# wang-xinyu/tensorrtx

Measured on AMD Instinct MI355X. Metric: images/sec @ batch=32 640x640 fp16 (yolov8n conv backbone + YoloLayer decode + NMS), higher is better.
Workload: dtype f16

## Files before the change

### include/trtx_hip.h

```cpp
#ifndef TRTX_HIP_H_
#define TRTX_HIP_H_

#include <stddef.h>
#include <stdint.h>

#ifdef __cplusplus
extern "C" {
#endif

#ifndef TRTX_NO_HIP_TYPES
struct ihipStream_t;
typedef struct ihipStream_t* trtx_stream_t;
#endif

#define TRTX_ABI_VERSION 1
#define TRTX_OK 0
#define TRTX_ERR_INVALID 1
#define TRTX_ERR_HIP 2
#define TRTX_ERR_WORKSPACE 3
#define TRTX_ERR_UNSUPPORTED 4
#define TRTX_ERR_NO_DEVICE 5
#define TRTX_ERR_IO 6
#define TRTX_ERR_STATE 7

// ... 19 lines not shown
                                   float* output, void* workspace, size_t workspace_bytes, trtx_stream_t stream);
int32_t trtx_yolo_task_head_decode_nhwc(const void* const* heads, const int* ld, const void* const* branches, const int* branch_ld,
                                        int n_levels, int batch, int classes, int net_h, int net_w, const int* strides,
                                        const float* dfl_weights, int max_out, int is_seg, int is_pose, int is_obb, int n_kpt,
                                        float kpt_conf, float* output, void* workspace, size_t workspace_bytes, trtx_stream_t stream);
int32_t trtx_yolo_task_head_decode_nhwc_f32(const void* const* heads, const int* ld, const void* const* branches, const int* branch_ld,
                                            int n_levels, int batch, int classes, int net_h, int net_w, const int* strides,
                                            const float* dfl_weights, int max_out, int is_seg, int is_pose, int is_obb, int n_kpt,
                                            float kpt_conf, float* output, void* workspace, size_t workspace_bytes, trtx_stream_t stream);

size_t trtx_yolo_nms_workspace(int batch);
int32_t trtx_yolo_nms(const float* decode_out, int batch, int max_out, float conf_thresh, float nms_thresh,
                      int32_t* keep_idx, int32_t* keep_cnt, float* keep_det, void* workspace, size_t workspace_bytes,
                      trtx_stream_t stream);


size_t trtx_yolov5_decode_workspace(int batch, const int* grid_w, const int* grid_h, int n_levels);
int32_t trtx_yolov5_decode(const float* const* inputs, int n_levels, int batch, int classes, int net_h, int net_w,
                           const int* grid_w, const int* grid_h, const float* anchors, int max_out, int is_segmentation,
                           float* output, void* workspace, size_t workspace_bytes, trtx_stream_t stream);
size_t trtx_yolov5_head_decode_workspace(int batch, const int* grid_w, const int* grid_h, int n_levels);
int32_t trtx_yolov5_head_decode_nhwc(const void* const* heads, const int* ld, int n_levels, int batch, int classes, int net_h, int net_w,
                                     const int* grid_w, const int* grid_h, const float* anchors, int max_out, float* output,
                                     void* workspace, size_t workspace_bytes, trtx_stream_t stream);
int32_t trtx_yolov5_head_decode_nhwc_f32(const void* const* heads, const int* ld, int n_levels, int batch, int classes, int net_h, int net_w,
                                         const int* grid_w, const int* grid_h, const float* anchors, int max_out, float* output,
                                         void* workspace, size_t workspace_bytes, trtx_stream_t stream);
size_t trtx_yolov7_decode_workspace(int batch, const int* grid_w, const int* grid_h, int n_levels);
int32_t trtx_yolov7_decode(const float* const* inputs, int n_levels, int batch, int classes, int net_h, int net_w,
                           const int* grid_w, const int* grid_h, const float* anchors, int max_out, float* output, void* workspace,
                           size_t workspace_bytes, trtx_stream_t stream);
size_t trtx_yolov7_head_decode_workspace(int batch, const int* grid_w, const int* grid_h, int n_levels);
int32_t trtx_yolov7_head_decode_nhwc(const void* const* heads, const int* ld, int n_levels, int batch, int classes, int net_h, int net_w,
                                     const int* grid_w, const int* grid_h, const float* anchors, int max_out, float* output,
                                     void* workspace, size_t workspace_bytes, trtx_stream_t stream);
int32_t trtx_yolov7_head_decode_nhwc_f32(const void* const* heads, const int* ld, int n_levels, int batch, int classes, int net_h, int net_w,
                                         const int* grid_w, const int* grid_h, const float* anchors, int max_out, float* output,
                                         void* workspace, size_t workspace_bytes, trtx_stream_t stream);
size_t trtx_darknet_decode_workspace(int batch, const int* grid_w, const int* grid_h, int n_levels);
int32_t trtx_darknet_decode(const float* const* inputs, int n_levels, int batch, int classes, int net_h, int net_w,
                            const int* grid_w, const int* grid_h, const float* anchors, int max_out, float* output, void* workspace,
                            size_t workspace_bytes, trtx_stream_t stream);
size_t trtx_darknet_head_decode_workspace(int batch, const int* grid_w, const int* grid_h, int n_levels);
int32_t trtx_darknet_head_decode_nhwc(const void* const* heads, const int* ld, int n_levels, int batch, int classes, int net_h, int net_w,
                                      const int* grid_w, const int* grid_h, const float* anchors, int max_out, float* output,
                                      void* workspace, size_t workspace_bytes, trtx_stream_t stream);
int32_t trtx_darknet_head_decode_nhwc_f32(const void* const* heads, const int* ld, int n_levels, int batch, int classes, int net_h, int net_w,
                                          const int* grid_w, const int* grid_h, const float* anchors, int max_out, float* output,
                                          void* workspace, size_t workspace_bytes, trtx_stream_t stream);
size_t trtx_yolov9_decode_workspace(int batch, int net_h, int net_w);
int32_t trtx_yolov9_decode(const float* const* inputs, int batch, int classes, int net_h, int net_w, int max_out, int is_segmentation,
                           float* output, void* workspace, size_t workspace_bytes, trtx_stream_t stream);
size_t trtx_yolov9_head_decode_workspace(int batch, int net_h, int net_w);
int32_t trtx_yolov9_head_decode_nhwc(const void* const* box, const int* box_ld, const void* const* cls, const int* cls_ld, int batch, int classes,
                                     int net_h, int net_w, const float* dfl_weights, int max_out, float* output, void* workspace,
                                     size_t workspace_bytes, trtx_stream_t stream);
int32_t trtx_yolov9_head_decode_nhwc_f32(const void* const* box, const int* box_ld, const void* const* cls, const int* cls_ld, int batch, int classes,
                                         int net_h, int net_w, const float* dfl_weights, int max_out, float* output, void* workspace,
                                         size_t workspace_bytes, trtx_stream_t stream);
int32_t trtx_yolo_nms_obb(const float* decode_out, int batch, int max_out, float conf_thresh, float nms_thresh, int32_t* keep_idx,
                          int32_t* keep_cnt, float* keep_det, void* workspace, size_t workspace_bytes, trtx_stream_t stream);
int32_t trtx_yolo_postprocess_gpu_obb(const float* decode_out, int batch, int max_out, float conf_thresh, float nms_thresh, float* out,
                                      trtx_stream_t stream);
int32_t trtx_yolov5_nms(const float* decode_out, int batch, int max_out, float conf_thresh, float nms_thresh, int32_t* keep_idx,
                        int32_t* keep_cnt, float* keep_det, void* workspace, size_t workspace_bytes, trtx_stream_t stream);
int32_t trtx_yolov9_nms(const float* decode_out, int batch, int max_out, float conf_thresh, float nms_thresh, int32_t* keep_idx,
                        int32_t* keep_cnt, float* keep_det, void* workspace, size_t workspace_bytes, trtx_stream_t stream);
int32_t trtx_yolov7_nms(const float* decode_out, int batch, int max_out, float conf_thresh, float nms_thresh, int32_t* keep_idx,
                        int32_t* keep_cnt, float* keep_det, void* workspace, size_t workspace_bytes, trtx_stream_t stream);
int32_t trtx_darknet_nms(const float* decode_out, int batch, int max_out, float conf_thresh, float nms_thresh, int32_t* keep_idx,
                         int32_t* keep_cnt, float* keep_det, void* workspace, size_t workspace_bytes, trtx_stream_t stream);
int32_t trtx_seg_masks(const float* decode_out, int det_floats, int box_format, const int32_t* keep_idx, const int32_t* keep_cnt, int batch,
                       int max_out, int max_keep, const float* proto, int mask_h, int mask_w, int net_h, int net_w, float* masks,
                       trtx_stream_t stream);

void trtx_letterbox_matrix(int src_w, int src_h, int dst_w, int dst_h, float* d2s_out );
int32_t trtx_letterbox_batch(const void* const* src, const int* src_w, const int* src_h, int batch, float* dst, int dst_w, int dst_h,
                             trtx_stream_t stream);
int32_t trtx_preprocess_init(int max_image_size, int ring_depth);
void trtx_preprocess_destroy(void);
int32_t trtx_batch_preprocess(const void* const* src_host, const int* src_w, const int* src_h, int batch, float* dst, int dst_w, int dst_h,
                              trtx_stream_t stream);

int32_t trtx_yolo_postprocess_gpu(const float* decode_out, int batch, int max_out, float conf_thresh, float nms_thresh,
                                  float* out, trtx_stream_t stream);

int32_t trtx_mish(const float* in, float* out, size_t n, trtx_stream_t stream);

size_t trtx_retina_decode_output_floats(int net_h, int net_w);
size_t trtx_retina_decode_workspace(int batch, int net_h, int net_w);
int32_t trtx_retina_decode(const float* const* inputs, int batch, int net_h, int net_w, float* output, void* workspace,
                           size_t workspace_bytes, trtx_stream_t stream);
size_t trtx_retina_nms_workspace(int batch, int net_h, int net_w);
int32_t trtx_retina_nms(const float* decode_out, int batch, int net_h, int net_w, double conf_thresh, float nms_thresh,
                        int max_keep, int32_t* keep_idx, int32_t* keep_cnt, float* keep_det, void* workspace,
                        size_t workspace_bytes, trtx_stream_t stream);

size_t trtx_rpn_decode_workspace(int batch, int num_anchors, int height, int width);
int32_t trtx_rpn_decode(int batch, const float* scores, const float* deltas, int height, int width, int image_height,
                        int image_width, float stride, const float* anchors_host, int num_anchors, int top_n,
                        float* out_scores, float* out_boxes, void* workspace, size_t workspace_bytes,
                        trtx_stream_t stream);
size_t trtx_sorted_nms_workspace(int batch, int n);
int32_t trtx_rpn_nms(int batch, const float* scores, const float* boxes, int pre_nms_topk, int post_nms_topk,
                     float nms_thresh, float* out_boxes, void* workspace, size_t workspace_bytes,
                     trtx_stream_t stream);
int32_t trtx_roi_align(int batch, const float* boxes, const float* features, int pooler_resolution, float spatial_scale,
                       int sampling_ratio, int num_proposals, int channels, int feature_h, int feature_w, float* out,
                       trtx_stream_t stream);
int32_t trtx_roi_align_nhwc_f16(int batch, const float* boxes, const void* features, int ld_in, int pooler_resolution,
                                float spatial_scale, int sampling_ratio, int num_proposals, int channels, int feature_h,
                                int feature_w, void* out, int ld_out, trtx_stream_t stream);
int32_t trtx_roi_align_nhwc_f16_strided(int batch, const float* boxes, const void* features, int ld_in, int pooler_resolution,
                                        float spatial_scale, int sampling_ratio, int num_proposals, int channels, int feature_h,
                                        int feature_w, void* out, int ld_out, int bin_step, trtx_stream_t stream);
size_t trtx_predictor_decode_workspace(int batch, int num_boxes, int num_classes);
int32_t trtx_predictor_decode(int batch, const float* scores, const float* deltas, const float* proposals, int num_boxes,
                              int num_classes, int image_height, int image_width, const float* bbox_reg_weights_host,
                              float* out_scores, float* out_boxes, float* out_classes, void* workspace,
                              size_t workspace_bytes, trtx_stream_t stream);
int32_t trtx_batched_nms(int nms_method, int batch, const float* scores, const float* boxes, const float* classes,
                         int count, int detections_per_im, float nms_thresh, float* out_scores, float* out_boxes,
                         float* out_classes, void* workspace, size_t workspace_bytes, trtx_stream_t stream);

int32_t trtx_mask_rcnn_inference(int batch, const float* labels, const float* masks, int detections_per_im, int output_size,
                                 int num_classes, float* out_masks, trtx_stream_t stream);

#define TRTX_ACT_NONE 0
#define TRTX_ACT_RELU 1
#define TRTX_ACT_SIGMOID 2
#define TRTX_ACT_SILU 3
#define TRTX_ACT_LEAKY 4
#define TRTX_ACT_TANH 5
int32_t trtx_conv_packed_dims(int cout, int cin_pad, int kh, int kw, int32_t* cout_pad, int32_t* kpad, int32_t* bn);
int32_t trtx_conv_pack_weights_f16(const float* w_kcrs, int cout, int cin, int kh, int kw, int cin_pad,
                                   const float* ch_scale, uint16_t* packed);
int32_t trtx_op_conv2d_nhwc_f16(const void* in, int N, int H, int W, int Cin, int ld_in, const void* wpacked,
                                const float* bias, void* out, int Cout, int ld_out, int kh, int kw, int sh, int sw,
                                int ph, int pw, int act1, const void* residual, int ld_res, int act2,
                                trtx_stream_t stream);
int32_t trtx_op_conv2d_tactics(int N, int H, int W, int Cin, int ld_in, int Cout, int ld_out, int kh, int kw, int sh, int sw, int ph, int pw,
                               int has_residual, int ld_res, int32_t* out6, int32_t max_out);
int32_t trtx_op_conv_force_tactic(const int32_t* tactic6);
int32_t trtx_op_conv_stem_nchw_f16(const float* in, int N, int C, int H, int W, const float* w_taps_cout, const float* bias, void* out, int Cout,
                                   int ld_out, int k, int stride, int pad, int act, trtx_stream_t stream);
int32_t trtx_op_conv_stem_pair_f16(const float* in, int N, int C, int H, int W, const float* stem_w_taps_cout, const float* stem_bias, int stem_act,
                                   const void* conv_wpacked, const float* conv_bias, int conv_act, void* out, int ld_out, trtx_stream_t stream);
int32_t trtx_op_conv_bneck_pair_f16(const void* in, int N, int H, int W, int ld_in, int in_coff, const void* w1_packed, const float* bias1, int act1,
                                    const void* w2_packed, const float* bias2, int act2, int shortcut, int act_after, void* out, int ld_out,
                                    trtx_stream_t stream);
int32_t trtx_op_conv_bneck_pair_or_two_f16(const void* in, int N, int H, int W, int ld_in, int in_coff, const void* w1_packed, const float* bias1, int act1,
                                           const void* w2_packed, const float* bias2, int act2, int shortcut, int act_after, void* mid, void* out,
                                           int ld_out, trtx_stream_t stream);
int32_t trtx_reorg_fold_weights(const float* w_kcrs, int cout, int cin, int kh, int kw, float* folded);
int32_t trtx_conv_packed_dims_f32(int cout, int cin_pad, int kh, int kw, int32_t* cout_pad, int32_t* kpad, int32_t* cink);
int32_t trtx_conv_pack_weights_f32(const float* w_kcrs, int cout, int cin, int kh, int kw, int cin_pad, const float* ch_scale, float* packed);
int32_t trtx_op_conv2d_nhwc_f32(const void* in, int N, int H, int W, int Cin, int ld_in, const void* wpacked, const float* bias, void* out, int Cout,
                                int ld_out, int kh, int kw, int sh, int sw, int ph, int pw, int act1, const void* residual, int ld_res, int act2,
                                const int32_t* tile4, trtx_stream_t stream);
int32_t trtx_op_conv2d_tactics_f32(int N, int H, int W, int Cin, int ld_in, int Cout, int ld_out, int kh, int kw, int sh, int sw, int ph, int pw,
                                   int has_residual, int ld_res, int32_t* out4, int32_t max_out);
int32_t trtx_conv_pack_weights_i8(const float* w_kcrs, int cout, int cin, int kh, int kw, const float* ch_scale, int8_t* packed, float* wscale_out,
                                  int32_t* cout_pad_out, int32_t* kpad_out);
int32_t trtx_op_conv2d_nhwc_i8(const void* in, int N, int H, int W, int Cin, int ld_in, const void* wpacked, const float* cscale, const float* bias, void* out,
                               int out_is_i8, float out_inv_scale, int Cout, int ld_out, int kh, int kw, int sh, int sw, int ph, int pw, int act1,
                               const void* residual, int res_is_i8, float res_scale, int ld_res, int act2, trtx_stream_t stream);
int32_t trtx_conv_pack_weights_grouped_f16(const float* w_kcrs, int cout, int cin_g, int kh, int kw, const float* ch_scale, uint16_t* packed,
                                           int32_t* kpad_out);
int32_t trtx_op_conv2d_grouped_nhwc_f16(const void* in, int N, int H, int W, int Cin, int ld_in, const void* wpacked, const float* bias, void* out,
                                        int Cout, int ld_out, int groups, int k, int pad, int act1, const void* residual, int ld_res, int act2,
                                        trtx_stream_t stream);
int32_t trtx_op_conv2d_dw_nhwc(const void* in, int dtype, int N, int H, int W, int C, int ld_in, const float* w_taps_c, const float* bias, void* out, int ld_out,
                               const void* residual, int ld_res, int k, int stride, int pad, int dilation, int act1, float alpha1, int act2, float alpha2,
                               trtx_stream_t stream);
int32_t trtx_op_psa_attention_f16(const void* qkv, int ld_qkv, void* out, int ld_out, void* vimg, int ld_v, int B, int heads, int N, int kd, int hd, float scale,
                                  trtx_stream_t stream);
int32_t trtx_op_area_attention_f16(const void* qkv, int ld_qkv, void* out, int ld_out, void* vimg, int ld_v, int B, int heads, int N, int area, int kd, int hd,
                                   float scale, trtx_stream_t stream);
int32_t trtx_op_area_attention_split_f16(const void* q, int ld_q, const void* k, int ld_k, const void* v, int ld_v, void* out, int ld_out, int B, int heads,
                                         int N, int area, int kd, int hd, float scale, trtx_stream_t stream);
size_t trtx_op_hgconv_workspace_bytes(int B, int N, int D, int E);
int32_t trtx_op_hgconv_geometry(int32_t* tiles, int max_tiles, int32_t* n_tiles);
int32_t trtx_op_hgconv_f16(const void* x, int ld_x, void* out, int ld_out, int B, int N, int D, int E, float logit_scale, const float* w_ctx, const float* b_ctx,
                           const float* proto, const float* w_pre, const float* b_pre, const float* w_edge, const float* b_edge, const float* w_node,
                           const float* b_node, void* workspace, size_t workspace_bytes, trtx_stream_t stream);
int32_t trtx_op_poison_lds(void* device_word, trtx_stream_t stream);
int32_t trtx_op_nchw_f32_to_nhwc_f16(const float* in, void* out, int N, int C, int H, int W, int Cpad, int ld_out,
                                     trtx_stream_t stream);
int32_t trtx_op_nhwc_f16_to_nchw_f32(const void* in, float* out, int N, int C, int H, int W, int ld_in,
                                     trtx_stream_t stream);

typedef struct trtx_builder trtx_builder;
typedef struct trtx_network trtx_network;
typedef struct trtx_hostmem trtx_hostmem;
typedef struct trtx_engine trtx_engine;
typedef struct trtx_context trtx_context;
typedef struct trtx_plugin trtx_plugin;

#define TRTX_MAX_DIMS 8
typedef struct trtx_dims {
    int32_t nb;
    int64_t d[TRTX_MAX_DIMS];
} trtx_dims;

#define TRTX_DTYPE_FLOAT 0
#define TRTX_DTYPE_HALF 1
#define TRTX_DTYPE_INT8 2
#define TRTX_DTYPE_INT32 3
#define TRTX_ACTIVATION_RELU 0
#define TRTX_ACTIVATION_SIGMOID 1
#define TRTX_ACTIVATION_TANH 2
#define TRTX_ACTIVATION_LEAKY_RELU 3
#define TRTX_POOLING_MAX 0
#define TRTX_POOLING_AVERAGE 1
#define TRTX_ELEMENTWISE_SUM 0
#define TRTX_ELEMENTWISE_PROD 1
#define TRTX_ELEMENTWISE_MAX 2
#define TRTX_ELEMENTWISE_MIN 3
#define TRTX_ELEMENTWISE_SUB 4
#define TRTX_ELEMENTWISE_DIV 5
#define TRTX_ELEMENTWISE_POW 6
#define TRTX_SCALE_UNIFORM 0
#define TRTX_SCALE_CHANNEL 1
#define TRTX_SCALE_ELEMENTWISE 2
#define TRTX_REDUCE_SUM 0
#define TRTX_REDUCE_PROD 1
#define TRTX_REDUCE_MAX 2
#define TRTX_REDUCE_MIN 3
#define TRTX_REDUCE_AVG 4
#define TRTX_MATMUL_NONE 0
#define TRTX_MATMUL_TRANSPOSE 1
#define TRTX_MATMUL_VECTOR 2
#define TRTX_UNARY_EXP 0
#define TRTX_UNARY_LAST 23
#define TRTX_RESIZE_NEAREST 0
#define TRTX_RESIZE_LINEAR 1
#define TRTX_FLAG_FP16 0
#define TRTX_FLAG_INT8 1
#define TRTX_P_STRIDE 1
#define TRTX_P_PADDING 2
#define TRTX_P_DILATION 3
#define TRTX_P_GROUPS 4
#define TRTX_P_ALPHA 5
#define TRTX_P_BETA 6
#define TRTX_P_AXIS 7
#define TRTX_P_RESHAPE 8
#define TRTX_P_FIRST_TRANSPOSE 9
#define TRTX_P_SECOND_TRANSPOSE 10
#define TRTX_P_RESIZE_MODE 11
#define TRTX_P_RESIZE_SCALES 12
#define TRTX_P_RESIZE_OUT_DIMS 13
#define TRTX_P_AVG_EXCLUSIVE 14
#define TRTX_P_KERNEL 15
#define TRTX_P_NB_OUT 16

typedef struct trtx_plugin_vtbl {
    void* self;
    int32_t (*get_nb_outputs)(void* self);
    int32_t (*get_output_dims)(void* self, int32_t index, const trtx_dims* inputs, int32_t nb_inputs, trtx_dims* out);
    int32_t (*configure)(void* self, const trtx_dims* in, int32_t nb_in, const trtx_dims* out, int32_t nb_out,
                         int32_t max_batch);
    int32_t (*initialize)(void* self);
    void (*terminate)(void* self);
    size_t (*workspace_size)(void* self, int32_t max_batch);
    int32_t (*enqueue)(void* self, int32_t batch, const void* const* inputs, void* const* outputs, void* workspace,
                       trtx_stream_t stream);
    size_t (*serialization_size)(void* self);
    void (*serialize)(void* self, void* buffer);
    const char* (*plugin_type)(void* self);
    const char* (*plugin_version)(void* self);
    int32_t (*clone)(void* self, struct trtx_plugin_vtbl* out);
    void (*destroy)(void* self);
} trtx_plugin_vtbl;

typedef struct trtx_plugin_field {
    const char* name;
    const void* data;
    int32_t type;
    int32_t length;
} trtx_plugin_field;

typedef struct trtx_creator_vtbl {
    void* self;
    const char* (*plugin_name)(void* self);
    const char* (*plugin_version)(void* self);
    int32_t (*create)(void* self, const char* name, const trtx_plugin_field* fields, int32_t nb_fields,
                      trtx_plugin_vtbl* out);
    int32_t (*deserialize)(void* self, const char* name, const void* data, size_t length, trtx_plugin_vtbl* out);
} trtx_creator_vtbl;

int32_t trtx_registry_register(const trtx_creator_vtbl* creator);
int32_t trtx_registry_get(const char* name, const char* version, trtx_creator_vtbl* out);

typedef struct trtx_wts trtx_wts;
int32_t trtx_wts_load(const char* path, trtx_wts** out);
int32_t trtx_wts_count(const trtx_wts* w);
int32_t trtx_wts_entry(const trtx_wts* w, int32_t i, const char** name, const float** values, int64_t* count);
int32_t trtx_wts_find(const trtx_wts* w, const char* name, const float** values, int64_t* count);
void trtx_wts_free(trtx_wts* w);

int32_t trtx_builder_create(trtx_builder** out);
void trtx_builder_destroy(trtx_builder* b);
int32_t trtx_builder_set_max_batch(trtx_builder* b, int32_t n);
int32_t trtx_builder_set_flag(trtx_builder* b, int32_t flag, int32_t on);
int32_t trtx_builder_set_workspace(trtx_builder* b, size_t bytes);
typedef struct trtx_calibrator_vtbl {
// ... 88 lines not shown
```

### tensorrtx_amd/capi.py

```python
import ctypes
import os

_HERE = os.path.dirname(os.path.abspath(__file__))
_LIB = None


class TrtxError(RuntimeError):
    def __init__(self, status, what):
        self.status = status
        msg = lib().trtx_status_string(status).decode() if _LIB is not None else "?"
        super().__init__(f"{what}: status {status} ({msg})")


def lib_path() -> str:
    return os.environ.get("TRTX_HIP_LIB") or os.path.join(_HERE, "lib", "libtrtx_hip.so")


def hip_runtimes_mapped():
    seen = []
    with open("/proc/self/maps") as f:
        for line in f:
            path = line.rsplit(" ", 1)[-1].strip()
            if "libamdhip64" in os.path.basename(path) and path not in seen:
                seen.append(path)
# ... 331 lines not shown
    return out


def yolov9_head_decode_nhwc(box, cls, classes, net_h, net_w, dfl_w, max_out=1000, out=None, batch=None, box_ld=None, cls_ld=None, ws=None):
    import torch
    L = lib()
    assert len(box) == 3 and len(cls) == 3
    B = box[0].shape[0] if batch is None else batch
    dev = box[0].device
    bp = (ctypes.c_void_p * 3)(*[x.data_ptr() for x in box])
    cp = (ctypes.c_void_p * 3)(*[x.data_ptr() for x in cls])
    bl = (ctypes.c_int * 3)(*(box_ld if box_ld is not None else [x.shape[-1] for x in box]))
    cl = (ctypes.c_int * 3)(*(cls_ld if cls_ld is not None else [x.shape[-1] for x in cls]))
    L.trtx_yolov9_head_decode_workspace.restype = ctypes.c_size_t
    if ws is None:
        ws = torch.empty(max(L.trtx_yolov9_head_decode_workspace(B, net_h, net_w), 256), dtype=torch.uint8, device=dev)
    if out is None:
        out = torch.zeros((B, 1 + max_out * DET5_FLOATS), dtype=torch.float32, device=dev)
    fn = L.trtx_yolov9_head_decode_nhwc_f32 if box[0].dtype == torch.float32 else L.trtx_yolov9_head_decode_nhwc
    check(fn(bp, bl, cp, cl, B, classes, net_h, net_w, _p(dfl_w), max_out, _p(out), _p(ws), ctypes.c_size_t(ws.numel()), _stream()),
          "trtx_yolov9_head_decode_nhwc")
    return out


def yolov9_nms(decode_out, max_out=1000, conf_thresh=0.5, nms_thresh=0.45, out=None, ws=None):
    L = lib()
    B = decode_out.shape[0]
    keep_idx, keep_cnt, keep_det, ws = _nms_buffers(B, max_out, 6, decode_out.device, out, ws)
    check(L.trtx_yolov9_nms(_p(decode_out), B, max_out, ctypes.c_float(conf_thresh), ctypes.c_float(nms_thresh), _p(keep_idx), _p(keep_cnt),
                            _p(keep_det), _p(ws), ctypes.c_size_t(ws.numel()), _stream()), "trtx_yolov9_nms")
    return keep_idx, keep_cnt, keep_det


def seg_masks(decode_out, keep_idx, keep_cnt, proto, net_h, net_w, max_keep, box_format=0, out=None):
    import torch
    B, max_out = keep_idx.shape
    assert decode_out.shape[0] == B and (decode_out.shape[1] - 1) % max_out == 0
    det_floats = (decode_out.shape[1] - 1) // max_out
    assert proto.dim() == 4 and proto.shape[0] == B and proto.shape[1] == 32
    mask_h, mask_w = int(proto.shape[2]), int(proto.shape[3])
    for t, dt in ((decode_out, torch.float32), (keep_idx, torch.int32), (keep_cnt, torch.int32), (proto, torch.float32)):
        assert t.is_cuda and t.dtype == dt and t.is_contiguous()
    if out is None:
        out = torch.zeros((B, max(max_keep, 0), mask_h, mask_w), dtype=torch.float32, device=proto.device)
    assert out.is_cuda and out.dtype == torch.float32 and out.is_contiguous() and out.numel() >= B * max(max_keep, 0) * mask_h * mask_w
    check(lib().trtx_seg_masks(_p(decode_out), det_floats, box_format, _p(keep_idx), _p(keep_cnt), B, max_out, max_keep, _p(proto), mask_h,
                               mask_w, net_h, net_w, _p(out), _stream()), "trtx_seg_masks")
    return out


def yolo_postprocess_gpu(decode_out, max_out=1000, conf_thresh=0.5, nms_thresh=0.45, out=None, ws=None):
    import torch
    B = decode_out.shape[0]
    if out is None:
        out = torch.empty((B, 1 + max_out * 7), dtype=torch.float32, device=decode_out.device)
    check(lib().trtx_yolo_postprocess_gpu(_p(decode_out), B, max_out, ctypes.c_float(conf_thresh), ctypes.c_float(nms_thresh),
                                          _p(out), _stream()), "trtx_yolo_postprocess_gpu")
    return out


ACT = {"none": 0, "relu": 1, "sigmoid": 2, "silu": 3, "leaky": 4, "tanh": 5, "mish": 6}


def _hw(v):
    if isinstance(v, (tuple, list)):
        h, w = v
        return int(h), int(w)
    return int(v), int(v)


def pack_conv_weights_f16(w_kcrs, cin_pad=None, ch_scale=None):
    import numpy as np
    L = lib()
    w = np.ascontiguousarray(w_kcrs, dtype=np.float32)
    cout, cin, kh, kw = w.shape
    cin_pad = cin_pad or (cin + 7) // 8 * 8
    cp, kp, bn = ctypes.c_int32(), ctypes.c_int32(), ctypes.c_int32()
    check(L.trtx_conv_packed_dims(cout, cin_pad, kh, kw, ctypes.byref(cp), ctypes.byref(kp), ctypes.byref(bn)),
          "trtx_conv_packed_dims")
    packed = np.zeros((cp.value, kp.value), dtype=np.uint16)
    sc = None
    if ch_scale is not None:
        sc = np.ascontiguousarray(ch_scale, dtype=np.float32)
    check(L.trtx_conv_pack_weights_f16(w.ctypes.data_as(ctypes.c_void_p), cout, cin, kh, kw, cin_pad,
                                       sc.ctypes.data_as(ctypes.c_void_p) if sc is not None else None,
                                       packed.ctypes.data_as(ctypes.c_void_p)), "trtx_conv_pack_weights_f16")
    return packed, cp.value, kp.value, bn.value


def conv2d_nhwc_f16(x, wpacked, bias, cout, kh, kw, stride, pad, act1="none", residual=None, act2="none",
                    out=None, out_ld=None):
    import torch
    L = lib()
    N, H, W, Cin = x.shape
    (sh, sw), (ph, pw) = _hw(stride), _hw(pad)
    Ho = (H + 2 * ph - kh) // sh + 1
    Wo = (W + 2 * pw - kw) // sw + 1
    if out is None:
        out = torch.empty((N, Ho, Wo, cout), dtype=torch.float16, device=x.device)
    ld_out = out_ld or out.shape[-1]
    check(L.trtx_op_conv2d_nhwc_f16(_p(x), N, H, W, Cin, x.stride(2), _p(wpacked), _p(bias), _p(out), cout, ld_out,
                                    kh, kw, sh, sw, ph, pw, ACT[act1], _p(residual),
                                    residual.stride(2) if residual is not None else 0, ACT[act2], _stream()),
          "trtx_op_conv2d_nhwc_f16")
    return out


def stem_weights(w_kcrs):
    import numpy as np
    w = np.ascontiguousarray(w_kcrs, dtype=np.float32)
    return np.ascontiguousarray(w.reshape(w.shape[0], -1).T)


def conv_stem_nchw_f16(x, w_taps_cout, bias, k, stride, pad, act="none", out=None, out_ld=None):
    import torch
    N, C, H, W = x.shape
    cout = w_taps_cout.shape[1]
    Ho, Wo = (H + 2 * pad - k) // stride + 1, (W + 2 * pad - k) // stride + 1
    if out is None:
        out = torch.empty((N, Ho, Wo, cout), dtype=torch.float16, device=x.device)
    check(lib().trtx_op_conv_stem_nchw_f16(_p(x), N, C, H, W, _p(w_taps_cout), _p(bias), _p(out), cout, out_ld or out.shape[-1], k, stride, pad,
                                           ACT[act], _stream()), "trtx_op_conv_stem_nchw_f16")
    return out


def conv_stem_pair_f16(x, stem_w_taps_cout, stem_bias, conv_wpacked, conv_bias, stem_act="silu", conv_act="silu", out=None, out_ld=None):
    import torch
    N, C, H, W = x.shape
    Hi, Wi = (H - 1) // 2 + 1, (W - 1) // 2 + 1
    Ho, Wo = (Hi - 1) // 2 + 1, (Wi - 1) // 2 + 1
    if out is None:
        out = torch.empty((N, Ho, Wo, 32), dtype=torch.float16, device=x.device)
    check(lib().trtx_op_conv_stem_pair_f16(_p(x), N, C, H, W, _p(stem_w_taps_cout), _p(stem_bias), ACT[stem_act], _p(conv_wpacked), _p(conv_bias),
                                           ACT[conv_act], _p(out), out_ld or out.shape[-1], _stream()), "trtx_op_conv_stem_pair_f16")
    return out


def conv_bneck_pair_f16(x, w1_packed, bias1, w2_packed, bias2, act1="silu", act2="silu", shortcut=True, act_after="none", out=None, out_ld=None, in_coff=None,
                        mid=None):
    import torch
    N, H, W, C = x.shape
    assert x.dtype == torch.float16 and x.stride(3) == 1 and (C == 16 if in_coff is None else in_coff + 16 <= C)
    if out is None:
        out = torch.empty((N, H, W, 16), dtype=torch.float16, device=x.device)
    head = (_p(x), N, H, W, x.stride(2), in_coff or 0, _p(w1_packed), _p(bias1), ACT[act1], _p(w2_packed), _p(bias2), ACT[act2], 1 if shortcut else 0, ACT[act_after])
    if mid is None:
        check(lib().trtx_op_conv_bneck_pair_f16(*head, _p(out), out_ld or out.shape[-1], _stream()), "trtx_op_conv_bneck_pair_f16")
    else:
        assert mid.dtype == torch.float16 and mid.is_contiguous() and tuple(mid.shape) == (N, H, W, 16)
        check(lib().trtx_op_conv_bneck_pair_or_two_f16(*head, _p(mid), _p(out), out_ld or out.shape[-1], _stream()), "trtx_op_conv_bneck_pair_or_two_f16")
    return out


def pack_conv_weights_grouped_f16(w_kcrs, ch_scale=None):
    import numpy as np
    L = lib()
    w = np.ascontiguousarray(w_kcrs, dtype=np.float32)
    cout, cin_g, kh, kw = w.shape
    kp = ctypes.c_int32()
    check(L.trtx_conv_pack_weights_grouped_f16(w.ctypes.data_as(ctypes.c_void_p), cout, cin_g, kh, kw, None, None, ctypes.byref(kp)),
          "trtx_conv_pack_weights_grouped_f16 (dims)")
    packed = np.zeros((cout, kp.value), dtype=np.uint16)
    sc = None if ch_scale is None else np.ascontiguousarray(ch_scale, dtype=np.float32)
    check(L.trtx_conv_pack_weights_grouped_f16(w.ctypes.data_as(ctypes.c_void_p), cout, cin_g, kh, kw,
                                               sc.ctypes.data_as(ctypes.c_void_p) if sc is not None else None,
                                               packed.ctypes.data_as(ctypes.c_void_p), ctypes.byref(kp)), "trtx_conv_pack_weights_grouped_f16")
    return packed


def conv2d_grouped_nhwc_f16(x, wpacked, bias, cout, groups, k, pad, act1="none", residual=None, act2="none", out=None, out_ld=None):
    import torch
    N, H, W, Cin = x.shape
    if out is None:
        out = torch.empty((N, H + 2 * pad - k + 1, W + 2 * pad - k + 1, cout), dtype=torch.float16, device=x.device)
    check(lib().trtx_op_conv2d_grouped_nhwc_f16(_p(x), N, H, W, Cin, x.stride(2), _p(wpacked), _p(bias), _p(out), cout, out_ld or out.shape[-1], groups, k,
                                                pad, ACT[act1], _p(residual), residual.stride(2) if residual is not None else 0, ACT[act2], _stream()),
          "trtx_op_conv2d_grouped_nhwc_f16")
    return out


def conv2d_dw_nhwc(x, w, bias, k, stride, act1="none", residual=None, act2="none", out=None, out_ld=None, alpha1=0.1, alpha2=0.1, pad=None, dilation=1):
    import numpy as np
    import torch
    N, H, W, C = x.shape
    assert x.dtype in (torch.float16, torch.float32) and (residual is None or residual.dtype == x.dtype)
    pad = k // 2 if pad is None else pad
    Ho, Wo = (H + 2 * pad - dilation * (k - 1) - 1) // stride + 1, (W + 2 * pad - dilation * (k - 1) - 1) // stride + 1
    taps = np.ascontiguousarray(np.asarray(w, dtype=np.float32).reshape(C, k * k).T)
    wg = torch.from_numpy(taps).to(x.device)
    if out is None:
        out = torch.empty((N, Ho, Wo, C), dtype=x.dtype, device=x.device)
    assert out.dtype == x.dtype
    check(lib().trtx_op_conv2d_dw_nhwc(_p(x), 1 if x.dtype == torch.float16 else 0, N, H, W, C, x.stride(2), _p(wg), _p(bias), _p(out),
                                       out_ld or out.shape[-1], _p(residual), residual.stride(2) if residual is not None else 0, k, stride, pad, dilation,
                                       ACT[act1], ctypes.c_float(alpha1), ACT[act2], ctypes.c_float(alpha2), _stream()), "trtx_op_conv2d_dw_nhwc")
    return out


def _attention(fn, what, qkv, heads, scale, out, vimg, out_ld, v_ld, qkv_ld, kd, hd, extra):
    import torch
    B, N, _ = qkv.shape
    for t in (qkv, out, vimg):
        assert t.is_cuda and t.dtype == torch.float16
    check(fn(_p(qkv), qkv_ld or qkv.stride(1), _p(out), out_ld or out.stride(1), _p(vimg), v_ld or vimg.stride(1), B, heads, N, *extra, kd, hd,
             ctypes.c_float(scale), _stream()), what)
    return out, vimg


def psa_attention(qkv, heads, scale, out=None, vimg=None, out_ld=None, v_ld=None, qkv_ld=None, kd=32, hd=64):
    import torch
    B, N, _ = qkv.shape
    out = torch.empty((B, N, heads * hd), dtype=torch.float16, device=qkv.device) if out is None else out
    vimg = torch.empty((B, N, heads * hd), dtype=torch.float16, device=qkv.device) if vimg is None else vimg
    return _attention(lib().trtx_op_psa_attention_f16, "trtx_op_psa_attention_f16", qkv, heads, scale, out, vimg, out_ld, v_ld, qkv_ld, kd, hd, ())


def area_attention(qkv, heads, area, scale, out=None, vimg=None, out_ld=None, v_ld=None, qkv_ld=None, kd=32, hd=32):
    import torch
    B, N, _ = qkv.shape
    out = torch.empty((B, N, heads * hd), dtype=torch.float16, device=qkv.device) if out is None else out
    vimg = torch.empty((B, N, heads * hd), dtype=torch.float16, device=qkv.device) if vimg is None else vimg
    return _attention(lib().trtx_op_area_attention_f16, "trtx_op_area_attention_f16", qkv, heads, scale, out, vimg, out_ld, v_ld, qkv_ld, kd, hd, (area,))


def area_attention_split(q, k, v, heads, area, scale, out=None, q_ld=None, k_ld=None, v_ld=None, out_ld=None, kd=32, hd=32):
    import torch
    B, N, _ = q.shape
    out = torch.empty((B, N, heads * hd), dtype=torch.float16, device=q.device) if out is None else out
    for t in (q, k, v, out):
        assert t.is_cuda and t.dtype == torch.float16
    check(lib().trtx_op_area_attention_split_f16(_p(q), q_ld or q.stride(1), _p(k), k_ld or k.stride(1), _p(v), v_ld or v.stride(1), _p(out),
                                                 out_ld or out.stride(1), B, heads, N, area, kd, hd, ctypes.c_float(scale), _stream()),
          "trtx_op_area_attention_split_f16")
    return out


HGCONV_WEIGHTS = ("w_ctx", "b_ctx", "proto", "w_pre", "b_pre", "w_edge", "b_edge", "w_node", "b_node")


def hgconv_workspace_bytes(B, N, D, E):
    L = lib()
    L.trtx_op_hgconv_workspace_bytes.restype = ctypes.c_size_t
    return int(L.trtx_op_hgconv_workspace_bytes(int(B), int(N), int(D), int(E)))


def hgconv_geometry():
    arr, n = (ctypes.c_int32 * 8)(), ctypes.c_int32()
    check(lib().trtx_op_hgconv_geometry(arr, 8, ctypes.byref(n)), "trtx_op_hgconv_geometry")
    return [int(arr[i]) for i in range(min(n.value, 8))]


def hgconv(x, E, logit_scale, weights, out=None, x_ld=None, out_ld=None, D=None, workspace=None):
    import torch
    L = lib()
    B, N, Dx = x.shape
    D = Dx if D is None else D
    assert x.is_cuda and x.dtype == torch.float16
    out = torch.empty((B, N, D), dtype=torch.float16, device=x.device) if out is None else out
    assert out.is_cuda and out.dtype == torch.float16
    ws = workspace if workspace is not None else torch.empty(max(hgconv_workspace_bytes(B, N, D, E), 256), dtype=torch.uint8, device=x.device)
    ws_arr = [weights[k].contiguous() for k in HGCONV_WEIGHTS]
    for w in ws_arr:
        assert w.is_cuda and w.dtype == torch.float32
    L.trtx_op_hgconv_f16.argtypes = ([ctypes.c_void_p, ctypes.c_int, ctypes.c_void_p, ctypes.c_int] + [ctypes.c_int] * 4 + [ctypes.c_float] +
                                     [ctypes.c_void_p] * 9 + [ctypes.c_void_p, ctypes.c_size_t, ctypes.c_void_p])
    check(L.trtx_op_hgconv_f16(_p(x), x_ld or x.stride(1), _p(out), out_ld or out.stride(1), B, N, D, E, float(logit_scale), *[_p(w) for w in ws_arr],
                               _p(ws), ws.numel(), _stream()), "trtx_op_hgconv_f16")
    return out


def pack_conv_weights_f32(w_kcrs, cin_pad=None, ch_scale=None):
    import numpy as np
    L = lib()
    w = np.ascontiguousarray(w_kcrs, dtype=np.float32)
    cout, cin, kh, kw = w.shape
    cin_pad = cin_pad or (cin + 3) // 4 * 4
    cp, kp, ck = ctypes.c_int32(), ctypes.c_int32(), ctypes.c_int32()
    check(L.trtx_conv_packed_dims_f32(cout, cin_pad, kh, kw, ctypes.byref(cp), ctypes.byref(kp), ctypes.byref(ck)), "trtx_conv_packed_dims_f32")
    packed = np.zeros((cp.value, kp.value), dtype=np.float32)
    sc = np.ascontiguousarray(ch_scale, dtype=np.float32) if ch_scale is not None else None
    check(L.trtx_conv_pack_weights_f32(w.ctypes.data_as(ctypes.c_void_p), cout, cin, kh, kw, cin_pad,
                                       sc.ctypes.data_as(ctypes.c_void_p) if sc is not None else None,
                                       packed.ctypes.data_as(ctypes.c_void_p)), "trtx_conv_pack_weights_f32")
    return packed, cp.value, kp.value, ck.value


def conv2d_nhwc_f32(x, wpacked, bias, cout, kh, kw, stride, pad, act1="none", residual=None, act2="none", out=None, out_ld=None, tile=None):
    import torch
    L = lib()
    N, H, W, Cin = x.shape
    if bias is not None and bias.numel() < (cout + 15) // 16 * 16:
        raise ValueError(f"bias holds {bias.numel()} floats, the fp32 tile reads cout_pad = {(cout + 15) // 16 * 16}")
    (sh, sw), (ph, pw) = _hw(stride), _hw(pad)
    Ho = (H + 2 * ph - kh) // sh + 1
    Wo = (W + 2 * pw - kw) // sw + 1
    if out is None:
        out = torch.empty((N, Ho, Wo, cout), dtype=torch.float32, device=x.device)
    ld_out = out_ld or out.shape[-1]
    t2 = (ctypes.c_int32 * 4)(*tile) if tile is not None else None
    check(L.trtx_op_conv2d_nhwc_f32(_p(x), N, H, W, Cin, x.stride(2), _p(wpacked), _p(bias), _p(out), cout, ld_out, kh, kw, sh, sw, ph, pw,
                                    ACT[act1], _p(residual), residual.stride(2) if residual is not None else 0, ACT[act2], t2, _stream()),
          "trtx_op_conv2d_nhwc_f32")
    return out


def conv2d_tactics_f32(N, H, W, Cin, Cout, k, stride, pad, residual=False, ld_in=None, ld_out=None, ld_res=None, max_out=32):
# ... 62 lines not shown
```

### tensorrtx_amd/csrc/kernels/conv_igemm.hip

```cpp
#include "../options.h"
#include "igemm_tile.h"
#include "patch_tile.h"

namespace trtx {
namespace {


struct ConvPatchGroupArgs {
    int n;
    int slot_start[kMaxConvGroup + 1];
    int chunk[kMaxConvGroup], tiles[kMaxConvGroup], tiles_n[kMaxConvGroup], tiles_x[kMaxConvGroup], tiles_y[kMaxConvGroup];
    unsigned in_bytes[kMaxConvGroup], w_bytes[kMaxConvGroup];
    ConvArgs p[kMaxConvGroup];
};
template <int NFRAG, int KC, int MI>
__global__ __launch_bounds__(256) void conv_patch_group_f16_kernel(const ConvPatchGroupArgs g) {
    __shared__ __attribute__((aligned(16))) char smem[patch_lds_bytes<NFRAG, KC, MI>()];
    const int xcd = blockIdx.x & 7, slot = blockIdx.x >> 3;
    int pid = 0;
#pragma unroll
    for (int k = 1; k < kMaxConvGroup; ++k) pid += (k < g.n && slot >= g.slot_start[k]) ? 1 : 0;
    pid = __builtin_amdgcn_readfirstlane(pid);
    const int local = xcd * g.chunk[pid] + (slot - g.slot_start[pid]);
    if (local >= g.tiles[pid]) return;
// ... 457 lines not shown
    const bool ws_ok = fp16 && !pinned && conv_ws_supported(a);
    if (ws_ok) push(a.bn, a.bk, 128, WSK_OFF, WS_ON);
    else push(a.bn, a.bk, 128, (wsk_default(a) && !work_efficient_only && !pinned) ? WSK_ON : WSK_OFF, WS_OFF);
    if (fp16 && options().gemm256 && conv_gemm256_worthwhile(a)) push(256, 64, 256, WSK_OFF, WS_OFF);
    const int bks[2] = {a.bk, (fp16 && a.CinK % 64 == 0 && a.CinK != 16 && a.Kpad % 64 == 0) ? (a.bk == 32 ? 64 : 32) : a.bk};
    static const int bns[5] = {128, 80, 64, 32, 16};
    for (int bi = 0; bi < 5; ++bi) {
        const int bn = bns[bi];
        if (a.Cout_pad % bn) continue;
        if (bn == 16 && a.Cout_pad > 32 && bn != a.bn) continue;
        if (work_efficient_only && bn != a.bn && bn != 64) continue;
        for (int ki = 0; ki < 2; ++ki) {
            ConvArgs t = a;
            t.bn = bn;
            t.bk = bks[ki];
            if (ki == 1 && bks[1] == bks[0]) continue;
            push(bn, t.bk, 128, WSK_OFF, WS_OFF);
            if (bm64_possible(t) && !work_efficient_only) push(bn, t.bk, 64, WSK_OFF, WS_OFF);
            if (bm256_possible(t) && (long)((a.M + 255) / 256) * (a.Cout_pad / bn) >= 512) push(bn, t.bk, 256, WSK_OFF, WS_OFF);
            if (wsk_possible(t) && !work_efficient_only && !pinned) push(bn, t.bk, 128, WSK_ON, WS_OFF);
            if (fp16 && options().patch && patch_possible(t)) push(bn, t.bk, 128, WSK_OFF, WS_PATCH);
            if (fp16 && (options().res & 1) && conv_res_possible(t)) push(bn, t.bk, 128, WSK_OFF, WS_RES3);
            if (fp16 && (options().res & 2) && !work_efficient_only && conv_res1_possible(t)) push(bn, t.bk, 128, WSK_OFF, WS_RES1);
        }
    }
    return n;
}

void conv_apply_tactic(ConvArgs* a, const ConvTactic& t) {
    a->bn = t.bn;
    a->bk = t.bk;
    a->bm = t.bm;
    a->t_wsk = t.wsk;
    a->t_ws = t.ws;
}

int32_t conv_igemm_f16(const ConvArgs& a0, hipStream_t s) {
    if (!conv_igemm_supported(a0) || (a0.in_i8 && !a0.cscale)) return TRTX_ERR_UNSUPPORTED;
    const bool fp16 = !a0.in_i8 && !a0.out_i8 && !a0.res_i8;
    if (a0.bn == 256) return conv_gemm256_f16(a0, s);
    if (fp16 && a0.t_ws == WS_RES3 && conv_res_possible(a0)) return conv_res_f16(&a0, 1, s);
    if (fp16 && a0.t_ws == WS_RES1 && conv_res1_possible(a0)) return conv_res1_f16(a0, s);
    if (fp16 && a0.t_ws != WS_OFF && a0.t_ws != WS_PATCH && a0.t_ws != WS_RES3 && a0.t_ws != WS_RES1 && conv_ws_supported(a0)) return conv_ws_f16(a0, s);
    const size_t img_in = (size_t)a0.H * a0.W * a0.ld_in * 2;
    const int per = (int)std::max<size_t>(1, (size_t)2000000000 / img_in);
    const unsigned w_bytes = (unsigned)((size_t)a0.Cout_pad * a0.Kpad * 2);
    for (int n0 = 0; n0 < a0.N; n0 += per) {
        ConvArgs a = a0;
        a.N = std::min(per, a0.N - n0);
        a.M = a.N * a.Ho * a.Wo;
        a.in = static_cast<const char*>(a0.in) + (size_t)n0 * img_in;
        a.out = static_cast<char*>(a0.out) + (size_t)n0 * a.Ho * a.Wo * a.ld_out * (a0.out_i8 ? 1 : 2);
        if (a0.residual) a.residual = static_cast<const char*>(a0.residual) + (size_t)n0 * a.Ho * a.Wo * a.ld_res * (a0.res_i8 ? 1 : 2);
        if (a0.up_C) a.up_in = static_cast<const char*>(a0.up_in) + (size_t)n0 * a.up_H * a.up_W * a.up_ld * 2;
        const unsigned in_bytes = (unsigned)((((size_t)a.N * a.H * a.W - 1) * a.ld_in + a.Cin) * 2);
        const bool wsk = a.t_wsk == WSK_OFF ? false : (a.t_wsk == WSK_ON ? wsk_possible(a) : wsk_default(a));
        const bool bm64 = a.bm == 64, bm256 = a.bm == 256;
        int32_t st = TRTX_OK;
        if (a.in_i8) {
            st = launch_bn<32, 1, true>(a, in_bytes, w_bytes, s);
        } else if (a.t_ws == WS_PATCH && patch_possible(a)) {
            st = launch_patch(a, in_bytes, w_bytes, s);
        } else if (wsk) {
            if (a.bn == 64) launch_wsk<4>(a, in_bytes, w_bytes, s);
            else launch_wsk<5>(a, in_bytes, w_bytes, s);
        } else if (a.bk == 64) {
            st = bm64 ? launch_bn<64, 1, false, 1>(a, in_bytes, w_bytes, s)
                      : (bm256 ? launch_bn<64, 1, false, 4>(a, in_bytes, w_bytes, s) : launch_bn<64, 1>(a, in_bytes, w_bytes, s));
        } else if (a.CinK == 16) {
            st = launch_bn<32, 2>(a, in_bytes, w_bytes, s);
        } else {
            st = bm64 ? launch_bn<32, 1, false, 1>(a, in_bytes, w_bytes, s)
                      : (bm256 ? launch_bn<32, 1, false, 4>(a, in_bytes, w_bytes, s) : launch_bn<32, 1>(a, in_bytes, w_bytes, s));
        }
        if (st != TRTX_OK) return st;
    }
    return check_launch("conv_igemm_f16");
}

namespace {
bool group_member_ok(const ConvArgs& a) {
    return conv_igemm_supported(a) && (a.in_i8 || (!a.out_i8 && !a.res_i8)) && !a.up_C && !a.scalar_out && a.CinK != 16 && a.bk == 32 && (a.bn == 64 || a.bn == 80) &&
           (a.bm == 0 || a.bm == 128) && a.t_wsk != WSK_ON && a.t_ws != WS_PATCH && (double)a.N * a.H * a.W * a.ld_in * 2.0 < 2.0e9;
}
template <int NFRAG, bool RS, bool ONE, bool I8 = false>
void launch_group(const ConvGroupArgs& g, hipStream_t s) {
    TRTX_LAUNCH((conv_igemm_group_f16_kernel<NFRAG, 32, RS, ONE, I8>), dim3(g.slot_start[g.n] * 8), dim3(256), 0, s, g);
}
}

bool conv_igemm_group_supported(const ConvArgs* a, int n) {
    if (n < 2 || n > kMaxConvGroup) return false;
    for (int k = 0; k < n; ++k) {
        if (!group_member_ok(a[k])) return false;
        if (a[k].t_ws != WS_OFF && conv_ws_supported(a[k])) return false;
        if (a[k].bn != a[0].bn || a[k].in_i8 != a[0].in_i8 || (a[k].t_rs != 0) != (a[0].t_rs != 0) || plain_gemm(a[k]) != plain_gemm(a[0])) return false;
    }
    return true;
}

int32_t conv_igemm_group_f16(const ConvArgs* a, int n, hipStream_t s) {
    if (!conv_igemm_group_supported(a, n)) return TRTX_ERR_UNSUPPORTED;
    if ((options().res & 4) && conv_res_group_possible(a, n)) return conv_res_f16(a, n, s);
    if (options().patch && patch_group_possible(a, n)) {
        const int32_t st = launch_patch_group(a, n, s);
        return st != TRTX_OK ? st : check_launch("conv_patch_group_f16");
    }
    ConvGroupArgs g{};
    g.n = n;
    int order[kMaxConvGroup];
    for (int k = 0; k < n; ++k) order[k] = k;
    std::sort(order, order + n, [&](int x, int y) {
        if (a[x].Kpad != a[y].Kpad) return a[x].Kpad > a[y].Kpad;
        const long mx = (long)a[x].N * a[x].Ho * a[x].Wo, my = (long)a[y].N * a[y].Ho * a[y].Wo;
        return mx != my ? mx > my : x < y;
    });
    int slots = 0;
    for (int k = 0; k < n; ++k) {
        const ConvArgs& ak = a[order[k]];
        g.p[k] = ak;
        g.p[k].M = ak.N * ak.Ho * ak.Wo;
        g.tiles_n[k] = ak.Cout_pad / ak.bn;
        g.tiles[k] = ((g.p[k].M + 127) / 128) * g.tiles_n[k];
        g.chunk[k] = (g.tiles[k] + 7) / 8;
        g.slot_start[k] = slots;
        slots += g.chunk[k];
        g.in_bytes[k] = (unsigned)((((size_t)ak.N * ak.H * ak.W - 1) * ak.ld_in + ak.Cin) * 2);
        g.w_bytes[k] = (unsigned)((size_t)ak.Cout_pad * ak.Kpad * 2);
    }
    for (int k = n; k <= kMaxConvGroup; ++k) g.slot_start[k] = slots;
    const bool rs = a[0].t_rs != 0;
    const bool one = plain_gemm(a[0]);
    const int nf = a[0].bn / 16;
    if (a[0].in_i8) {
        for (int k = 0; k < n; ++k)
            if (!a[k].cscale) return TRTX_ERR_UNSUPPORTED;
        if (nf == 4) {
            if (one) rs ? launch_group<4, true, true, true>(g, s) : launch_group<4, false, true, true>(g, s);
            else rs ? launch_group<4, true, false, true>(g, s) : launch_group<4, false, false, true>(g, s);
        } else {
            if (one) rs ? launch_group<5, true, true, true>(g, s) : launch_group<5, false, true, true>(g, s);
            else rs ? launch_group<5, true, false, true>(g, s) : launch_group<5, false, false, true>(g, s);
        }
    } else if (nf == 4) {
        if (one) rs ? launch_group<4, true, true>(g, s) : launch_group<4, false, true>(g, s);
        else rs ? launch_group<4, true, false>(g, s) : launch_group<4, false, false>(g, s);
    } else {
        if (one) rs ? launch_group<5, true, true>(g, s) : launch_group<5, false, true>(g, s);
        else rs ? launch_group<5, true, false>(g, s) : launch_group<5, false, false>(g, s);
    }
    return check_launch("conv_igemm_group_f16");
}

}
```

### tensorrtx_amd/csrc/kernels/igemm_tile.h

```cpp
#pragma once
#include <hip/hip_fp16.h>
#include <hip/hip_runtime.h>
#include <stdint.h>
#include <stdlib.h>
#include <string.h>

#include <algorithm>
#include <type_traits>

#include "../common.h"
#include "act.h"
#include "kernels.h"
#include "launch.h"
#include "patch_index.h"

#ifndef TRTX_STAMP
#define TRTX_STAMP(i, kt)
#endif
#ifndef TRTX_MARK
#define TRTX_MARK(i)
#endif

namespace trtx {
namespace {
// ... 135 lines not shown
                      (p.act2 == ACT_NONE || p.act2 == ACT_RELU);
#ifndef TRTX_NO_FAST_EPILOGUE
    if (fast) {
        if (res) conv_epilogue_fast<NFRAG, MI, I8, true, PS, !BIAS_FIXED>(p, acc, acci, mine, bias_lds, lane, n0, rbase, bf0, bf1, second, pixel_of);
        else conv_epilogue_fast<NFRAG, MI, I8, false, PS, !BIAS_FIXED>(p, acc, acci, mine, bias_lds, lane, n0, rbase, bf0, bf1, second, pixel_of);
        return;
    }
#endif
#pragma nounroll
    for (int i = 0; i < MI; ++i) {
#pragma unroll
        for (int ii = 0; ii < MI; ++ii) {
            if (ii != i) continue;
#pragma unroll
            for (int j = 0; j < NFRAG; ++j) {
                floatx4 v = acc[ii][j];
                if constexpr (I8) {
                    const float4 cs = *reinterpret_cast<const float4*>(p.cscale + n0 + j * 16 + ch_in);
                    v = floatx4{(float)acci[ii][j][0] * cs.x, (float)acci[ii][j][1] * cs.y, (float)acci[ii][j][2] * cs.z, (float)acci[ii][j][3] * cs.w};
                }
                *reinterpret_cast<floatx4*>(mine + px_in * PS + (j * 16 + ch_in) * 4) = v;
            }
        }
#pragma nounroll
        for (int q = lane; q < ITEMS; q += 64) {
            const int row = q / CPR, cc = q % CPR;
            const int m = pixel_of(rbase + i * 16 + row);
            const int co = n0 + cc * 8;
            if (m < 0 || co >= p.Cout) continue;
            const floatx4 lo = *reinterpret_cast<const floatx4*>(mine + row * PS + cc * 32);
            const floatx4 hi = *reinterpret_cast<const floatx4*>(mine + row * PS + cc * 32 + 16);
            float x[8] = {lo[0], lo[1], lo[2], lo[3], hi[0], hi[1], hi[2], hi[3]};
            if (p.bias) {
                float4 b0 = bf0, b1 = bf1;
                if constexpr (!BIAS_FIXED) {
                    b0 = *reinterpret_cast<const float4*>(bias_lds + cc * 32);
                    b1 = *reinterpret_cast<const float4*>(bias_lds + cc * 32 + 16);
                }
                x[0] += b0.x; x[1] += b0.y; x[2] += b0.z; x[3] += b0.w;
                x[4] += b1.x; x[5] += b1.y; x[6] += b1.z; x[7] += b1.w;
            }
            half8 v;
            if (p.act1 == ACT_SILU) {
#pragma unroll
                for (int e = 0; e < 8; ++e) v[e] = round_to_half(x[e] * __builtin_amdgcn_rcpf(1.0f + __expf(-x[e])));
            } else if (p.act1 == ACT_RELU) {
#pragma unroll
                for (int e = 0; e < 8; ++e) v[e] = round_to_half(x[e] > 0.f ? x[e] : 0.f);
            } else if (p.act1 == ACT_NONE) {
#pragma unroll
                for (int e = 0; e < 8; ++e) v[e] = round_to_half(x[e]);
            } else {
#pragma nounroll
                for (int e = 0; e < 8; ++e) v[e] = round_to_half(act_fast_rare(x[e], p.act1, p.alpha1));
            }
            const bool vec = !p.scalar_out;
            if (second) {
                half8 rv = half8{0, 0, 0, 0, 0, 0, 0, 0};
                if (res) {
                    if (p.res_i8) {
                        const long long rq = *reinterpret_cast<const long long*>(static_cast<const int8_t*>(p.residual) + (size_t)m * p.ld_res + co);
#pragma unroll
                        for (int e = 0; e < 8; ++e) rv[e] = round_to_half((float)(int8_t)(rq >> (8 * e)) * p.res_scale);
                    } else if (vec) {
                        rv = *reinterpret_cast<const half8*>(res + (size_t)m * p.ld_res + co);
                    } else {
#pragma nounroll
                        for (int e = 0; e < 8; ++e)
                            if (co + e < p.Cout) rv[e] = res[(size_t)m * p.ld_res + co + e];
                    }
                }
                if (p.act2 == ACT_NONE) {
#pragma unroll
                    for (int e = 0; e < 8; ++e) v[e] = round_to_half((float)v[e] + (float)rv[e]);
                } else if (p.act2 == ACT_RELU) {
#pragma unroll
                    for (int e = 0; e < 8; ++e) {
                        const float t = (float)v[e] + (float)rv[e];
                        v[e] = round_to_half(t > 0.f ? t : 0.f);
                    }
                } else {
#pragma nounroll
                    for (int e = 0; e < 8; ++e) v[e] = round_to_half(act_fast((float)v[e] + (float)rv[e], p.act2, p.alpha2));
                }
            }
            if (p.out_i8) {
                unsigned long long qv = 0;
#pragma unroll
                for (int e = 0; e < 8; ++e) {
                    float t = rintf((float)v[e] * p.out_inv_scale);
                    t = t > 127.f ? 127.f : (t < -127.f ? -127.f : t);
                    qv |= (unsigned long long)(unsigned char)(int8_t)(int)t << (8 * e);
                }
                *reinterpret_cast<unsigned long long*>(static_cast<int8_t*>(p.out) + (size_t)m * p.ld_out + co) = qv;
            } else if (vec) {
                *reinterpret_cast<half8*>(out + (size_t)m * p.ld_out + co) = v;
            } else {
#pragma nounroll
                for (int e = 0; e < 8; ++e)
                    if (co + e < p.Cout) out[(size_t)m * p.ld_out + co + e] = v[e];
            }
        }
    }
}

template <int NFRAG, int MI, typename PixelOf>
__device__ __forceinline__ void conv_epilogue_f32(const ConvArgs& p, floatx4 (&acc)[MI][NFRAG], int lane, int n0, PixelOf&& pixel_of, int rbase) {
    float* __restrict__ out = static_cast<float*>(p.out);
    const float* __restrict__ res = static_cast<const float*>(p.residual);
    const int px_in = lane & 15;
    const int ch_in = (lane >> 4) * 4;
    const bool vec = !p.scalar_out;
#pragma nounroll
    for (int i = 0; i < MI; ++i) {
        floatx4 v[NFRAG];
#pragma unroll
        for (int ii = 0; ii < MI; ++ii) {
            if (ii != i) continue;
#pragma unroll
            for (int j = 0; j < NFRAG; ++j) v[j] = acc[ii][j];
        }
        const int m = pixel_of(rbase + i * 16 + px_in);
#pragma unroll
        for (int j = 0; j < NFRAG; ++j) {
            const int co = n0 + j * 16 + ch_in;
            if (m < 0 || co >= p.Cout) continue;
            floatx4 x = v[j];
#pragma unroll
            for (int e = 0; e < 4; ++e) x[e] = act_f32(x[e], p.act1, p.alpha1);
            if (res) {
                floatx4 r = floatx4{0.f, 0.f, 0.f, 0.f};
                if (vec) {
                    r = *reinterpret_cast<const floatx4*>(res + (size_t)m * p.ld_res + co);
                } else {
#pragma unroll
                    for (int e = 0; e < 4; ++e)
                        if (co + e < p.Cout) r[e] = res[(size_t)m * p.ld_res + co + e];
                }
                x += r;
            }
#pragma unroll
            for (int e = 0; e < 4; ++e) x[e] = act_f32(x[e], p.act2, p.alpha2);
            if (vec) {
                *reinterpret_cast<floatx4*>(out + (size_t)m * p.ld_out + co) = x;
            } else {
#pragma unroll
                for (int e = 0; e < 4; ++e)
                    if (co + e < p.Cout) out[(size_t)m * p.ld_out + co + e] = x[e];
            }
        }
    }
}

template <int NFRAG, int BKT, int MI, bool RS>
constexpr int igemm_lds_bytes() {
    constexpr int BN = 16 * NFRAG, BM = kWaves * 16 * MI, ROW_B = BKT * 2, CH = BKT / 8, RPI = 64 / CH;
    constexpr int B_PASSES = (BN + kWaves * RPI - 1) / (kWaves * RPI), B_ROWS = B_PASSES * kWaves * RPI;
    constexpr int STAGE_BYTES = BM * ROW_B + B_ROWS * ROW_B;
    constexpr int NST = RS ? 2 : (BKT == 64 ? 2 : 3);
    constexpr int EPI_BYTES = kWaves * 16 * (16 * NFRAG * 4 + 16);
    return NST * STAGE_BYTES > EPI_BYTES ? NST * STAGE_BYTES : EPI_BYTES;
}

template <int NFRAG, int BKT, int TPS, bool I8 = false, int MI = 2, bool RS = false, bool UP = false, bool ONE = false, bool F32 = false, bool ROLES = false>
__device__ __forceinline__ void conv_igemm_tile(const ConvArgs& p, unsigned in_bytes, unsigned w_bytes, const int m0, const int n0, char* __restrict__ smem) {
    TRTX_MARK(0);
    constexpr int BN = 16 * NFRAG;
    constexpr int BM = kWaves * 16 * MI;
    constexpr int WR = 16 * MI;
    constexpr int ROW_B = BKT * 2;
    constexpr int CH = BKT / 8;
    constexpr int RPI = 64 / CH;
    constexpr int A_LOADS = BM / (kWaves * RPI);
    constexpr int B_PASSES = (BN + kWaves * RPI - 1) / (kWaves * RPI);
    constexpr int B_ROWS = B_PASSES * kWaves * RPI;
    constexpr int A_BYTES = BM * ROW_B;
    constexpr int STAGE_BYTES = A_BYTES + B_ROWS * ROW_B;
    constexpr int LOADS_PER_TILE = A_LOADS + B_PASSES;
    constexpr int KSUB = BKT / 32;
    constexpr int NST = RS ? 2 : (BKT == 64 ? 2 : 3);
    constexpr int EPI_BYTES = kWaves * 16 * (16 * NFRAG * 4 + 16);
    constexpr int LDS_BYTES = NST * STAGE_BYTES > EPI_BYTES ? NST * STAGE_BYTES : EPI_BYTES;
    static_assert(LDS_BYTES == igemm_lds_bytes<NFRAG, BKT, MI, RS>(), "the entry points allocate what the tile function uses");

    const int tid = threadIdx.x;
    const int lane = tid & 63;
    const int wave_all = __builtin_amdgcn_readfirstlane(tid >> 6);
    const bool fetcher = ROLES && wave_all >= kWaves;
    const int wave = ROLES ? (wave_all & (kWaves - 1)) : wave_all;
    static_assert(!ROLES || !RS, "roles: LDS-DMA operands, 4 + 4 waves");

    const __amdgpu_buffer_rsrc_t rs_in = __builtin_amdgcn_make_buffer_rsrc(const_cast<void*>(p.in), 0, in_bytes, 0x00020000);
    const __amdgpu_buffer_rsrc_t rs_w = __builtin_amdgcn_make_buffer_rsrc(const_cast<void*>(p.wgt), 0, w_bytes, 0x00020000);
    const unsigned up_bytes = UP ? (unsigned)((((size_t)p.N * p.up_H * p.up_W - 1) * p.up_ld + p.up_C) * 2) : 0u;
    const __amdgpu_buffer_rsrc_t rs_up = UP ? __builtin_amdgcn_make_buffer_rsrc(const_cast<void*>(p.up_in), 0, up_bytes, 0x00020000) : rs_in;

    const int lrow = lane / CH;
    const int lswz = BKT == 32 ? swz<32>(lrow) : ((lrow >> 1) | ((wave & 1) << 2));
    const int lchunk = (lane % CH) ^ lswz;
    const int tsel = TPS == 2 ? (lchunk >> 1) : 0;
    const int cchunk = TPS == 2 ? (lchunk & 1) : lchunk;
    const int HoWo = p.Ho * p.Wo;
    const float inv_howo = __builtin_amdgcn_rcpf((float)HoWo), inv_wo = __builtin_amdgcn_rcpf((float)p.Wo);
    unsigned a_base[A_LOADS];
    unsigned a_rows[A_LOADS];
    unsigned a_cols[A_LOADS];
    unsigned a_up[UP ? A_LOADS : 1];
#pragma unroll
    for (int i = 0; i < A_LOADS; ++i) {
        const int m = m0 + (kWaves * i + wave) * RPI + lrow;
        const bool ok = m < p.M;
        const int mm = ok ? m : 0;
        int n = (int)((float)mm * inv_howo);
        int rem = mm - n * HoWo;
        if (rem < 0) { --n; rem += HoWo; }
        if (rem >= HoWo) { ++n; rem -= HoWo; }
        int ho = (int)((float)rem * inv_wo);
        int wo = rem - ho * p.Wo;
        if (wo < 0) { --ho; wo += p.Wo; }
        if (wo >= p.Wo) { ++ho; wo -= p.Wo; }
        const int hi0 = ho * p.stride_h - p.pad_h;
        const int wi0 = wo * p.stride_w - p.pad_w;
        a_base[i] = (unsigned)(((n * p.H + hi0) * p.W + wi0) * p.ld_in + cchunk * 8) * 2u;
        if constexpr (UP) a_up[i] = (unsigned)(((n * p.up_H + (ho >> 1)) * p.up_W + (wo >> 1)) * p.up_ld + cchunk * 8) * 2u;
        if constexpr (ONE) a_base[i] = ok ? a_base[i] : kOOB;
        a_rows[i] = ok ? tap_range_mask(hi0, p.kh, p.H) : 0u;
        a_cols[i] = tap_range_mask(wi0, p.kw, p.W);
    }
    const int cmax = p.Cin - cchunk * 8;
    unsigned b_off[B_PASSES];
#pragma unroll
    for (int j = 0; j < B_PASSES; ++j) {
        const int row = (kWaves * j + wave) * RPI + lrow;
        b_off[j] = row < BN ? (unsigned)(((n0 + row) * p.Kpad + lchunk * 8) * 2) : kOOB;
    }
    constexpr bool B_PARTIAL = !RS && (BN % (kWaves * RPI) != 0);
    const bool b_last_live = !B_PARTIAL || (kWaves * (B_PASSES - 1) + wave) * RPI < BN;

    const int nk = p.Kpad / BKT;
    int s_kt = 0, s_uc = 0;
    unsigned a_taps[A_LOADS];
    unsigned t_add = 0, t_tap = 0;
    const int spt = p.CinK / BKT;
    const float inv_spt = __builtin_amdgcn_rcpf((float)spt), inv_kw = __builtin_amdgcn_rcpf((float)p.kw);
    auto build_window = [&](int base) {
        const int e = base + lane;
        const int tap = (int)(((float)e + 0.5f) * inv_spt);
        const int ucs = (e - tap * spt) * BKT;
        const int r = (int)(((float)tap + 0.5f) * inv_kw);
        const int q = tap - r * p.kw;
        t_add = (unsigned)((r * p.dil_h * p.W + q * p.dil_w) * p.ld_in + ucs) * 2u;
        t_tap = (unsigned)(tap < 31 ? tap : 31) | ((unsigned)ucs << 8);
    };
    if (TPS == 1) {
        build_window(0);
        unsigned rep = 0;
        for (int r = 0; r < p.kh; ++r) rep |= 1u << (r * p.kw);
#pragma unroll
        for (int i = 0; i < A_LOADS; ++i) {
            const unsigned rows = a_rows[i];
            const int lo = rows ? __builtin_ctz(rows) : 0, hi = rows ? 32 - __builtin_clz(rows) : 0;
            const unsigned range = hi > lo ? ((hi * p.kw >= 32 ? ~0u : ((1u << (hi * p.kw)) - 1u)) & ~((1u << (lo * p.kw)) - 1u)) : 0u;
            a_taps[i] = (a_cols[i] * rep) & range;
        }
    }
    const bool full_c = p.Cin == p.CinK;
    int s_r[TPS], s_q[TPS];
    unsigned s_toff[TPS];
    auto tap_next = [&](int& r, int& q) {
        ++q;
        const int wq = q == p.kw;
        q = wq ? 0 : q;
        r += wq;
    };
    s_r[0] = 0;
    s_q[0] = 0;
    if constexpr (TPS == 2) {
        s_r[1] = 0;
        s_q[1] = 0;
        tap_next(s_r[1], s_q[1]);
    }
#pragma unroll
    for (int t = 0; t < TPS; ++t) s_toff[t] = (unsigned)((s_r[t] * p.dil_h * p.W + s_q[t] * p.dil_w) * p.ld_in) * 2u;

    intx4 ra[RS ? A_LOADS : 1], rb[RS ? B_PASSES : 1];
    auto issue_tile = [&](int stage) {
        char* sbase = smem + stage * STAGE_BYTES;
        const bool live = s_kt < nk;
        if constexpr (ONE) {
            const unsigned koff = (unsigned)s_kt * (unsigned)(BKT * 2);
#pragma unroll
            for (int i = 0; i < A_LOADS; ++i) {
                const unsigned voff = a_base[i] + koff;
                if constexpr (RS) ra[i] = __builtin_amdgcn_raw_buffer_load_b128(rs_in, voff, 0, 0);
                else __builtin_amdgcn_raw_ptr_buffer_load_lds(rs_in, (lds_ptr_t)(sbase + (kWaves * i + wave) * RPI * ROW_B), 16, voff, 0, 0, 0);
            }
        } else if (TPS == 1) {
            const unsigned add = (unsigned)__builtin_amdgcn_readlane((int)t_add, s_kt & 63);
            const unsigned tw = (unsigned)__builtin_amdgcn_readlane((int)t_tap, s_kt & 63);
            const int tap = (int)(tw & 255u), uc = (int)(tw >> 8);
            const bool chunk_ok = full_c || uc < cmax;
            const bool from_up = UP && uc < p.up_C;
            const __amdgpu_buffer_rsrc_t rs_a = from_up ? rs_up : rs_in;
#pragma unroll
            for (int i = 0; i < A_LOADS; ++i) {
                const bool ok = ((a_taps[i] >> tap) & 1u) && chunk_ok && live;
                unsigned voff = ok ? a_base[i] + add : kOOB;
                if constexpr (UP) voff = from_up ? (ok ? a_up[i] + (unsigned)uc * 2u : kOOB) : voff;
                if constexpr (RS) ra[i] = __builtin_amdgcn_raw_buffer_load_b128(rs_a, voff, 0, 0);
                else __builtin_amdgcn_raw_ptr_buffer_load_lds(rs_a, (lds_ptr_t)(sbase + (kWaves * i + wave) * RPI * ROW_B), 16, voff, 0, 0, 0);
            }
        } else {
            const int r = tsel ? s_r[TPS - 1] : s_r[0];
            const int q = tsel ? s_q[TPS - 1] : s_q[0];
            const unsigned add = (tsel ? s_toff[TPS - 1] : s_toff[0]) + (unsigned)s_uc * 2u;
#pragma unroll
            for (int i = 0; i < A_LOADS; ++i) {
                const bool ok = ((a_rows[i] >> r) & (a_cols[i] >> q) & 1u) && s_uc < cmax && live;
                const unsigned voff = ok ? a_base[i] + add : kOOB;
                if constexpr (RS) ra[i] = __builtin_amdgcn_raw_buffer_load_b128(rs_in, voff, 0, 0);
                else __builtin_amdgcn_raw_ptr_buffer_load_lds(rs_in, (lds_ptr_t)(sbase + (kWaves * i + wave) * RPI * ROW_B), 16, voff, 0, 0, 0);
            }
        }
#pragma unroll
        for (int j = 0; j < B_PASSES; ++j) {
            if (B_PARTIAL && j == B_PASSES - 1 && !b_last_live) continue;
            const unsigned voff = ONE ? b_off[j] : (s_kt < nk ? b_off[j] : kOOB);
            if constexpr (RS) rb[j] = __builtin_amdgcn_raw_buffer_load_b128(rs_w, voff, 0, 0);
            else __builtin_amdgcn_raw_ptr_buffer_load_lds(rs_w, (lds_ptr_t)(sbase + A_BYTES + (kWaves * j + wave) * RPI * ROW_B), 16, voff, 0, 0, 0);
            b_off[j] += BKT * 2;
        }
        ++s_kt;
        if (TPS == 2) {
#pragma unroll
            for (int t = 0; t < TPS; ++t) {
                tap_next(s_r[t], s_q[t]);
                tap_next(s_r[t], s_q[t]);
                s_toff[t] = (unsigned)((s_r[t] * p.dil_h * p.W + s_q[t] * p.dil_w) * p.ld_in) * 2u;
            }
        } else if (!ONE && (s_kt & 63) == 0) {
            build_window(s_kt);
        }
    };

    auto commit = [&](int stage) {
        char* sbase = smem + stage * STAGE_BYTES + lane * 16;
#pragma unroll
        for (int i = 0; i < A_LOADS; ++i) *reinterpret_cast<intx4*>(sbase + (kWaves * i + wave) * RPI * ROW_B) = ra[i];
#pragma unroll
        for (int j = 0; j < B_PASSES; ++j) *reinterpret_cast<intx4*>(sbase + A_BYTES + (kWaves * j + wave) * RPI * ROW_B) = rb[j];
    };

    floatx4 acc[MI][NFRAG];
    intx4 acci[MI][NFRAG];
    floatx4 part[F32 ? MI : 1][F32 ? NFRAG : 1];
#pragma unroll
    for (int i = 0; i < MI; ++i)
#pragma unroll
        for (int j = 0; j < NFRAG; ++j) {
            acc[i][j] = floatx4{0.f, 0.f, 0.f, 0.f};
            acci[i][j] = intx4{0, 0, 0, 0};
            if constexpr (F32) part[i][j] = floatx4{0.f, 0.f, 0.f, 0.f};
        }
    if constexpr (F32) {
        if (p.bias) {
#pragma unroll
            for (int j = 0; j < NFRAG; ++j) {
                const floatx4 b4 = *reinterpret_cast<const floatx4*>(p.bias + n0 + j * 16 + (lane >> 4) * 4);
#pragma unroll
                for (int i = 0; i < MI; ++i) acc[i][j] = b4;
            }
        }
    }

    const int frow = lane & 15;
    const int fswz = swz<BKT>(frow);
    int f_off[KSUB];
#pragma unroll
    for (int h = 0; h < KSUB; ++h) f_off[h] = frow * ROW_B + ((((lane >> 4) + 4 * h) ^ fswz) * 16);
    const int a_frag = wave * WR * ROW_B;
    const int b_frag = A_BYTES;

    auto compute = [&](int stage) {
        const char* sb = smem + stage * STAGE_BYTES;
        if constexpr (F32) {
            static_assert(!F32 || !I8, "fp32 operands");
            __builtin_amdgcn_s_setprio(1);
#pragma unroll
            for (int h = 0; h < KSUB; ++h) {
                floatx4 af[MI], bf[NFRAG];
#pragma unroll
                for (int i = 0; i < MI; ++i) af[i] = *reinterpret_cast<const floatx4*>(sb + a_frag + i * 16 * ROW_B + f_off[h]);
#pragma unroll
                for (int j = 0; j < NFRAG; ++j) bf[j] = *reinterpret_cast<const floatx4*>(sb + b_frag + j * 16 * ROW_B + f_off[h]);
#pragma unroll
                for (int j = 0; j < NFRAG; ++j)
#pragma unroll
                    for (int i = 0; i < MI; ++i) {
                        acc[i][j] += part[i][j];
                        part[i][j] = __builtin_amdgcn_mfma_f32_16x16x4f32(bf[j][0], af[i][0], floatx4{0.f, 0.f, 0.f, 0.f}, 0, 0, 0);
                    }
#pragma unroll
                for (int s4 = 1; s4 < 4; ++s4)
#pragma unroll
                    for (int j = 0; j < NFRAG; ++j)
#pragma unroll
                        for (int i = 0; i < MI; ++i) part[i][j] = __builtin_amdgcn_mfma_f32_16x16x4f32(bf[j][s4], af[i][s4], part[i][j], 0, 0, 0);
            }
            __builtin_amdgcn_s_setprio(0);
            return;
        }
#pragma unroll
        for (int h = 0; h < KSUB; ++h) {
            if constexpr (I8) {
                intx4 af[MI];
#pragma unroll
                for (int i = 0; i < MI; ++i) af[i] = *reinterpret_cast<const intx4*>(sb + a_frag + i * 16 * ROW_B + f_off[h]);
#pragma unroll
                for (int j = 0; j < NFRAG; ++j) {
                    const intx4 bf = *reinterpret_cast<const intx4*>(sb + b_frag + j * 16 * ROW_B + f_off[h]);
#pragma unroll
                    for (int i = 0; i < MI; ++i) acci[i][j] = __builtin_amdgcn_mfma_i32_16x16x64_i8(bf, af[i], acci[i][j], 0, 0, 0);
                }
            } else {
                half8 af[MI];
#pragma unroll
                for (int i = 0; i < MI; ++i) af[i] = *reinterpret_cast<const half8*>(sb + a_frag + i * 16 * ROW_B + f_off[h]);
#pragma unroll
                for (int j = 0; j < NFRAG; ++j) {
                    const half8 bf = *reinterpret_cast<const half8*>(sb + b_frag + j * 16 * ROW_B + f_off[h]);
#pragma unroll
                    for (int i = 0; i < MI; ++i) acc[i][j] = __builtin_amdgcn_mfma_f32_16x16x32_f16(bf, af[i], acc[i][j], 0, 0, 0);
                }
            }
        }
    };

#define TRTX_KSTEP(S)                                                         \
    {                                                                         \
        TRTX_STAMP(0, kt);                                                    \
        if (B_PARTIAL && !b_last_live) asm volatile("s_waitcnt vmcnt(%0) lgkmcnt(0)" ::"n"((LOADS_PER_TILE - 1) * (NST - 2)) : "memory"); \
        else asm volatile("s_waitcnt vmcnt(%0) lgkmcnt(0)" ::"n"(LOADS_PER_TILE * (NST - 2)) : "memory"); \
        TRTX_STAMP(1, kt);                                                    \
        __builtin_amdgcn_s_barrier();                                         \
        TRTX_STAMP(2, kt);                                                    \
        issue_tile(((S) + NST - 1) % NST);                                    \
        TRTX_STAMP(3, kt);                                                    \
        compute(S);                                                           \
        TRTX_STAMP(4, kt);                                                    \
    }

    if constexpr (ROLES) {
        if (fetcher) {
#pragma unroll
            for (int st = 0; st < NST - 1; ++st) issue_tile(st);
            for (int kt = 0;;) {
                bool done = false;
#pragma unroll
                for (int st = 0; st < NST; ++st) {
                    if (done) continue;
                    if (B_PARTIAL && !b_last_live) asm volatile("s_waitcnt vmcnt(%0)" ::"n"((LOADS_PER_TILE - 1) * (NST - 2)) : "memory");
                    else asm volatile("s_waitcnt vmcnt(%0)" ::"n"(LOADS_PER_TILE * (NST - 2)) : "memory");
                    __builtin_amdgcn_s_barrier();
                    issue_tile((st + NST - 1) % NST);
                    if (++kt == nk) done = true;
                }
                if (done) break;
            }
            asm volatile("s_waitcnt vmcnt(0)" ::: "memory");
            if constexpr (!F32) __builtin_amdgcn_s_barrier();
            return;
        }
        for (int kt = 0;;) {
            bool done = false;
#pragma unroll
            for (int st = 0; st < NST; ++st) {
                if (done) continue;
                asm volatile("s_waitcnt lgkmcnt(0)" ::: "memory");
                __builtin_amdgcn_s_barrier();
                compute(st);
                if (++kt == nk) done = true;
            }
            if (done) break;
        }
        if constexpr (!F32) __builtin_amdgcn_s_barrier();
    } else if constexpr (RS) {
        issue_tile(0);
        commit(0);
        issue_tile(0);
        for (int kt = 0;;) {
            asm volatile("s_waitcnt lgkmcnt(0)" ::: "memory");
            __builtin_amdgcn_s_barrier();
            compute(kt & 1);
            commit((kt + 1) & 1);
            issue_tile(0);
            if (++kt == nk) break;
        }
    } else {
#pragma unroll
    for (int st = 0; st < NST - 1; ++st) {
        issue_tile(st);
        if (st == 0) TRTX_MARK(1);
    }
    for (int kt = 0;;) {
        bool done = false;
#pragma unroll
        for (int st = 0; st < NST; ++st) {
            if (done) continue;
            TRTX_KSTEP(st);
            if (++kt == nk) done = true;
        }
        if (done) break;
    }
    }
#undef TRTX_KSTEP
    asm volatile("s_waitcnt vmcnt(0)" ::: "memory");
    TRTX_MARK(2);

    if constexpr (F32) {
#pragma unroll
        for (int i = 0; i < MI; ++i)
#pragma unroll
            for (int j = 0; j < NFRAG; ++j) acc[i][j] += part[i][j];
        conv_epilogue_f32<NFRAG, MI>(p, acc, lane, n0, [&](int t) {
            const int m = m0 + t;
            return m < p.M ? m : -1;
        }, wave * WR);
    } else {
    conv_epilogue<NFRAG, MI, I8, LDS_BYTES>(p, acc, acci, smem, wave, lane, n0, [&](int t) {
        const int m = m0 + t;
        return m < p.M ? m : -1;
    }, wave * WR);
    }
    TRTX_MARK(3);
}

template <int NFRAG, int BKT, int TPS, bool I8 = false, int MI = 2, bool RS = false, bool UP = false, bool ONE = false, bool F32 = false, bool ROLES = false>
__global__ __launch_bounds__(kWaves * 64 * (ROLES ? 2 : 1)) void conv_igemm_f16_kernel(const ConvArgs p, unsigned in_bytes, unsigned w_bytes, int tiles_n,
                                                             int total_tiles, int xcd_chunk) {
    __shared__ __attribute__((aligned(16))) char smem[igemm_lds_bytes<NFRAG, BKT, MI, RS>()];
    int tile = blockIdx.x;
    if (xcd_chunk) {
        tile = (tile & 7) * xcd_chunk + (tile >> 3);
        if (tile >= total_tiles) return;
    }
    const int m0 = (tile / tiles_n) * (kWaves * 16 * MI);
    const int n0 = (tile % tiles_n) * (16 * NFRAG);
    conv_igemm_tile<NFRAG, BKT, TPS, I8, MI, RS, UP, ONE, F32, ROLES>(p, in_bytes, w_bytes, m0, n0, smem);
}

struct ConvGroupArgs {
    int n;
    int slot_start[kMaxConvGroup + 1];
    int chunk[kMaxConvGroup];
    int tiles[kMaxConvGroup];
    int tiles_n[kMaxConvGroup];
    unsigned in_bytes[kMaxConvGroup], w_bytes[kMaxConvGroup];
    ConvArgs p[kMaxConvGroup];
};
template <int NFRAG, int BKT, bool RS, bool ONE, bool I8 = false>
__global__ __launch_bounds__(256) void conv_igemm_group_f16_kernel(const ConvGroupArgs g) {
    __shared__ __attribute__((aligned(16))) char smem[igemm_lds_bytes<NFRAG, BKT, 2, RS>()];
    const int xcd = blockIdx.x & 7, slot = blockIdx.x >> 3;
    int pid = 0;
#pragma unroll
    for (int k = 1; k < kMaxConvGroup; ++k) pid += (k < g.n && slot >= g.slot_start[k]) ? 1 : 0;
    pid = __builtin_amdgcn_readfirstlane(pid);
    const int local = xcd * g.chunk[pid] + (slot - g.slot_start[pid]);
    if (local >= g.tiles[pid]) return;
    const int tn = g.tiles_n[pid];
    const int m0 = (local / tn) * 128;
    const int n0 = (local % tn) * (16 * NFRAG);
    conv_igemm_tile<NFRAG, BKT, 1, I8, 2, RS, false, ONE>(g.p[pid], g.in_bytes[pid], g.w_bytes[pid], m0, n0, smem);
}

}
}
```

### tensorrtx_amd/csrc/kernels/kernels.h

```cpp
#pragma once
#include <hip/hip_runtime.h>
#include <stddef.h>
#include <stdint.h>

namespace trtx {

enum Act : int { ACT_NONE = 0, ACT_RELU = 1, ACT_SIGMOID = 2, ACT_SILU = 3, ACT_LEAKY = 4, ACT_TANH = 5,
                 ACT_MISH = 6 ,
                 ACT_GELU_TANH = 7 ,
                 ACT_EXP = 8  };
enum DType : int { DT_F32 = 0, DT_F16 = 1, DT_I8 = 2 };
inline size_t dtype_size(int dt) { return dt == DT_F16 ? 2 : (dt == DT_I8 ? 1 : 4); }
enum EwOp : int { EW_SUM = 0, EW_PROD = 1, EW_MAX = 2, EW_MIN = 3, EW_SUB = 4, EW_DIV = 5, EW_POW = 6 };
enum PoolOp : int { POOL_MAX = 0, POOL_AVG = 1 };

enum Ws : int {
    WS_AUTO = 0,
    WS_OFF = 1,
    WS_ON = 2,
    WS_PATCH = 3,
    WS_F32_REGS = 5,
    WS_F32_ROLES = 6,
    WS_RES3 = 7,
    WS_RES1 = 8,
};
enum Wsk : int {
    WSK_RULE = 0,
    WSK_OFF = 1,
    WSK_ON = 2,
};

struct ConvArgs {
    const void* in;
    const void* wgt;
    const float* bias;
    void* out;
    const void* residual;
    int N, H, W, Cin, ld_in;
    int Ho, Wo, Cout, Cout_pad, ld_out, ld_res;
    int kh, kw, stride_h, stride_w, pad_h, pad_w, dil_h, dil_w, groups;
    int K, Kpad, M;
    int act1, act2;
    float alpha1, alpha2;
    int bn;
    int scalar_out;
    int CinK;
    int bk;
    int in_i8, out_i8, res_i8;
    const float* cscale;
    float out_inv_scale, res_scale;
    int bm;
    int t_wsk;
    int t_ws;
    int t_rs;
    const void* up_in;
    int up_C, up_ld, up_H, up_W;
    int f32;
    int k_pinned;
};

struct ConvTactic {
    int bn, bk, bm;
    int wsk, ws;
};

struct LaunchProbe {
    hipEvent_t start = nullptr, stop = nullptr;
    int launches = 0;
};
void conv_set_launch_probe(LaunchProbe* p);
LaunchProbe* conv_launch_probe();

int conv_igemm_pick_bn(int cout);
int conv_igemm_pick_bk(int cin, int taps);
int conv_igemm_pick_cink(int cin, int bk);
bool conv_igemm_supported(const ConvArgs& a);
void conv_pack_weights_i8(const float* w_kcrs, int cout, int cin, int kh, int kw, int cink, const float* ch_scale, int cout_pad, int kpad,
                          int8_t* packed, float* wscale_out);
int32_t conv_igemm_f16(const ConvArgs& a, hipStream_t s);
int conv_tactics(const ConvArgs& a, ConvTactic* out, int max_out, bool work_efficient_only = false);
void conv_apply_tactic(ConvArgs* a, const ConvTactic& t);
constexpr int kMaxConvGroup = 4;
bool conv_igemm_group_supported(const ConvArgs* a, int n);
int32_t conv_igemm_group_f16(const ConvArgs* a, int n, hipStream_t s);
bool conv_gemm256_possible(const ConvArgs& a);
bool conv_gemm256_worthwhile(const ConvArgs& a);
int32_t conv_gemm256_f16(const ConvArgs& a, hipStream_t s);
int conv_igemm_f32_pick_cink(int cin);
bool conv_igemm_f32_supported(const ConvArgs& a);
int32_t conv_igemm_f32(const ConvArgs& a, hipStream_t s);
int conv_tactics_f32(const ConvArgs& a, ConvTactic* out, int max_out);
void conv_pack_weights_igemm_f32(const float* w_kcrs, int cout, int cin, int kh, int kw, int cink, int kpad, int cout_pad, const float* ch_scale, float* packed);
bool conv_res_possible(const ConvArgs& a);
bool conv_res_group_possible(const ConvArgs* a, int n);
int32_t conv_res_f16(const ConvArgs* a, int n, hipStream_t s);
bool conv_res1_possible(const ConvArgs& a);
int32_t conv_res1_f16(const ConvArgs& a, hipStream_t s);
bool conv_ws_supported(const ConvArgs& a);
int32_t conv_ws_f16(const ConvArgs& a, hipStream_t s);
int32_t poison_lds(unsigned* device_word, hipStream_t s);
bool conv_stem_supported(const ConvArgs& a);
int32_t conv_stem_nchw_f32(const ConvArgs& a, hipStream_t s);
bool conv_stem_f32_supported(const ConvArgs& a);
int32_t conv_stem_nchw_f32_out_f32(const ConvArgs& a, hipStream_t s);
constexpr int kStemMaxFrames = 64;
struct StemFrame {
    const void* src;
    int w, h;
    float d2s[6];
};
int32_t conv_stem_frames_f32(const ConvArgs& a, const StemFrame* frames, hipStream_t s);
bool conv_stem_pair_possible(const ConvArgs& stem, const ConvArgs& conv);
int32_t conv_stem_pair_f16(const ConvArgs& stem, const ConvArgs& conv, hipStream_t s);
bool conv_bneck_pair_possible(const ConvArgs& first, const ConvArgs& second);
int32_t conv_bneck_pair_f16(const ConvArgs& first, const ConvArgs& second, hipStream_t s);
int32_t conv_bneck_pair_or_two_f16(const ConvArgs& first, const ConvArgs& second, hipStream_t s);
int32_t conv_direct(const ConvArgs& a, int dtype, hipStream_t s);
bool conv_dw_supported(const ConvArgs& a);
bool psa_attention_supported(int kd, int hd);
int32_t psa_attention_f16(const void* qkv, int ld_qkv, void* out, int ld_out, void* vimg, int ld_v, int B, int heads, int N, int kd, int hd,
                          float scale, hipStream_t s);
bool area_attention_supported(int kd, int hd);
int32_t area_attention_f16(const void* qkv, int ld_qkv, void* out, int ld_out, void* vimg, int ld_v, int B, int heads, int N, int area, int kd,
                           int hd, float scale, hipStream_t s);
bool area_attention_split_supported(int kd, int hd);
int32_t area_attention_split_f16(const void* q, int ld_q, const void* k, int ld_k, const void* v, int ld_v, void* out, int ld_out, int B, int heads, int N,
                                 int area, int kd, int hd, float scale, hipStream_t s);
int32_t conv_dw(const ConvArgs& a, int dtype, hipStream_t s);
struct HgconvWeights {
    const float* w_ctx;
    const float* b_ctx;
    const float* proto;
    const float* w_pre;
    const float* b_pre;
    const float* w_edge;
    const float* b_edge;
    const float* w_node;
    const float* b_node;
};
bool hgconv_supported(int D, int E);
size_t hgconv_workspace_bytes(int B, int N, int D, int E);
int hgconv_geometry(int32_t* tiles, int max_tiles);
int32_t hgconv_f16(const void* x, int ld_x, void* out, int ld_out, int B, int N, int D, int E, float logit_scale, const HgconvWeights& w, void* workspace,
                   size_t workspace_bytes, hipStream_t s);
bool conv_grouped_supported(const ConvArgs& a);
int conv_grouped_kpad(const ConvArgs& a);
int32_t conv_grouped(const ConvArgs& a, hipStream_t s);
int32_t deconv_direct(const ConvArgs& a, int dtype, hipStream_t s);

int32_t nchw_f32_to_nhwc(const float* in, void* out, int dtype, int N, int C, int H, int W, int Cpad, int ld_out,
                         hipStream_t s);
int32_t nhwc_to_nchw_f32(const void* in, int dtype, float* out, int N, int C, int H, int W, int ld_in, hipStream_t s);

int32_t nhwc_maxpool_chain3_f16(const void* in, void* o1, void* o2, void* o3, int N, int H, int W, int C, int ld_in, int ld1,
                                int ld2, int ld3, int k, hipStream_t s, int f32 = 0);
int32_t nhwc_depth_to_space_f16(const void* in, void* out, int N, int H, int W, int C, int bh, int bw, int ld_in, int ld_out,
                                hipStream_t s);
int32_t nhwc_pool(const void* in, void* out, int dtype, int op, int N, int H, int W, int C, int ld_in, int Ho, int Wo,
                  int ld_out, int kh, int kw, int sh, int sw, int ph, int pw, int avg_exclusive, hipStream_t s);
int32_t nhwc_resize_nearest(const void* in, void* out, int dtype, int N, int H, int W, int C, int ld_in, int Ho,
                            int Wo, int ld_out, hipStream_t s);
int32_t nhwc_zero_pad(const void* in, void* out, int dtype, int N, int H, int W, int C, int ld_in, int Ho, int Wo, int ld_out, int top,
                      int left, hipStream_t s);
int32_t nhwc_elementwise(const void* a, const void* b, void* out, int dtype, int op, long pixels, int C, int ld_a,
                         int ld_b, int ld_out, hipStream_t s);
int32_t nhwc_activation(const void* in, void* out, int dtype, int act, float alpha, long pixels, int C, int ld_in,
                        int ld_out, hipStream_t s);
int32_t nhwc_gated_add(const void* a, const void* b, const float* gate, void* out, int dtype, long pixels, int C, int ld_a, int ld_b, int ld_out,
                       hipStream_t s);
int32_t nhwc_scale(const void* in, void* out, int dtype, const float* scale, const float* shift, long pixels, int C,
                   int ld_in, int ld_out, hipStream_t s);
int32_t nhwc_copy(const void* in, void* out, int dtype, long pixels, int C, int ld_in, int ld_out, hipStream_t s);
int32_t nhwc_reduce_hw_avg(const void* in, void* out, int dtype, int N, int HW, int C, int ld_in, int ld_out,
                           hipStream_t s);

int32_t nhwc_absmax_f16(const void* x, long pixels, int C, int ld, unsigned* out_float_bits, hipStream_t s);
int32_t nhwc_hist_f16(const void* x, long pixels, int C, int ld, float range, unsigned long long* hist8192, hipStream_t s);
int32_t nhwc_resize_nearest_i8(const void* in, void* out, int N, int H, int W, int C, int ld_in, int Ho, int Wo, int ld_out, float ratio,
                               hipStream_t s);

struct StridedView {
    int rank;
    long shape[6];
    long stride_in[6];
    long stride_in2[6];
};
int32_t lin_gather(const float* in, float* out, const StridedView& v, hipStream_t s);
int32_t lin_scatter(const float* in, float* out, const StridedView& v, hipStream_t s);
int32_t lin_elementwise(const float* a, const float* b, float* out, int op, const StridedView& v, hipStream_t s);
int32_t lin_activation(const float* in, float* out, int act, float alpha, long n, hipStream_t s);
int32_t lin_softmax(const float* in, float* out, long outer, long axis, long inner, hipStream_t s);
int32_t lin_matmul(const float* A, const float* B, float* C, int batch, int M, int N, int K, int ta, int tb,
                   long bsA, long bsB, hipStream_t s, int binner = 1, long bsA2 = 0, long bsB2 = 0);
int32_t lin_reduce(const float* in, float* out, int op , long outer, long axis, long inner,
                   hipStream_t s);
int32_t lin_scale(const float* in, float* out, const float* scale, const float* shift, const float* power, int mode,
                  long outer, long C, long inner, hipStream_t s);

}
```

### tensorrtx_amd/csrc/ops_capi.cpp

```cpp
#include <hip/hip_runtime.h>
#include <stdlib.h>
#include <string.h>

#include <vector>

#include "common.h"
#include "options.h"
#include "kernels/kernels.h"
#include "runtime/pack.h"

using namespace trtx;

extern "C" const char* trtx_status_string(int32_t s) {
    switch (s) {
        case TRTX_OK: return "ok";
        case TRTX_ERR_INVALID: return "invalid argument";
        case TRTX_ERR_HIP: return "HIP error";
        case TRTX_ERR_WORKSPACE: return "workspace too small";
        case TRTX_ERR_UNSUPPORTED: return "unsupported configuration";
        case TRTX_ERR_NO_DEVICE: return "no HIP device";
        case TRTX_ERR_IO: return "I/O or parse error";
        case TRTX_ERR_STATE: return "invalid call order";
        default: return "unknown status";
    }
// ... 15 lines not shown
extern "C" int32_t trtx_conv_packed_dims(int cout, int cin_pad, int kh, int kw, int32_t* cout_pad, int32_t* kpad,
                                         int32_t* bn) {
    if (cout < 1 || cin_pad < 1 || kh < 1 || kw < 1) return TRTX_ERR_INVALID;
    const int b = conv_igemm_pick_bn(cout);
    if (bn) *bn = b;
    if (cout_pad) *cout_pad = (cout + b - 1) / b * b;
    if (kpad) {
        const int bk = conv_igemm_pick_bk(cin_pad, kh * kw);
        *kpad = (kh * kw * conv_igemm_pick_cink(cin_pad, bk) + bk - 1) / bk * bk;
    }
    return TRTX_OK;
}

extern "C" int32_t trtx_conv_pack_weights_f16(const float* w_kcrs, int cout, int cin, int kh, int kw, int cin_pad,
                                              const float* ch_scale, uint16_t* packed) {
    if (!w_kcrs || !packed || cin_pad < cin) return TRTX_ERR_INVALID;
    const int bk = conv_igemm_pick_bk(cin_pad, kh * kw);
    pack_conv_weights_f16(w_kcrs, cout, cin, kh, kw, conv_igemm_pick_cink(cin_pad, bk), bk, ch_scale, packed);
    return TRTX_OK;
}

static ConvArgs op_conv_args(int N, int H, int W, int Cin, int ld_in, int Cout, int ld_out, int kh, int kw, int sh, int sw, int ph, int pw,
                             int act1, int has_res, int ld_res, int act2) {
    ConvArgs a{};
    a.N = N; a.H = H; a.W = W; a.Cin = Cin; a.ld_in = ld_in;
    a.Ho = (H + 2 * ph - kh) / sh + 1;
    a.Wo = (W + 2 * pw - kw) / sw + 1;
    a.Cout = Cout;
    a.bn = conv_igemm_pick_bn(Cout);
    a.Cout_pad = (Cout + a.bn - 1) / a.bn * a.bn;
    a.ld_out = ld_out; a.ld_res = ld_res;
    a.kh = kh; a.kw = kw; a.stride_h = sh; a.stride_w = sw; a.pad_h = ph; a.pad_w = pw; a.dil_h = 1; a.dil_w = 1;
    a.groups = 1;
    a.bk = conv_igemm_pick_bk(Cin, kh * kw);
    a.CinK = conv_igemm_pick_cink(Cin, a.bk);
    a.K = kh * kw * a.CinK;
    a.Kpad = (a.K + a.bk - 1) / a.bk * a.bk;
    a.M = N * a.Ho * a.Wo;
    a.act1 = act1; a.act2 = act2; a.alpha1 = 0.1f; a.alpha2 = 0.1f;
    a.scalar_out = (Cout % 8 || ld_out % 8 || (has_res && ld_res % 8)) ? 1 : 0;
    return a;
}

static bool g_force_tactic = false;
static ConvTactic g_forced{};

extern "C" int32_t trtx_op_conv_force_tactic(const int32_t* t) {
    if (t && t[5] != 0) return TRTX_ERR_UNSUPPORTED;
    g_force_tactic = t != nullptr;
    if (t) g_forced = ConvTactic{t[0], t[1], t[2], t[3], t[4]};
    return TRTX_OK;
}

extern "C" int32_t trtx_op_conv2d_tactics(int N, int H, int W, int Cin, int ld_in, int Cout, int ld_out, int kh, int kw, int sh, int sw, int ph,
                                          int pw, int has_residual, int ld_res, int32_t* out6, int32_t max_out) {
    if (!out6 || max_out < 1 || N < 1 || kh < 1 || kw < 1 || sh < 1 || sw < 1) return 0;
    ConvArgs a = op_conv_args(N, H, W, Cin, ld_in, Cout, ld_out, kh, kw, sh, sw, ph, pw, 0, has_residual, ld_res, 0);
    a.residual = has_residual ? reinterpret_cast<const void*>(1) : nullptr;
    std::vector<ConvTactic> t(max_out);
    const int n = conv_tactics(a, t.data(), max_out);
    for (int i = 0; i < n; ++i) {
        out6[6 * i + 0] = t[i].bn; out6[6 * i + 1] = t[i].bk; out6[6 * i + 2] = t[i].bm; out6[6 * i + 3] = t[i].wsk; out6[6 * i + 4] = t[i].ws;
        out6[6 * i + 5] = 0;
    }
    return n;
}

extern "C" int32_t trtx_op_conv2d_nhwc_f16(const void* in, int N, int H, int W, int Cin, int ld_in, const void* wpacked,
                                           const float* bias, void* out, int Cout, int ld_out, int kh, int kw, int sh,
                                           int sw, int ph, int pw, int act1, const void* residual, int ld_res,
                                           int act2, trtx_stream_t stream) {
    ConvArgs a = op_conv_args(N, H, W, Cin, ld_in, Cout, ld_out, kh, kw, sh, sw, ph, pw, act1, residual != nullptr, ld_res, act2);
    a.in = in;
    a.wgt = wpacked;
    a.bias = bias;
    a.out = out;
    a.residual = residual;
    if (reinterpret_cast<uintptr_t>(out) & 15) a.scalar_out = 1;
    if (g_force_tactic) conv_apply_tactic(&a, g_forced);
    const int reps = options().op_reps;
    int32_t st = TRTX_OK;
    for (int r = 0; r < reps && st == TRTX_OK; ++r) st = conv_igemm_f16(a, stream);
    return st;
}

static ConvArgs op_stem_args(const float* in, int N, int C, int H, int W, const float* w_taps_cout, const float* bias, int Cout, int k, int stride, int pad, int act) {
    ConvArgs a{};
    a.in = in; a.wgt = w_taps_cout; a.bias = bias;
    a.N = N; a.H = H; a.W = W; a.Cin = C; a.ld_in = C;
    a.Ho = (H + 2 * pad - k) / stride + 1;
    a.Wo = (W + 2 * pad - k) / stride + 1;
    a.Cout = Cout; a.Cout_pad = Cout;
    a.kh = k; a.kw = k; a.stride_h = stride; a.stride_w = stride; a.pad_h = pad; a.pad_w = pad; a.dil_h = 1; a.dil_w = 1;
    a.groups = 1;
    a.K = k * k * C; a.Kpad = a.K;
    a.M = N * a.Ho * a.Wo;
    a.act1 = act; a.alpha1 = 0.1f; a.alpha2 = 0.1f;
    return a;
}

extern "C" int32_t trtx_op_conv_stem_nchw_f16(const float* in, int N, int C, int H, int W, const float* w_taps_cout, const float* bias, void* out, int Cout,
                                              int ld_out, int k, int stride, int pad, int act, trtx_stream_t stream) {
    if (!in || !w_taps_cout || !out || N < 1 || C < 1 || H < 1 || W < 1 || k < 1 || stride < 1 || pad < 0 || H + 2 * pad < k || W + 2 * pad < k) return TRTX_ERR_INVALID;
    ConvArgs a = op_stem_args(in, N, C, H, W, w_taps_cout, bias, Cout, k, stride, pad, act);
    a.out = out;
    a.ld_out = ld_out;
    return conv_stem_nchw_f32(a, static_cast<hipStream_t>(stream));
}

extern "C" int32_t trtx_op_conv_stem_pair_f16(const float* in, int N, int C, int H, int W, const float* stem_w_taps_cout, const float* stem_bias, int stem_act,
                                              const void* conv_wpacked, const float* conv_bias, int conv_act, void* out, int ld_out, trtx_stream_t stream) {
    if (!in || !stem_w_taps_cout || !conv_wpacked || !out || N < 1 || C < 1 || H < 1 || W < 1) return TRTX_ERR_INVALID;
    const ConvArgs s = op_stem_args(in, N, C, H, W, stem_w_taps_cout, stem_bias, 16, 3, 2, 1, stem_act);
    ConvArgs c = op_conv_args(N, s.Ho, s.Wo, 16, 16, 32, ld_out, 3, 3, 2, 2, 1, 1, conv_act, 0, 0, 0);
    c.wgt = conv_wpacked;
    c.bias = conv_bias;
    c.out = out;
    return conv_stem_pair_f16(s, c, static_cast<hipStream_t>(stream));
}

static int32_t op_bneck_pair(const void* in, int N, int H, int W, int ld_in, int in_coff, const void* w1_packed, const float* bias1, int act1, const void* w2_packed,
                             const float* bias2, int act2, int shortcut, int act_after, void* mid, void* out, int ld_out, bool or_two, trtx_stream_t stream) {
    if (!in || !w1_packed || !w2_packed || !out || N < 1 || H < 1 || W < 1 || ld_in < 16 || ld_in % 8 || in_coff < 0 || in_coff % 8 || in_coff + 16 > ld_in ||
        ld_out < 16 || ld_out % 8 || (or_two && !mid))
        return TRTX_ERR_INVALID;
    ConvArgs a = op_conv_args(N, H, W, 16, ld_in, 16, 16, 3, 3, 1, 1, 1, 1, act1, 0, 0, 0);
    ConvArgs b = op_conv_args(N, H, W, 16, 16, 16, ld_out, 3, 3, 1, 1, 1, 1, act2, shortcut ? 1 : 0, shortcut ? ld_in : 0, act_after);
    a.in = static_cast<const uint16_t*>(in) + in_coff;
    a.wgt = w1_packed;
    a.bias = bias1;
    a.out = mid;
    b.in = mid;
    b.wgt = w2_packed;
    b.bias = bias2;
    b.out = out;
    b.residual = shortcut ? a.in : nullptr;
    if (or_two) return conv_bneck_pair_or_two_f16(a, b, static_cast<hipStream_t>(stream));
    if (!conv_bneck_pair_possible(a, b)) return TRTX_ERR_INVALID;
    return conv_bneck_pair_f16(a, b, static_cast<hipStream_t>(stream));
}

extern "C" int32_t trtx_op_conv_bneck_pair_f16(const void* in, int N, int H, int W, int ld_in, int in_coff, const void* w1_packed, const float* bias1, int act1,
                                               const void* w2_packed, const float* bias2, int act2, int shortcut, int act_after, void* out, int ld_out,
                                               trtx_stream_t stream) {
    return op_bneck_pair(in, N, H, W, ld_in, in_coff, w1_packed, bias1, act1, w2_packed, bias2, act2, shortcut, act_after, nullptr, out, ld_out, false, stream);
}

extern "C" int32_t trtx_op_conv_bneck_pair_or_two_f16(const void* in, int N, int H, int W, int ld_in, int in_coff, const void* w1_packed, const float* bias1, int act1,
                                                      const void* w2_packed, const float* bias2, int act2, int shortcut, int act_after, void* mid, void* out,
                                                      int ld_out, trtx_stream_t stream) {
    return op_bneck_pair(in, N, H, W, ld_in, in_coff, w1_packed, bias1, act1, w2_packed, bias2, act2, shortcut, act_after, mid, out, ld_out, true, stream);
}

extern "C" int32_t trtx_conv_pack_weights_grouped_f16(const float* w_kcrs, int cout, int cin_g, int kh, int kw, const float* ch_scale, uint16_t* packed,
                                                      int32_t* kpad_out) {
    if (!w_kcrs || cout < 1 || cin_g < 1 || kh < 1 || kw < 1) return TRTX_ERR_INVALID;
    const int kpad = (kh * kw * cin_g + 31) / 32 * 32;
    if (kpad_out) *kpad_out = kpad;
    if (packed) pack_conv_weights_grouped_f16(w_kcrs, cout, cin_g, kh, kw, kpad, ch_scale, packed);
    return TRTX_OK;
}

extern "C" int32_t trtx_op_conv2d_grouped_nhwc_f16(const void* in, int N, int H, int W, int Cin, int ld_in, const void* wpacked, const float* bias, void* out,
                                                   int Cout, int ld_out, int groups, int k, int pad, int act1, const void* residual, int ld_res, int act2,
                                                   trtx_stream_t stream) {
    if (N < 1 || H < 1 || W < 1 || Cin < 1 || Cout < 1 || groups < 1 || k < 1 || pad < 0 || H + 2 * pad < k || W + 2 * pad < k) return TRTX_ERR_INVALID;
    ConvArgs a{};
    a.in = in; a.wgt = wpacked; a.bias = bias; a.out = out; a.residual = residual;
    a.N = N; a.H = H; a.W = W; a.Cin = Cin; a.ld_in = ld_in;
    a.Ho = H + 2 * pad - k + 1;
    a.Wo = W + 2 * pad - k + 1;
    a.Cout = Cout; a.Cout_pad = Cout; a.ld_out = ld_out; a.ld_res = ld_res;
    a.kh = k; a.kw = k; a.stride_h = 1; a.stride_w = 1; a.pad_h = pad; a.pad_w = pad; a.dil_h = 1; a.dil_w = 1;
    a.groups = groups;
    a.K = k * k * (Cin / groups);
    a.Kpad = conv_grouped_kpad(a);
    a.M = N * a.Ho * a.Wo;
    a.act1 = act1; a.act2 = act2; a.alpha1 = 0.1f; a.alpha2 = 0.1f;
    const int reps = options().op_reps;
    int32_t st = TRTX_OK;
    for (int r = 0; r < reps && st == TRTX_OK; ++r) st = conv_grouped(a, static_cast<hipStream_t>(stream));
    return st;
}

extern "C" int32_t trtx_op_conv2d_dw_nhwc(const void* in, int dtype, int N, int H, int W, int C, int ld_in, const float* w_taps_c, const float* bias, void* out,
                                          int ld_out, const void* residual, int ld_res, int k, int stride, int pad, int dilation, int act1, float alpha1,
                                          int act2, float alpha2, trtx_stream_t stream) {
    if (!in || !w_taps_c || !out || N < 1 || H < 1 || W < 1 || C < 1 || k < 1 || stride < 1 || pad < 0 || dilation < 1) return TRTX_ERR_INVALID;
    if (dtype != DT_F16 && dtype != DT_F32) return TRTX_ERR_UNSUPPORTED;
    if (H + 2 * pad < dilation * (k - 1) + 1 || W + 2 * pad < dilation * (k - 1) + 1) return TRTX_ERR_INVALID;
    ConvArgs a{};
    a.in = in; a.wgt = w_taps_c; a.bias = bias; a.out = out; a.residual = residual;
    a.N = N; a.H = H; a.W = W; a.Cin = C; a.ld_in = ld_in;
    a.Ho = (H + 2 * pad - dilation * (k - 1) - 1) / stride + 1;
    a.Wo = (W + 2 * pad - dilation * (k - 1) - 1) / stride + 1;
    a.Cout = C; a.Cout_pad = C; a.ld_out = ld_out; a.ld_res = ld_res;
    a.kh = k; a.kw = k; a.stride_h = stride; a.stride_w = stride; a.pad_h = pad; a.pad_w = pad; a.dil_h = dilation; a.dil_w = dilation;
    a.groups = C;
    a.K = k * k;
    a.Kpad = a.K;
    a.M = N * a.Ho * a.Wo;
    a.act1 = act1; a.act2 = act2; a.alpha1 = alpha1; a.alpha2 = alpha2;
    a.f32 = dtype == DT_F32;
    return conv_dw(a, dtype, static_cast<hipStream_t>(stream));
}

extern "C" int32_t trtx_op_psa_attention_f16(const void* qkv, int ld_qkv, void* out, int ld_out, void* vimg, int ld_v, int B, int heads, int N, int kd, int hd,
                                             float scale, trtx_stream_t stream) {
    if (!qkv || !out || !vimg) return TRTX_ERR_INVALID;
    return psa_attention_f16(qkv, ld_qkv, out, ld_out, vimg, ld_v, B, heads, N, kd, hd, scale, static_cast<hipStream_t>(stream));
}

extern "C" int32_t trtx_op_area_attention_f16(const void* qkv, int ld_qkv, void* out, int ld_out, void* vimg, int ld_v, int B, int heads, int N, int area,
                                              int kd, int hd, float scale, trtx_stream_t stream) {
    if (!qkv || !out || !vimg) return TRTX_ERR_INVALID;
    return area_attention_f16(qkv, ld_qkv, out, ld_out, vimg, ld_v, B, heads, N, area, kd, hd, scale, static_cast<hipStream_t>(stream));
}

extern "C" int32_t trtx_op_area_attention_split_f16(const void* q, int ld_q, const void* k, int ld_k, const void* v, int ld_v, void* out, int ld_out, int B,
                                                    int heads, int N, int area, int kd, int hd, float scale, trtx_stream_t stream) {
    if (!q || !k || !v || !out) return TRTX_ERR_INVALID;
    return area_attention_split_f16(q, ld_q, k, ld_k, v, ld_v, out, ld_out, B, heads, N, area, kd, hd, scale, static_cast<hipStream_t>(stream));
}

extern "C" size_t trtx_op_hgconv_workspace_bytes(int B, int N, int D, int E) { return hgconv_workspace_bytes(B, N, D, E); }

extern "C" int32_t trtx_op_hgconv_geometry(int32_t* tiles, int max_tiles, int32_t* n_tiles) {
    if (!tiles || !n_tiles || max_tiles < 1) return TRTX_ERR_INVALID;
    *n_tiles = hgconv_geometry(tiles, max_tiles);
    return TRTX_OK;
}

extern "C" int32_t trtx_op_hgconv_f16(const void* x, int ld_x, void* out, int ld_out, int B, int N, int D, int E, float logit_scale, const float* w_ctx,
                                      const float* b_ctx, const float* proto, const float* w_pre, const float* b_pre, const float* w_edge, const float* b_edge,
                                      const float* w_node, const float* b_node, void* workspace, size_t workspace_bytes, trtx_stream_t stream) {
    if (!x || !out || !w_ctx || !b_ctx || !proto || !w_pre || !b_pre || !w_edge || !b_edge || !w_node || !b_node || !workspace) return TRTX_ERR_INVALID;
    const HgconvWeights w{w_ctx, b_ctx, proto, w_pre, b_pre, w_edge, b_edge, w_node, b_node};
    return hgconv_f16(x, ld_x, out, ld_out, B, N, D, E, logit_scale, w, workspace, workspace_bytes, static_cast<hipStream_t>(stream));
}

static ConvArgs op_conv_args_f32(int N, int H, int W, int Cin, int ld_in, int Cout, int ld_out, int kh, int kw, int sh, int sw, int ph, int pw,
                                 int act1, int has_res, int ld_res, int act2) {
    ConvArgs a{};
    a.f32 = 1;
    a.N = N; a.H = H; a.W = W; a.Cin = Cin; a.ld_in = ld_in;
    a.Ho = (H + 2 * ph - kh) / sh + 1;
    a.Wo = (W + 2 * pw - kw) / sw + 1;
    a.Cout = Cout;
    a.Cout_pad = (Cout + 15) / 16 * 16;
    a.ld_out = ld_out; a.ld_res = ld_res;
    a.kh = kh; a.kw = kw; a.stride_h = sh; a.stride_w = sw; a.pad_h = ph; a.pad_w = pw; a.dil_h = 1; a.dil_w = 1;
    a.groups = 1;
    a.bk = 16;
    a.CinK = conv_igemm_f32_pick_cink(Cin);
    a.K = kh * kw * a.CinK;
    a.Kpad = (a.K + 15) / 16 * 16;
    a.M = N * a.Ho * a.Wo;
    a.act1 = act1; a.act2 = act2; a.alpha1 = 0.1f; a.alpha2 = 0.1f;
    a.scalar_out = (Cout % 4 || ld_out % 4 || (has_res && ld_res % 4)) ? 1 : 0;
    return a;
}

extern "C" int32_t trtx_conv_packed_dims_f32(int cout, int cin_pad, int kh, int kw, int32_t* cout_pad, int32_t* kpad, int32_t* cink) {
    if (cout < 1 || cin_pad < 1 || kh < 1 || kw < 1) return TRTX_ERR_INVALID;
    const int ck = conv_igemm_f32_pick_cink(cin_pad);
    if (cout_pad) *cout_pad = (cout + 15) / 16 * 16;
    if (kpad) *kpad = (kh * kw * ck + 15) / 16 * 16;
    if (cink) *cink = ck;
    return TRTX_OK;
}

extern "C" int32_t trtx_conv_pack_weights_f32(const float* w_kcrs, int cout, int cin, int kh, int kw, int cin_pad, const float* ch_scale, float* packed) {
    if (!w_kcrs || !packed || cin_pad < cin) return TRTX_ERR_INVALID;
    const int ck = conv_igemm_f32_pick_cink(cin_pad);
    conv_pack_weights_igemm_f32(w_kcrs, cout, cin, kh, kw, ck, (kh * kw * ck + 15) / 16 * 16, (cout + 15) / 16 * 16, ch_scale, packed);
    return TRTX_OK;
}

extern "C" int32_t trtx_op_conv2d_tactics_f32(int N, int H, int W, int Cin, int ld_in, int Cout, int ld_out, int kh, int kw, int sh, int sw, int ph,
                                              int pw, int has_residual, int ld_res, int32_t* out2, int32_t max_out) {
    if (!out2 || max_out < 1 || N < 1 || kh < 1 || kw < 1 || sh < 1 || sw < 1) return 0;
    ConvArgs a = op_conv_args_f32(N, H, W, Cin, ld_in, Cout, ld_out, kh, kw, sh, sw, ph, pw, 0, has_residual, ld_res, 0);
    a.residual = has_residual ? reinterpret_cast<const void*>(1) : nullptr;
    std::vector<ConvTactic> t(max_out);
    const int n = conv_tactics_f32(a, t.data(), max_out);
    for (int i = 0; i < n; ++i) {
        out2[4 * i + 0] = t[i].bn;
        out2[4 * i + 1] = t[i].bm;
        out2[4 * i + 2] = t[i].ws;
        out2[4 * i + 3] = t[i].bk;
    }
    return n;
}

extern "C" int32_t trtx_op_conv2d_nhwc_f32(const void* in, int N, int H, int W, int Cin, int ld_in, const void* wpacked, const float* bias, void* out,
                                           int Cout, int ld_out, int kh, int kw, int sh, int sw, int ph, int pw, int act1, const void* residual,
                                           int ld_res, int act2, const int32_t* tile2, trtx_stream_t stream) {
    ConvArgs a = op_conv_args_f32(N, H, W, Cin, ld_in, Cout, ld_out, kh, kw, sh, sw, ph, pw, act1, residual != nullptr, ld_res, act2);
    a.in = in;
    a.wgt = wpacked;
    a.bias = bias;
    a.out = out;
    a.residual = residual;
    if ((reinterpret_cast<uintptr_t>(out) & 15) || (residual && (reinterpret_cast<uintptr_t>(residual) & 15))) a.scalar_out = 1;
    if (tile2) {
        a.bn = tile2[0];
// ... 72 lines not shown
```

### tensorrtx_amd/csrc/options.cpp

```cpp
#include "options.h"

#include <stdlib.h>

namespace trtx {
namespace {
const char* env(const char* name) { return getenv(name); }
int env_int(const char* name, int unset) {
    const char* v = env(name);
    return (v && *v) ? atoi(v) : unset;
}
bool env_is(const char* name, int value) {
    const char* v = env(name);
    return v && *v && atoi(v) == value;
}
bool env_set(const char* name) { return env(name) != nullptr; }
}

Options read_options() {
    Options o;
    o.tune = env_int("TRTX_TUNE", -1);
    o.tune_verbose = env_set("TRTX_TUNE_VERBOSE");
    o.tune_margin = env_int("TRTX_TUNE_MARGIN", -1);
    if (const char* v = env("TRTX_TACTIC_CACHE")) o.tactic_cache = v;
    o.graph = env_is("TRTX_GRAPH", 1);
    if (const char* v = env("TRTX_CALIB_REPORT")) o.calib_report = v;
    if (const char* v = env("TRTX_INT8_CLIP_LIMIT"); v && *v) o.int8_clip_limit = atof(v);
    o.lanes = env_int("TRTX_LANES", 0);
    o.group_convs = !env_is("TRTX_GROUP_CONVS", 0);
    o.fold_upsample = !env_is("TRTX_FOLD_UPSAMPLE", 0);
    o.stem_pair = !env_is("TRTX_STEM_PAIR", 0);
    o.bneck_pair = !env_is("TRTX_BNECK_PAIR", 0);
    o.ws = !env_set("TRTX_CONV_NOWS");
    o.wsk = !env_set("TRTX_CONV_NOWSK");
    o.gemm256 = !env_is("TRTX_GEMM256", 0);
    o.patch = !env_is("TRTX_CONV_PATCH", 0);
    o.res = env_int("TRTX_CONV_RES", 7);
    o.roles = !env_is("TRTX_CONV_ROLES", 0);
    o.f32_mfma = !env_set("TRTX_F32_DIRECT");
    o.conv_grouped = !env_is("TRTX_CONV_GROUPED", 0);
    o.area_attention = !env_is("TRTX_AREA_ATTENTION", 0);
    o.aattn_split = !env_is("TRTX_AATTN_SPLIT", 0);
    o.hgconv = !env_is("TRTX_HGCONV", 0);
    o.gated_add = !env_is("TRTX_GATED_ADD", 0);
    o.yolo5_head = !env_is("TRTX_YOLO5_HEAD", 0);
    o.yolo7_head = !env_is("TRTX_YOLO7_HEAD", 0);
    o.darknet_head = !env_is("TRTX_DARKNET_HEAD", 0);
    o.reorg_fold = !env_is("TRTX_REORG_FOLD", 0);
    o.spp_parallel_chain = !env_is("TRTX_SPP_PARALLEL_CHAIN", 0);
    o.yolo9_head = !env_is("TRTX_YOLO9_HEAD", 0);
    o.roialign_fused = !env_set("TRTX_ROIALIGN_PLUGIN");
    o.roialign_fold_stride = !env_is("TRTX_ROIALIGN_FOLD_STRIDE", 0);
    o.profile_kernel_events = !env_set("TRTX_PROFILE_NO_KERNEL_EVENTS");
    o.op_reps = env_int("TRTX_OP_REPS", 1);
    return o;
}

const Options& options() {
    static const Options o = read_options();
    return o;
}

}
```

### tensorrtx_amd/csrc/options.h

```cpp
#pragma once
#include <string>

namespace trtx {

struct Options {
    int tune = -1;
    bool tune_verbose = false;
    int tune_margin = -1;
    std::string tactic_cache;
    bool graph = false;
    std::string calib_report;
    double int8_clip_limit = 1e-4;
    int lanes = 0;
    bool group_convs = true;
    bool fold_upsample = true;
    bool stem_pair = true;
    bool bneck_pair = true;
    bool ws = true;
    bool wsk = true;
    bool gemm256 = true;
    bool patch = true;
    int res = 7;
    bool roles = true;
    bool f32_mfma = true;
    bool conv_grouped = true;
    bool area_attention = true;
    bool aattn_split = true;
    bool hgconv = true;
    bool gated_add = true;
    bool yolo9_head = true;
    bool yolo5_head = true;
    bool yolo7_head = true;
    bool darknet_head = true;
    bool reorg_fold = true;
    bool spp_parallel_chain = true;
    bool roialign_fused = true;
    bool roialign_fold_stride = true;
    bool profile_kernel_events = true;
    int op_reps = 1;
};

Options read_options();
const Options& options();

}
```

### tensorrtx_amd/csrc/runtime/engine.cpp

```cpp
#include "engine.h"

#include <stdlib.h>
#include <string.h>

#include <sstream>

#include "../common.h"
#include "../options.h"
#include "int8.h"
#include "plugin.h"

using namespace trtx;

trtx_engine::~trtx_engine() {
    int left = plugins_initialized;
    for (auto& op : plan.ops)
        if (op.kind == OP_PLUGIN && left-- > 0 && op.plugin->v.terminate) op.plugin->v.terminate(op.plugin->v.self);
    if (d_weights) (void)hipFree(d_weights);
}

trtx_context::~trtx_context() {
    for (hipStream_t st : lane_stream)
        if (st) {
            (void)hipStreamSynchronize(st);
            (void)hipStreamDestroy(st);
        }
    for (hipEvent_t ev : op_event)
        if (ev) (void)hipEventDestroy(ev);
    for (hipEvent_t ev : lane_done)
        if (ev) (void)hipEventDestroy(ev);
    if (start_event) (void)hipEventDestroy(start_event);
    for (auto& g : graphs) {
        if (g.exec) (void)hipGraphExecDestroy(g.exec);
        if (g.graph) (void)hipGraphDestroy(g.graph);
    }
    if (d_arena) (void)hipFree(d_arena);
}

namespace trtx {

namespace {

struct Resolver {
    const Plan& plan;
    char* arena;
    char* weights;
    void* const* bindings;
    char* base(const PTensor& t) const {
        const Storage& s = plan.storages[t.storage];
        switch (s.kind) {
            case ST_ARENA: return arena + s.offset;
            case ST_WEIGHTS: return weights + s.offset;
            default: return static_cast<char*>(bindings[s.binding]);
        }
    }
    void* ptr(int tid) const {
        const PTensor& t = plan.tensors[tid];
        const size_t es = dtype_size(t.dtype);
        return base(t) + (t.layout == LAY_NHWC ? (size_t)t.rcoff : (size_t)t.reoff) * es;
    }
};

StridedView batch_view(const StridedView& v, int batch, long bs_in, long bs_in2) {
    StridedView o{};
    o.rank = v.rank + 1;
    o.shape[0] = batch;
    o.stride_in[0] = bs_in;
    o.stride_in2[0] = bs_in2;
    for (int d = 0; d < v.rank; ++d) {
        o.shape[d + 1] = v.shape[d];
        o.stride_in[d + 1] = v.stride_in[d];
        o.stride_in2[d + 1] = v.stride_in2[d];
    }
    return o;
}

}

int32_t execute_plan(trtx_context* c, int batch, void* const* bindings, hipStream_t stream,
                     std::vector<OpTiming>* prof) {
    trtx_engine* e = c->engine;
    const Plan& plan = e->plan;
    if (batch < 1 || batch > plan.max_batch) {
        fprintf(stderr, "[trtx_hip] enqueue: batch %d outside [1, %d]\n", batch, plan.max_batch);
        return TRTX_ERR_INVALID;
    }
    for (size_t b = 0; b < plan.binding_tensor.size(); ++b)
        if (!bindings[b] && !(c->frames && plan.binding_is_input[b])) {
            fprintf(stderr, "[trtx_hip] enqueue: binding %zu is null\n", b);
            return TRTX_ERR_INVALID;
        }
    Resolver R{plan, static_cast<char*>(c->d_arena), static_cast<char*>(e->d_weights), bindings};
    char* W = static_cast<char*>(e->d_weights);
    std::vector<hipEvent_t> evs;
    std::vector<LaunchProbe> probes;
    const bool no_probe = !options().profile_kernel_events;
    if (prof) {
        evs.resize(plan.ops.size() + 1);
        for (auto& ev : evs) TRTX_HIP_TRY(hipEventCreate(&ev));
        probes.resize(plan.ops.size());
        if (!no_probe && !c->tuning)
            for (size_t k = 0; k < plan.ops.size(); ++k)
                if ((plan.ops[k].kind == OP_CONV && plan.ops[k].igemm) || plan.ops[k].kind == OP_CONV_GROUP)
                    if (hipEventCreate(&probes[k].start) != hipSuccess || hipEventCreate(&probes[k].stop) != hipSuccess) (void)hipGetLastError();
        TRTX_HIP_TRY(hipEventRecord(evs[0], stream));
    }
    auto free_probes = [&]() {
        conv_set_launch_probe(nullptr);
        for (auto& pr : probes) {
            if (pr.start) (void)hipEventDestroy(pr.start);
            if (pr.stop) (void)hipEventDestroy(pr.stop);
        }
        probes.clear();
    };
    hipStream_t const user_stream = stream;
    const bool lanes = !prof && !c->observer && plan.num_lanes > 1;
    std::vector<char> lane_started(plan.num_lanes, 0);
    auto bail = [&](int32_t st) {
        (void)hipGetLastError();
        if (lanes)
            for (int l = 1; l < plan.num_lanes; ++l)
                if (lane_started[l] && hipEventRecord(c->lane_done[l], c->lane_stream[l]) == hipSuccess)
                    (void)hipStreamWaitEvent(user_stream, c->lane_done[l], 0);
        for (auto& ev : evs) (void)hipEventDestroy(ev);
        evs.clear();
        free_probes();
        return st;
    };
    if (lanes && hipEventRecord(c->start_event, user_stream) != hipSuccess) return bail(TRTX_ERR_HIP);
    ConvArgs pair_stem{};
    bool pair_pending = false;
    auto defers_to_next = [&](size_t k) {
        if (c->observer || c->tuning || k + 1 >= plan.ops.size()) return false;
        const POp &o = plan.ops[k], &nx = plan.ops[k + 1];
        return nx.bneck_pair && nx.kind == OP_CONV && o.kind == OP_CONV && o.igemm && nx.lane == o.lane && nx.in[0] == o.out[0];
    };
    for (size_t k = 0; k < plan.ops.size(); ++k) {
        const POp& op = plan.ops[k];
        hipStream_t stream = user_stream;
        if (lanes) {
            if (op.lane > 0) {
                stream = c->lane_stream[op.lane];
                if (!lane_started[op.lane]) {
                    if (hipStreamWaitEvent(stream, c->start_event, 0) != hipSuccess) return bail(TRTX_ERR_HIP);
                    lane_started[op.lane] = 1;
                }
            }
            for (int d : op.wait_ops)
                if (hipStreamWaitEvent(stream, c->op_event[d], 0) != hipSuccess) return bail(TRTX_ERR_HIP);
        }
        const PTensor& t0 = plan.tensors[op.in.empty() ? op.out[0] : op.in[0]];
        const PTensor& to = plan.tensors[op.out[0]];
        auto nb = [&](const PTensor& t) { return (t.nfix ? t.nfix : batch) * t.nmul; };
        int32_t st = TRTX_OK;
        const bool skip = c->tuning && (op.kind == OP_PLUGIN || op.kind == OP_YOLO_HEAD || op.kind == OP_YOLO_TASK_HEAD || op.kind == OP_YOLO5_HEAD || op.kind == OP_YOLO9_HEAD || op.kind == OP_YOLO7_HEAD || op.kind == OP_DARKNET_HEAD || op.kind == OP_ROI_ALIGN);
        if (!skip) switch (op.kind) {
            case OP_CONV:
            case OP_DECONV: {
                ConvArgs a = op.conv;
                a.in = R.ptr(op.in[0]);
                a.out = R.ptr(op.out[0]);
                a.residual = op.in.size() > 1 ? R.ptr(op.in[1]) : nullptr;
                a.up_in = op.extra_in.empty() ? nullptr : R.ptr(op.extra_in[0]);
                a.wgt = W + op.w_off;
                a.bias = reinterpret_cast<const float*>(W + op.b_off);
                a.cscale = a.in_i8 ? reinterpret_cast<const float*>(W + op.s_off) : nullptr;
                a.N = op.stem ? (plan.explicit_batch ? (int)t0.dims.d[0] : batch) : nb(t0);
                a.M = a.N * a.Ho * a.Wo;
                if (op.stem && !c->frames && !c->observer && !c->tuning && k + 1 < plan.ops.size() && plan.ops[k + 1].stem_pair && plan.ops[k + 1].lane == op.lane) {
                    const POp& nx = plan.ops[k + 1];
                    ConvArgs b = nx.conv;
                    b.out = R.ptr(nx.out[0]);
                    b.wgt = W + nx.w_off;
                    b.bias = reinterpret_cast<const float*>(W + nx.b_off);
                    b.N = nb(to);
                    b.M = b.N * b.Ho * b.Wo;
                    if (conv_stem_pair_possible(a, b)) {
                        pair_stem = a;
                        pair_pending = true;
                        break;
                    }
                }
                if (op.stem_pair && pair_pending) {
                    pair_pending = false;
                    if (prof && probes[k].start && probes[k].stop) conv_set_launch_probe(&probes[k]);
                    st = conv_stem_pair_f16(pair_stem, a, stream);
                    conv_set_launch_probe(nullptr);
                    break;
                }
                if (defers_to_next(k)) break;
                if (op.bneck_pair && k > 0 && defers_to_next(k - 1)) {
                    const POp& fo = plan.ops[k - 1];
                    ConvArgs f = fo.conv;
                    f.in = R.ptr(fo.in[0]);
                    f.out = R.ptr(fo.out[0]);
                    f.wgt = W + fo.w_off;
                    f.bias = reinterpret_cast<const float*>(W + fo.b_off);
                    f.N = nb(plan.tensors[fo.in[0]]);
                    f.M = f.N * f.Ho * f.Wo;
                    if (prof && probes[k].start && probes[k].stop) conv_set_launch_probe(&probes[k]);
                    st = conv_bneck_pair_or_two_f16(f, a, stream);
                    conv_set_launch_probe(nullptr);
                    break;
                }
                if (op.kind == OP_DECONV)
                    st = deconv_direct(a, op.dtype, stream);
                else if (op.stem && c->frames)
                    st = a.f32 ? TRTX_ERR_UNSUPPORTED : conv_stem_frames_f32(a, c->frames, stream);
                else if (op.stem)
                    st = a.f32 ? conv_stem_nchw_f32_out_f32(a, stream) : conv_stem_nchw_f32(a, stream);
                else if (op.igemm) {
                    if (prof && probes[k].start && probes[k].stop) conv_set_launch_probe(&probes[k]);
                    st = a.f32 ? conv_igemm_f32(a, stream) : conv_igemm_f16(a, stream);
                    conv_set_launch_probe(nullptr);
                } else if (op.dw)
                    st = conv_dw(a, op.dtype, stream);
                else if (op.grouped)
                    st = conv_grouped(a, stream);
                else
                    st = conv_direct(a, op.dtype, stream);
                break;
            }
            case OP_CONV_GROUP: {
                ConvArgs ga[kMaxConvGroup];
                const int gn = (int)op.group.size();
                if (gn < 2 || gn > kMaxConvGroup) { st = TRTX_ERR_STATE; break; }
                for (int m = 0; m < gn; ++m) {
                    const POp& mo = op.group[m];
                    ConvArgs& a = ga[m];
                    a = mo.conv;
                    a.in = R.ptr(mo.in[0]);
                    a.out = R.ptr(mo.out[0]);
                    a.residual = mo.in.size() > 1 ? R.ptr(mo.in[1]) : nullptr;
                    a.up_in = nullptr;
                    a.wgt = W + mo.w_off;
                    a.bias = reinterpret_cast<const float*>(W + mo.b_off);
                    a.cscale = a.in_i8 ? reinterpret_cast<const float*>(W + mo.s_off) : nullptr;
                    a.N = nb(plan.tensors[mo.in[0]]);
                    a.M = a.N * a.Ho * a.Wo;
                }
                if (prof && probes[k].start && probes[k].stop) conv_set_launch_probe(&probes[k]);
                st = conv_igemm_group_f16(ga, gn, stream);
                conv_set_launch_probe(nullptr);
                if (st == TRTX_ERR_UNSUPPORTED) {
                    st = TRTX_OK;
                    for (int m = 0; m < gn && st == TRTX_OK; ++m) st = conv_igemm_f16(ga[m], stream);
                }
                break;
            }
            case OP_POOL:
                st = nhwc_pool(R.ptr(op.in[0]), R.ptr(op.out[0]), op.dtype, op.i[0], nb(t0), t0.H, t0.W, t0.C, t0.ld, to.H,
                               to.W, to.ld, op.i[1], op.i[2], op.i[3], op.i[4], op.i[5], op.i[6], op.i[7], stream);
                break;
            case OP_POOL_CHAIN: {
                const PTensor &y1 = plan.tensors[op.out[0]], &y2 = plan.tensors[op.out[1]], &y3 = plan.tensors[op.out[2]];
                st = nhwc_maxpool_chain3_f16(R.ptr(op.in[0]), R.ptr(op.out[0]), R.ptr(op.out[1]), R.ptr(op.out[2]), nb(t0), t0.H,
                                             t0.W, t0.C, t0.ld, y1.ld, y2.ld, y3.ld, op.i[1], stream, op.dtype == DT_F32 ? 1 : 0);
                break;
            }
            case OP_D2S:
                st = nhwc_depth_to_space_f16(R.ptr(op.in[0]), R.ptr(op.out[0]), nb(t0), t0.H, t0.W, to.C, op.i[0], op.i[1], t0.ld,
                                             to.ld, stream);
                break;
            case OP_RESIZE:
                if (t0.dtype == DT_I8) {
                    st = nhwc_resize_nearest_i8(R.ptr(op.in[0]), R.ptr(op.out[0]), nb(t0), t0.H, t0.W, t0.C, t0.ld, to.H, to.W, to.ld,
                                                t0.scale / to.scale, stream);
                    break;
                }
                st = nhwc_resize_nearest(R.ptr(op.in[0]), R.ptr(op.out[0]), op.dtype, nb(t0), t0.H, t0.W, t0.C, t0.ld, to.H,
                                         to.W, to.ld, stream);
                break;
            case OP_EW_NHWC: {
                const PTensor& t1 = plan.tensors[op.in[1]];
                st = nhwc_elementwise(R.ptr(op.in[0]), R.ptr(op.in[1]), R.ptr(op.out[0]), op.dtype, op.i[0],
                                      (long)nb(t0) * t0.H * t0.W, t0.C, t0.ld, t1.ld, to.ld, stream);
                break;
            }
            case OP_GATED_ADD: {
                const PTensor& t1 = plan.tensors[op.in[1]];
                st = nhwc_gated_add(R.ptr(op.in[0]), R.ptr(op.in[1]), reinterpret_cast<const float*>(W + op.w_off), R.ptr(op.out[0]), op.dtype,
                                    (long)nb(t0) * t0.H * t0.W, t0.C, t0.ld, t1.ld, to.ld, stream);
                break;
            }
            case OP_ACT_NHWC:
                st = nhwc_activation(R.ptr(op.in[0]), R.ptr(op.out[0]), op.dtype, op.i[0], op.f[0],
                                     (long)nb(t0) * t0.H * t0.W, t0.C, t0.ld, to.ld, stream);
                break;
            case OP_SCALE_NHWC:
                st = nhwc_scale(R.ptr(op.in[0]), R.ptr(op.out[0]), op.dtype, reinterpret_cast<const float*>(W + op.s_off),
                                reinterpret_cast<const float*>(W + op.b_off), (long)nb(t0) * t0.H * t0.W, t0.C, t0.ld,
                                to.ld, stream);
                break;
            case OP_COPY_NHWC:
                st = nhwc_copy(R.ptr(op.in[0]), R.ptr(op.out[0]), op.dtype, (long)nb(t0) * t0.H * t0.W, t0.C, t0.ld, to.ld,
                               stream);
                break;
            case OP_REDUCE_HW:
                st = nhwc_reduce_hw_avg(R.ptr(op.in[0]), R.ptr(op.out[0]), op.dtype, nb(t0), t0.H * t0.W, t0.C, t0.ld, to.ld,
                                        stream);
                break;
            case OP_TO_NHWC:
                st = nchw_f32_to_nhwc(static_cast<const float*>(R.ptr(op.in[0])), R.ptr(op.out[0]), to.dtype, nb(to), to.C,
                                      to.H, to.W, to.Calloc ? to.Calloc : to.C, to.ld, stream);
                break;
            case OP_TO_LINEAR:
                st = nhwc_to_nchw_f32(R.ptr(op.in[0]), t0.dtype, static_cast<float*>(R.ptr(op.out[0])), nb(t0), t0.C, t0.H,
                                      t0.W, t0.ld, stream);
                break;
            case OP_GATHER: {
                const float* src = static_cast<const float*>(R.ptr(op.in[0])) + op.off0;
                const StridedView v = to.batched ? batch_view(op.view, batch, t0.batched ? t0.dims.volume() : 0, 0) : op.view;
                st = lin_gather(src, static_cast<float*>(R.ptr(op.out[0])), v, stream);
                break;
            }
            case OP_SCATTER: {
                float* dst = static_cast<float*>(R.ptr(op.out[0])) + op.off0;
                StridedView v = op.view;
                if (to.batched) {
                    if (!t0.batched) {
                        for (int b = 0; b < batch && st == TRTX_OK; ++b)
                            st = lin_scatter(static_cast<const float*>(R.ptr(op.in[0])), dst + (long)b * to.dims.volume(), v,
                                             stream);
                        break;
                    }
                    v = batch_view(op.view, batch, to.dims.volume(), 0);
                }
                st = lin_scatter(static_cast<const float*>(R.ptr(op.in[0])), dst, v, stream);
                break;
            }
            case OP_EW_LIN: {
                const PTensor& t1 = plan.tensors[op.in[1]];
                const StridedView v = to.batched ? batch_view(op.view, batch, t0.batched ? t0.dims.volume() : 0,
                                                              t1.batched ? t1.dims.volume() : 0)
                                                 : op.view;
                st = lin_elementwise(static_cast<const float*>(R.ptr(op.in[0])), static_cast<const float*>(R.ptr(op.in[1])),
                                     static_cast<float*>(R.ptr(op.out[0])), op.i[0], v, stream);
                break;
            }
            case OP_ACT_LIN:
                st = lin_activation(static_cast<const float*>(R.ptr(op.in[0])), static_cast<float*>(R.ptr(op.out[0])), op.i[0],
                                    op.f[0], (long)(to.batched ? batch : 1) * to.dims.volume(), stream);
                break;
            case OP_SCALE_LIN: {
                const long bmul = to.batched ? batch : 1;
                st = lin_scale(static_cast<const float*>(R.ptr(op.in[0])), static_cast<float*>(R.ptr(op.out[0])),
                               reinterpret_cast<const float*>(W + op.s_off), reinterpret_cast<const float*>(W + op.b_off),
                               reinterpret_cast<const float*>(W + op.w_off), op.i[0], bmul * op.i[1], op.i[2], op.i[3],
                               stream);
                break;
            }
            case OP_SOFTMAX:
                st = lin_softmax(static_cast<const float*>(R.ptr(op.in[0])), static_cast<float*>(R.ptr(op.out[0])),
                                 (long)(to.batched ? batch : 1) * op.i[0], op.i[1], op.i[2], stream);
                break;
            case OP_MATMUL: {
                const PTensor& t1 = plan.tensors[op.in[1]];
                if (op.view.rank > 0) {
                    const StridedView& v = op.view;
                    const long outer = v.rank == 2 ? v.shape[0] : 1, inner = v.shape[v.rank - 1];
                    st = lin_matmul(static_cast<const float*>(R.ptr(op.in[0])), static_cast<const float*>(R.ptr(op.in[1])),
                                    static_cast<float*>(R.ptr(op.out[0])), (int)(outer * inner), op.i[0], op.i[1], op.i[2], op.i[3], op.i[4],
                                    v.rank == 2 ? v.stride_in[0] : 0, v.rank == 2 ? v.stride_in2[0] : 0, stream, (int)inner,
                                    v.stride_in[v.rank - 1], v.stride_in2[v.rank - 1]);
                    break;
                }
                st = lin_matmul(static_cast<const float*>(R.ptr(op.in[0])), static_cast<const float*>(R.ptr(op.in[1])),
                                static_cast<float*>(R.ptr(op.out[0])), to.batched ? batch : 1, op.i[0], op.i[1], op.i[2],
                                op.i[3], op.i[4], t0.batched ? t0.dims.volume() : 0, t1.batched ? t1.dims.volume() : 0,
                                stream);
                break;
            }
            case OP_REDUCE_LIN:
                st = lin_reduce(static_cast<const float*>(R.ptr(op.in[0])), static_cast<float*>(R.ptr(op.out[0])), op.i[0],
                                (long)(to.batched ? batch : 1) * op.i[1], op.i[2], op.i[3], stream);
                break;
            case OP_PLUGIN: {
                std::vector<const void*> ins;
                std::vector<void*> outs;
                for (int t : op.in) ins.push_back(R.ptr(t));
                for (int t : op.out) outs.push_back(R.ptr(t));
                void* ws = op.ws_bytes ? static_cast<char*>(c->d_arena) + op.ws_off : nullptr;
                const int pb = plan.explicit_batch && op.i[0] > 0 ? op.i[0] : batch;
                const int rc = op.plugin->v.enqueue(op.plugin->v.self, pb, ins.data(), outs.data(), ws, stream);
                if (rc != 0) {
                    fprintf(stderr, "[trtx_hip] plugin %s enqueue returned %d\n", op.name.c_str(), rc);
                    st = TRTX_ERR_HIP;
                }
                break;
            }
            case OP_YOLO_HEAD: {
                const int nl = op.i[4];
// ... 487 lines not shown
```

### tensorrtx_amd/csrc/runtime/plan.cpp

```cpp
#include "plan.h"

#include <sstream>

namespace trtx {

const char* op_kind_name(int k) {
    static const char* n[] = {"conv",     "deconv",    "pool",      "resize",     "ew_nhwc", "act_nhwc", "scale_nhwc",
                              "copy_nhwc", "reduce_hw", "to_nhwc",   "to_linear",  "gather",  "scatter",  "ew_lin",
                              "act_lin",  "scale_lin", "softmax",   "matmul",     "reduce_lin", "plugin", "copy_lin", "yolo_head",
                              "pool_chain", "depth_to_space", "roi_align", "conv_chain", "conv_group", "attention",
                              "yolo_task_head", "yolo5_head", "yolo9_head", "yolo7_head", "hgconv", "gated_add", "attention_split",
                              "darknet_head", "pad_nhwc"};
    return (k >= 0 && k <= OP_PAD_NHWC) ? n[k] : "?";
}

std::string Plan::describe_json() const {
    std::ostringstream o;
    double flops = 0, bytes = 0;
    int n_conv = 0, n_igemm = 0;
    for (const auto& op : ops) {
        flops += op.flops;
        bytes += op.bytes;
        if (op.kind == OP_CONV) {
            ++n_conv;
            n_igemm += op.igemm ? 1 : 0;
        }
        n_conv += (int)op.group.size();
        n_igemm += (int)op.group.size();
    }
    o << "{\"fp16\":" << (fp16 ? "true" : "false") << ",\"max_batch\":" << max_batch << ",\"arena_bytes\":" << arena_bytes
      << ",\"weight_bytes\":" << weight_bytes << ",\"n_lanes\":" << num_lanes << ",\"n_ops\":" << ops.size() << ",\"n_conv\":" << n_conv
      << ",\"n_igemm\":" << n_igemm << ",\"flops_per_sample\":" << flops << ",\"bytes_per_sample\":" << bytes
      << ",\"ops\":[";
    for (size_t k = 0; k < ops.size(); ++k) {
        const POp& op = ops[k];
        o << (k ? "," : "") << "{\"kind\":\"" << op_kind_name(op.kind) << "\",\"name\":\"";
        for (char c : op.name) o << ((c == '"' || c == '\\' || (unsigned char)c < 0x20) ? ' ' : c);
        o << "\",\"flops\":" << op.flops << ",\"bytes\":" << op.bytes;
        auto conv_fields = [&](const POp& op) {
            const ConvArgs& a = op.conv;
            o << ",\"igemm\":" << (op.igemm ? "true" : "false") << ",\"stem\":" << (op.stem ? "true" : "false") << (op.stem_pair ? ",\"stem_pair\":true" : "")
              << (op.bneck_pair ? ",\"bneck_pair\":true" : "") << ",\"cin\":" << (a.in_i8 ? 2 * a.Cin : a.Cin) << ",\"cout\":" << a.Cout
              << ",\"k\":[" << a.kh << "," << a.kw << "],\"stride\":[" << a.stride_h << "," << a.stride_w << "],\"hw_in\":["
              << a.H << "," << a.W << "],\"hw_out\":[" << a.Ho << "," << a.Wo << "],\"act1\":" << a.act1
              << ",\"act2\":" << a.act2 << ",\"alpha1\":" << a.alpha1 << ",\"alpha2\":" << a.alpha2 << ",\"up_c\":" << a.up_C << ",\"residual\":" << (op.in.size() > 1 ? "true" : "false")
              << ",\"bn_folded\":" << (op.scale_layer >= 0 ? "true" : "false") << ",\"ld_in\":" << a.ld_in
              << ",\"ld_out\":" << a.ld_out << ",\"i8\":[" << a.in_i8 << "," << a.out_i8 << "," << a.res_i8 << "],\"nmul\":" << (op.stem ? 1 : tensors[op.in[0]].nmul) << ",\"nfix\":"
              << (op.stem ? 0 : tensors[op.in[0]].nfix);
            if (op.dw) o << ",\"dw\":true";
            if (op.grouped) o << ",\"grouped\":true";
            if (op.cout_real) o << ",\"cout_real\":" << op.cout_real;
            if (op.reorg_cin) o << ",\"reorg_cin\":" << op.reorg_cin;
        };
        if (op.kind == OP_CONV || op.kind == OP_DECONV) conv_fields(op);
        if (op.kind == OP_ACT_NHWC || op.kind == OP_ACT_LIN) o << ",\"act\":" << op.i[0];
        if (op.kind == OP_ATTENTION) o << ",\"heads\":" << op.i[0] << ",\"n\":" << op.i[1] << ",\"kd\":" << op.i[2] << ",\"hd\":" << op.i[3];
        if (op.kind == OP_ATTENTION && op.i[4] > 0) o << ",\"area\":" << op.i[4] << ",\"kernel\":\"mfma\"";
        if (op.kind == OP_ATTENTION_SPLIT)
            o << ",\"heads\":" << op.i[0] << ",\"n\":" << op.i[1] << ",\"kd\":" << op.i[2] << ",\"hd\":" << op.i[3] << ",\"area\":" << op.i[4] << ",\"k_offset\":" << op.i[5];
        if (op.kind == OP_HGCONV)
            o << ",\"n\":" << op.i[0] << ",\"d\":" << op.i[1] << ",\"e\":" << op.i[2] << ",\"logit_scale\":" << op.f[0] << ",\"ld\":[" << tensors[op.in[0]].ld << ","
              << tensors[op.out[0]].ld << "],\"ws_bytes\":" << op.ws_bytes;
        if (op.kind == OP_YOLO_TASK_HEAD) {
            o << ",\"task\":\"" << (op.i[9] == 1 ? "seg" : (op.i[9] == 2 ? "pose" : "obb")) << "\",\"classes\":" << op.i[0] << ",\"nk\":" << op.i[10]
              << ",\"branch_ld\":[";
            for (size_t j = 0; j < op.extra_in.size(); ++j) o << (j ? "," : "") << tensors[op.extra_in[j]].ld;
            o << "]";
        }
        if (op.kind == OP_POOL || op.kind == OP_POOL_CHAIN)
            o << ",\"k\":[" << op.i[1] << "," << op.i[2] << "],\"stride\":[" << op.i[3] << "," << op.i[4] << "],\"outputs\":" << op.out.size();
        if (op.kind == OP_PAD_NHWC) o << ",\"pre\":[" << op.i[0] << "," << op.i[1] << "]";
        if (op.kind == OP_YOLO5_HEAD || op.kind == OP_YOLO7_HEAD || op.kind == OP_DARKNET_HEAD) {
            o << ",\"classes\":" << op.i[0] << ",\"levels\":" << op.i[4] << ",\"anchor_levels\":" << op.fv.size() / 6 << ",\"grids\":[";
            for (int j = 0; j < op.i[4]; ++j) o << (j ? "," : "") << "[" << op.iv[2 * j] << "," << op.iv[2 * j + 1] << "]";
            o << "],\"ld\":[";
            for (size_t j = 0; j < op.in.size(); ++j) o << (j ? "," : "") << tensors[op.in[j]].ld;
            o << "]";
        }
        if (op.kind == OP_YOLO9_HEAD) {
            o << ",\"classes\":" << op.i[0] << ",\"levels\":" << op.i[4] << ",\"grids\":[";
            for (int j = 0; j < op.i[4]; ++j) o << (j ? "," : "") << "[" << op.i[2] / (8 << j) << "," << op.i[1] / (8 << j) << "]";
            o << "],\"strides\":[";
            for (int j = 0; j < op.i[4]; ++j) o << (j ? "," : "") << (8 << j);
            o << "],\"box_ld\":[";
            for (size_t j = 0; j < op.in.size(); ++j) o << (j ? "," : "") << tensors[op.in[j]].ld;
            o << "],\"cls_ld\":[";
            for (size_t j = 0; j < op.extra_in.size(); ++j) o << (j ? "," : "") << tensors[op.extra_in[j]].ld;
            o << "]";
        }
        if (op.kind == OP_CONV_GROUP) {
            o << ",\"members\":[";
            for (size_t j = 0; j < op.group.size(); ++j) {
                const POp& m = op.group[j];
                o << (j ? "," : "") << "{\"name\":\"";
                for (char c : m.name) o << ((c == '"' || c == '\\' || (unsigned char)c < 0x20) ? ' ' : c);
                o << "\",\"flops\":" << m.flops << ",\"bytes\":" << m.bytes;
                conv_fields(m);
                o << ",\"in\":[";
                for (size_t q = 0; q < m.in.size(); ++q) o << (q ? "," : "") << m.in[q];
                o << "],\"out\":[" << m.out[0] << "]}";
            }
            o << "]";
        }
        o << ",\"lane\":" << op.lane << ",\"waits\":[";
        for (size_t j = 0; j < op.wait_ops.size(); ++j) o << (j ? "," : "") << op.wait_ops[j];
        o << "],\"in\":[";
        for (size_t j = 0; j < op.in.size(); ++j) o << (j ? "," : "") << op.in[j];
        o << "],\"out\":[";
        for (size_t j = 0; j < op.out.size(); ++j) o << (j ? "," : "") << op.out[j];
        o << "]}";
    }
    o << "],\"tensors\":[";
    for (size_t k = 0; k < tensors.size(); ++k) {
        const PTensor& t = tensors[k];
        o << (k ? "," : "") << "{\"id\":" << t.id << ",\"net\":" << t.net_tensor << ",\"layout\":\""
          << (t.layout == LAY_NHWC ? "nhwc" : "linear") << "\",\"dims\":[";
        for (int d = 0; d < t.dims.nb; ++d) o << (d ? "," : "") << t.dims.d[d];
        o << "],\"storage\":" << t.storage << ",\"coff\":" << t.rcoff << ",\"ld\":" << t.ld << ",\"dtype\":" << t.dtype << ",\"scale\":" << t.scale
          << ",\"view\":"
          << (t.parent >= 0 ? "true" : "false") << "}";
    }
    o << "],\"storages\":[";
    for (size_t k = 0; k < storages.size(); ++k) {
        const Storage& s = storages[k];
        o << (k ? "," : "") << "{\"kind\":" << s.kind << ",\"bytes\":" << s.bytes << ",\"offset\":" << s.offset
          << ",\"first\":" << s.first_use << ",\"last\":" << s.last_use << "}";
    }
    o << "]}";
    return o.str();
}

}
```

### tensorrtx_amd/csrc/runtime/plan.h

```cpp
#pragma once
#include <memory>
#include <string>
#include <vector>

#include "../kernels/kernels.h"
#include "graph.h"
#include "plugin.h"

namespace trtx {

enum Layout : int { LAY_LINEAR = 0, LAY_NHWC = 1 };
enum StorageKind : int { ST_ARENA = 0, ST_WEIGHTS = 1, ST_BINDING = 2 };

enum OpKind : int {
    OP_CONV = 0,
    OP_DECONV,
    OP_POOL,
    OP_RESIZE,
    OP_EW_NHWC,
    OP_ACT_NHWC,
    OP_SCALE_NHWC,
    OP_COPY_NHWC,
    OP_REDUCE_HW,
    OP_TO_NHWC,
    OP_TO_LINEAR,
    OP_GATHER,
    OP_SCATTER,
    OP_EW_LIN,
    OP_ACT_LIN,
    OP_SCALE_LIN,
    OP_SOFTMAX,
    OP_MATMUL,
    OP_REDUCE_LIN,
    OP_PLUGIN,
    OP_COPY_LIN,
    OP_YOLO_HEAD,
    OP_POOL_CHAIN,
    OP_D2S,
    OP_ROI_ALIGN,
    OP_RESERVED_47,
    OP_CONV_GROUP,
    OP_ATTENTION,
    OP_YOLO_TASK_HEAD,
    OP_YOLO5_HEAD,
    OP_YOLO9_HEAD,
    OP_YOLO7_HEAD,
    OP_HGCONV,
    OP_GATED_ADD,
    OP_ATTENTION_SPLIT,
    OP_DARKNET_HEAD,
    OP_PAD_NHWC,
};
const char* op_kind_name(int k);

struct PTensor {
    int id = -1;
    int net_tensor = -1;
    std::string name;
    Dims dims;
    bool batched = true;
    int layout = LAY_LINEAR;
    int dtype = DT_F32;
    int nfix = 0;
    int nmul = 1;
    int C = 0, H = 0, W = 0;
    bool pad_zeroed = false;
    int parent = -1;
    int coff = 0;
    long eoff = 0;
    int ld = 0;
    int storage = -1;
    int rcoff = 0;
    long reoff = 0;
    int Calloc = 0;
    float scale = 0.f;
    long sample_elems() const { return layout == LAY_NHWC ? (long)nmul * H * W * ld : (long)dims.volume(); }
};

struct Storage {
    int kind = ST_ARENA;
    size_t bytes = 0;
    size_t offset = 0;
    int binding = -1;
    int first_use = 1 << 30, last_use = -1;
};
inline size_t align256(size_t v) { return (v + 255) / 256 * 256; }

struct POp {
    int kind = 0;
    std::string name;
    std::vector<int> in, out;
    std::vector<int> extra_in;
    int dtype = DT_F32;
    ConvArgs conv{};
    bool igemm = false;
    bool stem = false;
    bool stem_pair = false;
    bool bneck_pair = false;
    bool from_deconv = false;
    bool dw = false;
    bool grouped = false;
    int reorg_cin = 0;
    int cout_real = 0;
    std::vector<POp> group;
    int src_layer = -1;
    int scale_layer = -1;
    size_t w_off = 0, b_off = 0, s_off = 0;
    int i[12] = {0};
    float f[4] = {0};
    std::vector<int> iv;
    std::vector<float> fv;
    StridedView view{};
    long off0 = 0;
    bool view_batched_in = false, view_batched_in2 = false, view_batched_out = true;
    std::shared_ptr<PluginHolder> plugin;
    size_t ws_off = 0, ws_bytes = 0;
    int lane = 0;
    std::vector<int> wait_ops;
    bool signal = false;
    double flops = 0;
    double bytes = 0;
};

struct Plan {
    bool explicit_batch = false;
    bool fp16 = false;
    int max_batch = 1;
    std::vector<PTensor> tensors;
    std::vector<Storage> storages;
    std::vector<POp> ops;
    std::vector<int> binding_tensor;
    std::vector<int> binding_ptensor;
    std::vector<bool> binding_is_input;
    int num_lanes = 1;
    size_t arena_bytes = 0;
    size_t weight_bytes = 0;
    std::vector<uint8_t> weight_blob;
    std::string error;

    std::string describe_json() const;
};

bool lower_network(const Network& net, Plan* plan);
struct CalibrationLowering {
    CalibrationLowering();
    ~CalibrationLowering();
    static bool active();
};
bool pack_weights(const Network& net, Plan* plan);

}
```

### tensorrtx_amd/csrc/runtime/plan_passes.cpp

```cpp
#include "plan_passes.h"

#include <algorithm>

namespace trtx {
namespace {

bool fail(std::string* err, const std::string& m) {
    *err = m;
    return false;
}

size_t tensor_bytes(const Plan& plan, const PTensor& t) {
    const size_t es = dtype_size(t.dtype);
    if (t.layout == LAY_NHWC) {
        const size_t n = (t.nfix ? (size_t)t.nfix : (size_t)plan.max_batch) * (size_t)t.nmul;
        return n * t.H * t.W * (size_t)t.Calloc * es;
    }
    return (t.batched ? (size_t)plan.max_batch : 1) * (size_t)t.dims.volume() * es;
}

bool choose_conv_kernel(const Plan& plan, const PassInputs& e, POp& op) {
    ConvArgs& a = op.conv;
    const PTensor& ti = plan.tensors[op.in[0]];
    const PTensor& to = plan.tensors[op.out[0]];
// ... 540 lines not shown
            for (int m : mem) indep = indep && !anc.has(m, j) && !anc.has(j, m);
            if (!indep) continue;
            margs.push_back(args_at_max_batch(plan.ops[j]));
            std::vector<ConvArgs> trial = margs;
            int big = 0;
            for (size_t q = 1; q < trial.size(); ++q)
                if (trial[q].M > trial[big].M) big = (int)q;
            const int rs = trial[big].t_rs;
            for (ConvArgs& ma : trial) ma.t_rs = rs;
            if (!conv_igemm_group_supported(trial.data(), (int)trial.size())) {
                margs.pop_back();
                continue;
            }
            mem.push_back(j);
        }
        if (mem.size() < 2) continue;
        const int gi = (int)groups.size();
        groups.push_back(mem);
        for (int m : mem) group_of[m] = gi;
        if (!acyclic()) {
            for (int m : mem) group_of[m] = -1;
            groups.pop_back();
        }
    }
    if (groups.empty()) return;
    if (mark_only) {
        for (const auto& mem : groups)
            for (int m : mem) {
                plan.ops[m].conv.t_wsk = WSK_OFF;
                plan.ops[m].conv.k_pinned = 1;
            }
        return;
    }
    Contracted c = contract();
    const int nn = (int)c.first_op.size();
    std::vector<int>&indeg = c.indeg, &first_op = c.first_op;
    const std::vector<std::vector<int>>& succ = c.succ;
    std::vector<char> emitted(nn, 0);
    std::vector<POp> out;
    out.reserve(nn);
    for (int step = 0; step < nn; ++step) {
        int pick = -1;
        for (int v = 0; v < nn; ++v)
            if (!emitted[v] && indeg[v] == 0) { pick = v; break; }
        if (pick < 0) return;
        emitted[pick] = 1;
        for (int w : succ[pick]) --indeg[w];
        const int k0 = first_op[pick];
        if (group_of[k0] < 0) {
            out.push_back(plan.ops[k0]);
            continue;
        }
        POp g;
        g.kind = OP_CONV_GROUP;
        g.dtype = plan.ops[k0].dtype;
        g.conv = plan.ops[k0].conv;
        int big = groups[group_of[k0]][0];
        for (int m : groups[group_of[k0]])
            if ((long)plan.ops[m].conv.Ho * plan.ops[m].conv.Wo * plan.tensors[plan.ops[m].in[0]].nmul >
                (long)plan.ops[big].conv.Ho * plan.ops[big].conv.Wo * plan.tensors[plan.ops[big].in[0]].nmul)
                big = m;
        for (int m : groups[group_of[k0]]) {
            POp mo = plan.ops[m];
            mo.conv.t_rs = plan.ops[big].conv.t_rs;
            mo.conv.t_wsk = WSK_OFF;
            mo.conv.k_pinned = 1;
            g.group.push_back(mo);
            g.name += (g.name.empty() ? "" : " + ") + mo.name;
            for (int t : mo.in)
                if (std::find(g.in.begin(), g.in.end(), t) == g.in.end()) g.in.push_back(t);
            g.out.push_back(mo.out[0]);
            g.flops += mo.flops;
            g.bytes += mo.bytes;
        }
        g.name = "[group of " + std::to_string(g.group.size()) + "] " + g.name;
        out.push_back(std::move(g));
    }
    plan.ops = std::move(out);
}

void mark_stem_pair(Plan& plan, const PassInputs& e) {
    if (!e.opt.stem_pair || e.dt != DT_F16 || e.int8 || CalibrationLowering::active()) return;
    const int n = (int)plan.ops.size();
    for (int k = 0; k + 1 < n; ++k) {
        const POp& st = plan.ops[k];
        POp& cv = plan.ops[k + 1];
        if (st.kind != OP_CONV || !st.stem || st.conv.f32 || st.out.size() != 1) continue;
        if (cv.kind != OP_CONV || !cv.igemm || cv.stem || cv.from_deconv || cv.in.size() != 1 || !cv.extra_in.empty() || cv.in[0] != st.out[0]) continue;
        const PTensor& mid = plan.tensors[st.out[0]];
        if (mid.storage < 0 || plan.storages[mid.storage].kind != ST_ARENA || is_binding_tensor(plan, mid.id) || is_binding_tensor(plan, owner_of(plan, mid.id))) continue;
        bool shared = false;
        auto touches = [&](const POp& op) {
            for (const std::vector<int>* v : {&op.in, &op.out, &op.extra_in})
                for (int t : *v)
                    if (plan.tensors[t].storage == mid.storage) return true;
            return false;
        };
        for (int j = 0; j < n && !shared; ++j) {
            if (j == k || j == k + 1) continue;
            shared = touches(plan.ops[j]);
            for (const POp& m : plan.ops[j].group) shared = shared || touches(m);
        }
        if (shared) continue;
        ConvArgs a = st.conv, b = cv.conv;
        const PTensor& t_in = plan.tensors[st.in[0]];
        a.N = plan.explicit_batch ? (int)t_in.dims.d[0] : plan.max_batch;
        a.M = a.N * a.Ho * a.Wo;
        b.N = (mid.nfix ? mid.nfix : plan.max_batch) * mid.nmul;
        b.M = b.N * b.Ho * b.Wo;
        if (!conv_stem_pair_possible(a, b)) continue;
        cv.stem_pair = true;
    }
}

void mark_bneck_pair(Plan& plan, const PassInputs& e) {
    if (!e.opt.bneck_pair || e.dt != DT_F16 || e.int8 || CalibrationLowering::active()) return;
    const int n = (int)plan.ops.size();
    auto plain = [](const POp& op) { return op.kind == OP_CONV && op.igemm && !op.stem && !op.stem_pair && !op.bneck_pair && !op.from_deconv && op.extra_in.empty() && op.out.size() == 1; };
    for (int k = 0; k + 1 < n; ++k) {
        const POp& c0 = plan.ops[k];
        POp& c1 = plan.ops[k + 1];
        if (!plain(c0) || !plain(c1) || c0.in.size() != 1 || c1.in.empty() || c1.in.size() > 2 || c1.in[0] != c0.out[0]) continue;
        if (c1.in.size() == 2 && c1.in[1] != c0.in[0]) continue;
        const PTensor& mid = plan.tensors[c0.out[0]];
        if (mid.parent >= 0 || mid.storage < 0 || plan.storages[mid.storage].kind != ST_ARENA || is_binding_tensor(plan, mid.id)) continue;
        bool shared = false;
        auto touches = [&](const POp& op) {
            for (const std::vector<int>* v : {&op.in, &op.out, &op.extra_in})
                for (int t : *v)
                    if (plan.tensors[t].storage == mid.storage) return true;
            return false;
        };
        for (int j = 0; j < n && !shared; ++j) {
            if (j == k || j == k + 1) continue;
            shared = touches(plan.ops[j]);
            for (const POp& m : plan.ops[j].group) shared = shared || touches(m);
        }
        const PTensor &t_in = plan.tensors[c0.in[0]], &t_out = plan.tensors[c1.out[0]];
        if (shared || t_in.storage == mid.storage || t_out.storage == mid.storage) continue;
        if (t_in.layout != LAY_NHWC || t_out.layout != LAY_NHWC) continue;
        if (t_in.storage == t_out.storage && t_in.rcoff < t_out.rcoff + std::max(t_out.C, 1) && t_out.rcoff < t_in.rcoff + std::max(t_in.C, 1)) continue;
        ConvArgs a = c0.conv, b = c1.conv;
        a.N = (t_in.nfix ? t_in.nfix : plan.max_batch) * t_in.nmul;
        a.M = a.N * a.Ho * a.Wo;
        b.N = (mid.nfix ? mid.nfix : plan.max_batch) * mid.nmul;
        b.M = b.N * b.Ho * b.Wo;
        b.residual = c1.in.size() > 1 ? reinterpret_cast<const void*>(1) : nullptr;
        if (!conv_bneck_pair_possible(a, b)) continue;
        c1.bneck_pair = true;
        ++k;
    }
}

void assign_lanes(Plan& plan, const PassInputs& e, const std::vector<std::vector<int>>& deps) {
    const int nops = (int)plan.ops.size();
    int max_lanes = e.max_aux_streams >= 0 ? 1 + e.max_aux_streams : 4;
    if (e.opt.lanes > 0) max_lanes = std::max(1, std::min(16, e.opt.lanes));
    std::vector<int> tail(max_lanes, -1);
    plan.num_lanes = 1;
    for (int k = 0; k < nops; ++k) {
        int lane = -1;
        for (int d : deps[k])
            if (tail[plan.ops[d].lane] == d && (lane < 0 || d > tail[lane])) lane = plan.ops[d].lane;
        if (lane < 0 && deps[k].empty()) lane = 0;
        if (lane < 0) {
            for (int l = 0; l < max_lanes && lane < 0; ++l)
                if (tail[l] < 0) lane = l;
        }
        if (lane < 0) {
            lane = 0;
            for (int l = 1; l < max_lanes; ++l)
                if (tail[l] < tail[lane]) lane = l;
        }
        plan.ops[k].lane = lane;
        tail[lane] = k;
        plan.num_lanes = std::max(plan.num_lanes, lane + 1);
    }
    std::vector<std::vector<int>> covered(max_lanes, std::vector<int>(max_lanes, -1));
    for (int k = 0; k < nops; ++k) {
        POp& op = plan.ops[k];
        for (int d : deps[k]) {
            const int ld = plan.ops[d].lane;
            if (ld == op.lane || covered[op.lane][ld] >= d) continue;
            op.wait_ops.push_back(d);
            plan.ops[d].signal = true;
            covered[op.lane][ld] = d;
        }
    }
}

void plan_arena(Plan& plan, const Ancestors& anc) {
    const int nops = (int)plan.ops.size();
    auto before = [&](int a, int b) { return a == b || anc.has(a, b); };
    std::vector<std::vector<int>> touch(plan.storages.size());
    for (int k = 0; k < nops; ++k) {
        const POp& op = plan.ops[k];
        auto mark = [&](int t) {
            const int st = plan.tensors[t].storage;
            Storage& s = plan.storages[st];
            s.first_use = std::min(s.first_use, k);
            s.last_use = std::max(s.last_use, k);
            if (touch[st].empty() || touch[st].back() != k) touch[st].push_back(k);
        };
        for (int t : op.in) mark(t);
        for (int t : op.extra_in) mark(t);
        for (int t : op.out) mark(t);
        if (op.bneck_pair && k > 0)
            for (int t : plan.ops[k - 1].in) mark(t);
    }
    std::vector<std::pair<int, int>> ws_storage;
    for (int k = 0; k < nops; ++k) {
        const int kind = plan.ops[k].kind;
        if ((kind != OP_PLUGIN && kind != OP_YOLO_HEAD && kind != OP_YOLO_TASK_HEAD && kind != OP_YOLO5_HEAD && kind != OP_YOLO9_HEAD && kind != OP_YOLO7_HEAD && kind != OP_DARKNET_HEAD && kind != OP_HGCONV) || plan.ops[k].ws_bytes == 0) continue;
        Storage s;
        s.kind = ST_ARENA;
        s.bytes = plan.ops[k].ws_bytes;
        s.first_use = s.last_use = k;
        ws_storage.push_back({k, (int)plan.storages.size()});
        plan.storages.push_back(s);
        touch.push_back({k});
    }
    auto ordered = [&](int sa, int sb) {
        for (int x : touch[sa])
            for (int y : touch[sb])
                if (!before(x, y) || x == y) return false;
        return true;
    };
    std::vector<int> order;
    for (size_t si = 0; si < plan.storages.size(); ++si)
        if (plan.storages[si].kind == ST_ARENA && plan.storages[si].last_use >= 0) order.push_back((int)si);
    std::stable_sort(order.begin(), order.end(),
                     [&](int x, int y) { return plan.storages[x].first_use < plan.storages[y].first_use; });
    std::vector<int> placed;
    size_t arena = 0;
    for (int si : order) {
        Storage& st = plan.storages[si];
        const size_t need = align256(st.bytes);
        std::vector<std::pair<size_t, size_t>> busy;
        for (int pj : placed) {
            const Storage& o = plan.storages[pj];
            if (ordered(pj, si) || ordered(si, pj)) continue;
            busy.push_back({o.offset, o.offset + align256(o.bytes)});
        }
        std::sort(busy.begin(), busy.end());
        size_t off = 0;
        for (auto& bz : busy) {
            if (off + need <= bz.first) break;
            off = std::max(off, bz.second);
        }
        st.offset = off;
        arena = std::max(arena, off + need);
        placed.push_back(si);
    }
    plan.arena_bytes = arena;
    for (auto& w : ws_storage) plan.ops[w.first].ws_off = plan.storages[w.second].offset;
}

}

bool finalize_plan(Plan& plan, const PassInputs& e, std::string* err) {
    resolve_view_geometry(plan);
    fold_upsample(plan, e);
    assign_int8_served(plan, e);
    assign_storages(plan);
    if (!select_conv_kernels(plan, e, err) || !configure_plugins(plan, err)) return false;
    chain_sppf_pools(plan, e);
    chain_spp_parallel_pools(plan, e);
    group_convs(plan, e);
    mark_stem_pair(plan, e);
    mark_bneck_pair(plan, e);
    const std::vector<std::vector<int>> deps = op_dependencies(plan);
    assign_lanes(plan, e, deps);
    for (size_t k = 1; k < plan.ops.size(); ++k)
        if (plan.ops[k].bneck_pair && (plan.ops[k].lane != plan.ops[k - 1].lane || plan.ops[k - 1].signal)) plan.ops[k].bneck_pair = false;
    plan_arena(plan, ancestors(plan, deps, true));
    return true;
}

}
```

Measured before the change: 39400.

## Fuse sibling box/class head conv groups into one dual-output igemm kernel

Adds a plan pass that finds two grouped conv ops reading the same inputs, such as the YOLOv8 box (64-channel) and class (80-channel) head convs. It moves them next to each other and marks the second as a sibling pair. At runtime the pair launches a single dual-tile igemm kernel that loads each input tile once and accumulates both weight sets into separate accumulators, with separate epilogues. This is meant to remove a duplicate input read and a launch, at the cost of more registers and LDS per block and two pipeline stages instead of three. The pass only runs when the sibling_pair option is set and a single lane is configured.

```diff
diff --git a/include/trtx_hip.h b/include/trtx_hip.h
--- a/include/trtx_hip.h
+++ b/include/trtx_hip.h
@@ -195,6 +195,12 @@
 int32_t trtx_op_conv_bneck_pair_or_two_f16(const void* in, int N, int H, int W, int ld_in, int in_coff, const void* w1_packed, const float* bias1, int act1,
                                            const void* w2_packed, const float* bias2, int act2, int shortcut, int act_after, void* mid, void* out,
                                            int ld_out, trtx_stream_t stream);
+int32_t trtx_op_conv_dual_group_f16(int n, const void* const* in, const int32_t* geom, int k, int stride, int pad, const void* const* w0, const float* const* bias0,
+                                    void* const* out0, const int32_t* side0, const void* const* w1, const float* const* bias1, void* const* out1,
+                                    const int32_t* side1, const void* const* res1, int ld_res1, int i8_1, trtx_stream_t stream);
+int32_t trtx_op_conv_dual_group_or_two_f16(int n, const void* const* in, const int32_t* geom, int k, int stride, int pad, const void* const* w0,
+                                           const float* const* bias0, void* const* out0, const int32_t* side0, const void* const* w1, const float* const* bias1,
+                                           void* const* out1, const int32_t* side1, const void* const* res1, int ld_res1, int i8_1, trtx_stream_t stream);
 int32_t trtx_reorg_fold_weights(const float* w_kcrs, int cout, int cin, int kh, int kw, float* folded);
 int32_t trtx_conv_packed_dims_f32(int cout, int cin_pad, int kh, int kw, int32_t* cout_pad, int32_t* kpad, int32_t* cink);
 int32_t trtx_conv_pack_weights_f32(const float* w_kcrs, int cout, int cin, int kh, int kw, int cin_pad, const float* ch_scale, float* packed);
diff --git a/tensorrtx_amd/capi.py b/tensorrtx_amd/capi.py
--- a/tensorrtx_amd/capi.py
+++ b/tensorrtx_amd/capi.py
@@ -507,6 +507,23 @@
     return out
 
 
+def conv_dual_group_f16(xs, w0, b0, outs0, w1, b1, outs1, k=3, stride=1, pad=1, act0="silu", act1="silu", cout0=None, cout1=None, res1=None, i8_1=False,
+                        or_two=False, status_only=False):
+    import torch
+    n = len(xs)
+    A = lambda seq: None if seq is None else (ctypes.c_void_p * n)(*[t.data_ptr() if t is not None else None for t in seq])
+    geom = (ctypes.c_int32 * (5 * n))(*[v for x in xs for v in (x.shape[0], x.shape[1], x.shape[2], x.shape[3], x.stride(2))])
+    side = lambda outs, couts, act: (ctypes.c_int32 * (3 * n))(*[v for j, o in enumerate(outs) for v in (couts[j] if couts else o.shape[-1], o.stride(2), ACT[act])])
+    assert all(t.dtype == torch.float16 and t.stride(3) == 1 for t in list(xs) + list(outs0) + list(outs1))
+    fn = lib().trtx_op_conv_dual_group_or_two_f16 if or_two else lib().trtx_op_conv_dual_group_f16
+    st = fn(n, A(xs), geom, k, stride, pad, A(w0), A(b0), A(outs0), side(outs0, cout0, act0), A(w1), A(b1), A(outs1), side(outs1, cout1, act1),
+            A(res1), res1[0].stride(2) if res1 is not None else 0, 1 if i8_1 else 0, _stream())
+    if status_only:
+        return st
+    check(st, "trtx_op_conv_dual_group_f16")
+    return outs0, outs1
+
+
 def pack_conv_weights_grouped_f16(w_kcrs, ch_scale=None):
     import numpy as np
     L = lib()
diff --git a/tensorrtx_amd/csrc/kernels/conv_igemm.hip b/tensorrtx_amd/csrc/kernels/conv_igemm.hip
--- a/tensorrtx_amd/csrc/kernels/conv_igemm.hip
+++ b/tensorrtx_amd/csrc/kernels/conv_igemm.hip
@@ -633,4 +633,88 @@
     return check_launch("conv_igemm_group_f16");
 }
 
-}
+namespace {
+bool slices_overlap(const void* pa, long rows_a, int ld_a, int c_a, const void* pb, long rows_b, int ld_b, int c_b) {
+    if (!pa || !pb || rows_a < 1 || rows_b < 1) return false;
+    const uintptr_t a0 = reinterpret_cast<uintptr_t>(pa), a1 = a0 + (((size_t)rows_a - 1) * ld_a + c_a) * 2;
+    const uintptr_t b0 = reinterpret_cast<uintptr_t>(pb), b1 = b0 + (((size_t)rows_b - 1) * ld_b + c_b) * 2;
+    if (a1 <= b0 || b1 <= a0) return false;
+    if (ld_a != ld_b) return true;
+    const size_t row = (size_t)ld_a * 2;
+    const size_t d = b0 >= a0 ? (b0 - a0) % row : (row - (a0 - b0) % row) % row;
+    return !(d >= (size_t)c_a * 2 && d + (size_t)c_b * 2 <= row);
+}
+bool dual_member_ok(const ConvArgs& a, int bn) {
+    return group_member_ok(a) && !a.in_i8 && !a.residual && a.bn == bn && a.Cout_pad == bn && a.t_ws != WS_RES3 && a.t_ws != WS_RES1 &&
+           !(a.t_ws != WS_OFF && conv_ws_supported(a));
+}
+int32_t dual_group_refusal(const ConvArgs* a0, const ConvArgs* a1, int n) {
+    if (n < 1 || n > kMaxDualGroup) return TRTX_ERR_UNSUPPORTED;
+    for (int k = 0; k < n; ++k) {
+        const ConvArgs &x = a0[k], &y = a1[k];
+        if (!dual_member_ok(x, 64) || !dual_member_ok(y, 80)) return TRTX_ERR_UNSUPPORTED;
+        if (x.in != y.in || x.N != y.N || x.H != y.H || x.W != y.W || x.Cin != y.Cin || x.CinK != y.CinK || x.ld_in != y.ld_in || x.Ho != y.Ho || x.Wo != y.Wo ||
+            x.kh != y.kh || x.kw != y.kw || x.stride_h != y.stride_h || x.stride_w != y.stride_w || x.pad_h != y.pad_h || x.pad_w != y.pad_w || x.Kpad != y.Kpad)
+            return TRTX_ERR_UNSUPPORTED;
+    }
+    for (int k = 0; k < 2 * n; ++k) {
+        const ConvArgs& o = k < n ? a0[k] : a1[k - n];
+        const long rows_o = (long)o.N * o.Ho * o.Wo;
+        for (int j = 0; j < n; ++j)
+            if (slices_overlap(o.out, rows_o, o.ld_out, o.Cout, a0[j].in, (long)a0[j].N * a0[j].H * a0[j].W, a0[j].ld_in, a0[j].Cin)) return TRTX_ERR_INVALID;
+        for (int j = k + 1; j < 2 * n; ++j) {
+            const ConvArgs& u = j < n ? a0[j] : a1[j - n];
+            if (slices_overlap(o.out, rows_o, o.ld_out, o.Cout, u.out, (long)u.N * u.Ho * u.Wo, u.ld_out, u.Cout)) return TRTX_ERR_INVALID;
+        }
+    }
+    return TRTX_OK;
+}
+}
+
+bool conv_dual_group_possible(const ConvArgs* a0, const ConvArgs* a1, int n) { return dual_group_refusal(a0, a1, n) == TRTX_OK; }
+
+int32_t conv_dual_group_f16(const ConvArgs* a0, const ConvArgs* a1, int n, hipStream_t s) {
+    const int32_t why = dual_group_refusal(a0, a1, n);
+    if (why != TRTX_OK) return why;
+    ConvDualGroupArgs g{};
+    static_assert(sizeof(ConvDualGroupArgs) < 2048, "kernel arguments stay well under 4 KB");
+    g.n = n;
+    int order[kMaxDualGroup];
+    for (int k = 0; k < n; ++k) order[k] = k;
+    std::sort(order, order + n, [&](int x, int y) {
+        if (a0[x].Kpad != a0[y].Kpad) return a0[x].Kpad > a0[y].Kpad;
+        const long mx = (long)a0[x].N * a0[x].Ho * a0[x].Wo, my = (long)a0[y].N * a0[y].Ho * a0[y].Wo;
+        return mx != my ? mx > my : x < y;
+    });
+    int slots = 0;
+    for (int k = 0; k < n; ++k) {
+        const ConvArgs &x = a0[order[k]], &y = a1[order[k]];
+        g.p[k] = x;
+        g.p[k].M = x.N * x.Ho * x.Wo;
+        g.q[k] = ConvDualSide{y.wgt, y.bias, y.out, y.Cout, y.Cout_pad, y.ld_out, y.act1, y.act2, y.alpha1, y.alpha2, (unsigned)((size_t)y.Cout_pad * y.Kpad * 2)};
+        g.tiles[k] = (g.p[k].M + 127) / 128;
+        g.chunk[k] = (g.tiles[k] + 7) / 8;
+        g.slot_start[k] = slots;
+        slots += g.chunk[k];
+        g.in_bytes[k] = (unsigned)((((size_t)x.N * x.H * x.W - 1) * x.ld_in + x.Cin) * 2);
+        g.w_bytes[k] = (unsigned)((size_t)x.Cout_pad * x.Kpad * 2);
+    }
+    for (int k = n; k <= kMaxDualGroup; ++k) g.slot_start[k] = slots;
+    TRTX_LAUNCH((conv_igemm_dual_group_f16_kernel<4, 5>), dim3(slots * 8), dim3(256), 0, s, g);
+    return check_launch("conv_dual_group_f16");
+}
+
+int32_t conv_dual_group_or_two_f16(const ConvArgs* a0, const ConvArgs* a1, int n, hipStream_t s) {
+    if (conv_dual_group_possible(a0, a1, n)) return conv_dual_group_f16(a0, a1, n, s);
+    for (const ConvArgs* a : {a0, a1}) {
+        int32_t st = n >= 2 ? conv_igemm_group_f16(a, n, s) : TRTX_ERR_UNSUPPORTED;
+        if (st == TRTX_ERR_UNSUPPORTED) {
+            st = TRTX_OK;
+            for (int k = 0; k < n && st == TRTX_OK; ++k) st = conv_igemm_f16(a[k], s);
+        }
+        if (st != TRTX_OK) return st;
+    }
+    return TRTX_OK;
+}
+
+}
diff --git a/tensorrtx_amd/csrc/kernels/igemm_tile.h b/tensorrtx_amd/csrc/kernels/igemm_tile.h
--- a/tensorrtx_amd/csrc/kernels/igemm_tile.h
+++ b/tensorrtx_amd/csrc/kernels/igemm_tile.h
@@ -311,20 +311,25 @@
     }
 }
 
-template <int NFRAG, int BKT, int MI, bool RS>
+template <int NFRAG, int BKT, int MI, bool RS, int NF1 = 0, int STAGES = 0>
 constexpr int igemm_lds_bytes() {
-    constexpr int BN = 16 * NFRAG, BM = kWaves * 16 * MI, ROW_B = BKT * 2, CH = BKT / 8, RPI = 64 / CH;
+    constexpr int BN = 16 * (NFRAG + NF1), BM = kWaves * 16 * MI, ROW_B = BKT * 2, CH = BKT / 8, RPI = 64 / CH;
     constexpr int B_PASSES = (BN + kWaves * RPI - 1) / (kWaves * RPI), B_ROWS = B_PASSES * kWaves * RPI;
     constexpr int STAGE_BYTES = BM * ROW_B + B_ROWS * ROW_B;
-    constexpr int NST = RS ? 2 : (BKT == 64 ? 2 : 3);
-    constexpr int EPI_BYTES = kWaves * 16 * (16 * NFRAG * 4 + 16);
+    constexpr int NST = STAGES ? STAGES : (RS ? 2 : (BKT == 64 ? 2 : 3));
+    constexpr int EPI_BYTES = kWaves * 16 * (16 * (NFRAG > NF1 ? NFRAG : NF1) * 4 + 16);
     return NST * STAGE_BYTES > EPI_BYTES ? NST * STAGE_BYTES : EPI_BYTES;
 }
 
-template <int NFRAG, int BKT, int TPS, bool I8 = false, int MI = 2, bool RS = false, bool UP = false, bool ONE = false, bool F32 = false, bool ROLES = false>
-__device__ __forceinline__ void conv_igemm_tile(const ConvArgs& p, unsigned in_bytes, unsigned w_bytes, const int m0, const int n0, char* __restrict__ smem) {
+template <int NFRAG, int BKT, int TPS, bool I8 = false, int MI = 2, bool RS = false, bool UP = false, bool ONE = false, bool F32 = false, bool ROLES = false,
+          int NF1 = 0, int STAGES = 0>
+__device__ __forceinline__ void conv_igemm_tile(const ConvArgs& p, unsigned in_bytes, unsigned w_bytes, const int m0, const int n0, char* __restrict__ smem,
+                                                const ConvArgs* p1 = nullptr, unsigned w1_bytes = 0) {
     TRTX_MARK(0);
-    constexpr int BN = 16 * NFRAG;
+    constexpr bool DUAL = NF1 > 0;
+    constexpr int BN = 16 * (NFRAG + NF1);
+    static_assert(!DUAL || (BKT == 32 && TPS == 1 && !I8 && !RS && !UP && !ONE && !F32 && !ROLES && (16 * NFRAG) % (kWaves * 16) == 0),
+                  "dual tile: fp16, 32-wide k-steps, LDS-DMA operands, the seam on a DMA pass boundary");
     constexpr int BM = kWaves * 16 * MI;
     constexpr int WR = 16 * MI;
     constexpr int ROW_B = BKT * 2;
@@ -337,10 +342,10 @@
     constexpr int STAGE_BYTES = A_BYTES + B_ROWS * ROW_B;
     constexpr int LOADS_PER_TILE = A_LOADS + B_PASSES;
     constexpr int KSUB = BKT / 32;
-    constexpr int NST = RS ? 2 : (BKT == 64 ? 2 : 3);
-    constexpr int EPI_BYTES = kWaves * 16 * (16 * NFRAG * 4 + 16);
+    constexpr int NST = STAGES ? STAGES : (RS ? 2 : (BKT == 64 ? 2 : 3));
+    constexpr int EPI_BYTES = kWaves * 16 * (16 * (NFRAG > NF1 ? NFRAG : NF1) * 4 + 16);
     constexpr int LDS_BYTES = NST * STAGE_BYTES > EPI_BYTES ? NST * STAGE_BYTES : EPI_BYTES;
-    static_assert(LDS_BYTES == igemm_lds_bytes<NFRAG, BKT, MI, RS>(), "the entry points allocate what the tile function uses");
+    static_assert(LDS_BYTES == igemm_lds_bytes<NFRAG, BKT, MI, RS, NF1, STAGES>(), "the entry points allocate what the tile function uses");
 
     const int tid = threadIdx.x;
     const int lane = tid & 63;
@@ -351,6 +356,7 @@
 
     const __amdgpu_buffer_rsrc_t rs_in = __builtin_amdgcn_make_buffer_rsrc(const_cast<void*>(p.in), 0, in_bytes, 0x00020000);
     const __amdgpu_buffer_rsrc_t rs_w = __builtin_amdgcn_make_buffer_rsrc(const_cast<void*>(p.wgt), 0, w_bytes, 0x00020000);
+    const __amdgpu_buffer_rsrc_t rs_w1 = DUAL ? __builtin_amdgcn_make_buffer_rsrc(const_cast<void*>(p1->wgt), 0, w1_bytes, 0x00020000) : rs_w;
     const unsigned up_bytes = UP ? (unsigned)((((size_t)p.N * p.up_H * p.up_W - 1) * p.up_ld + p.up_C) * 2) : 0u;
     const __amdgpu_buffer_rsrc_t rs_up = UP ? __builtin_amdgcn_make_buffer_rsrc(const_cast<void*>(p.up_in), 0, up_bytes, 0x00020000) : rs_in;
 
@@ -392,6 +398,8 @@
     for (int j = 0; j < B_PASSES; ++j) {
         const int row = (kWaves * j + wave) * RPI + lrow;
         b_off[j] = row < BN ? (unsigned)(((n0 + row) * p.Kpad + lchunk * 8) * 2) : kOOB;
+        if constexpr (DUAL)
+            if (row >= 16 * NFRAG && row < BN) b_off[j] = (unsigned)(((row - 16 * NFRAG) * p.Kpad + lchunk * 8) * 2);
     }
     constexpr bool B_PARTIAL = !RS && (BN % (kWaves * RPI) != 0);
     const bool b_last_live = !B_PARTIAL || (kWaves * (B_PASSES - 1) + wave) * RPI < BN;
@@ -486,6 +494,8 @@
             if (B_PARTIAL && j == B_PASSES - 1 && !b_last_live) continue;
             const unsigned voff = ONE ? b_off[j] : (s_kt < nk ? b_off[j] : kOOB);
             if constexpr (RS) rb[j] = __builtin_amdgcn_raw_buffer_load_b128(rs_w, voff, 0, 0);
+            else if (DUAL && j * kWaves * RPI >= 16 * NFRAG)
+                __builtin_amdgcn_raw_ptr_buffer_load_lds(rs_w1, (lds_ptr_t)(sbase + A_BYTES + (kWaves * j + wave) * RPI * ROW_B), 16, voff, 0, 0, 0);
             else __builtin_amdgcn_raw_ptr_buffer_load_lds(rs_w, (lds_ptr_t)(sbase + A_BYTES + (kWaves * j + wave) * RPI * ROW_B), 16, voff, 0, 0, 0);
             b_off[j] += BKT * 2;
         }
@@ -513,14 +523,18 @@
     floatx4 acc[MI][NFRAG];
     intx4 acci[MI][NFRAG];
     floatx4 part[F32 ? MI : 1][F32 ? NFRAG : 1];
-#pragma unroll
-    for (int i = 0; i < MI; ++i)
+    floatx4 acc1[MI][DUAL ? NF1 : 1];
+#pragma unroll
+    for (int i = 0; i < MI; ++i) {
 #pragma unroll
         for (int j = 0; j < NFRAG; ++j) {
             acc[i][j] = floatx4{0.f, 0.f, 0.f, 0.f};
             acci[i][j] = intx4{0, 0, 0, 0};
             if constexpr (F32) part[i][j] = floatx4{0.f, 0.f, 0.f, 0.f};
         }
+#pragma unroll
+        for (int j = 0; j < (DUAL ? NF1 : 1); ++j) acc1[i][j] = floatx4{0.f, 0.f, 0.f, 0.f};
+    }
     if constexpr (F32) {
         if (p.bias) {
 #pragma unroll
@@ -590,6 +604,14 @@
                     const half8 bf = *reinterpret_cast<const half8*>(sb + b_frag + j * 16 * ROW_B + f_off[h]);
 #pragma unroll
                     for (int i = 0; i < MI; ++i) acc[i][j] = __builtin_amdgcn_mfma_f32_16x16x32_f16(bf, af[i], acc[i][j], 0, 0, 0);
+                }
+                if constexpr (DUAL) {
+#pragma unroll
+                    for (int j = 0; j < NF1; ++j) {
+                        const half8 bf = *reinterpret_cast<const half8*>(sb + b_frag + (NFRAG + j) * 16 * ROW_B + f_off[h]);
+#pragma unroll
+                        for (int i = 0; i < MI; ++i) acc1[i][j] = __builtin_amdgcn_mfma_f32_16x16x32_f16(bf, af[i], acc1[i][j], 0, 0, 0);
+                    }
                 }
             }
         }
@@ -690,6 +712,13 @@
         const int m = m0 + t;
         return m < p.M ? m : -1;
     }, wave * WR);
+    if constexpr (DUAL) {
+        intx4 acci_b[MI][NF1];
+        conv_epilogue<NF1, MI, false, LDS_BYTES>(*p1, acc1, acci_b, smem, wave, lane, 0, [&](int t) {
+            const int m = m0 + t;
+            return m < p.M ? m : -1;
+        }, wave * WR);
+    }
     }
     TRTX_MARK(3);
 }
@@ -733,5 +762,41 @@
     conv_igemm_tile<NFRAG, BKT, 1, I8, 2, RS, false, ONE>(g.p[pid], g.in_bytes[pid], g.w_bytes[pid], m0, n0, smem);
 }
 
-}
-}
+struct ConvDualSide {
+    const void* wgt;
+    const float* bias;
+    void* out;
+    int Cout, Cout_pad, ld_out, act1, act2;
+    float alpha1, alpha2;
+    unsigned w_bytes;
+};
+struct ConvDualGroupArgs {
+    int n;
+    int slot_start[kMaxDualGroup + 1];
+    int chunk[kMaxDualGroup], tiles[kMaxDualGroup];
+    unsigned in_bytes[kMaxDualGroup], w_bytes[kMaxDualGroup];
+    ConvArgs p[kMaxDualGroup];
+    ConvDualSide q[kMaxDualGroup];
+};
+constexpr int kDualStages = 2;
+template <int NF0, int NF1>
+__global__ __launch_bounds__(256) void conv_igemm_dual_group_f16_kernel(const ConvDualGroupArgs g) {
+    __shared__ __attribute__((aligned(16))) char smem[igemm_lds_bytes<NF0, 32, 2, false, NF1, kDualStages>()];
+    const int xcd = blockIdx.x & 7, slot = blockIdx.x >> 3;
+    int pid = 0;
+#pragma unroll
+    for (int k = 1; k < kMaxDualGroup; ++k) pid += (k < g.n && slot >= g.slot_start[k]) ? 1 : 0;
+    pid = __builtin_amdgcn_readfirstlane(pid);
+    const int local = xcd * g.chunk[pid] + (slot - g.slot_start[pid]);
+    if (local >= g.tiles[pid]) return;
+    const ConvDualSide& s1 = g.q[pid];
+    ConvArgs p1 = g.p[pid];
+    p1.wgt = s1.wgt; p1.bias = s1.bias; p1.out = s1.out;
+    p1.Cout = s1.Cout; p1.Cout_pad = s1.Cout_pad; p1.ld_out = s1.ld_out;
+    p1.act1 = s1.act1; p1.act2 = s1.act2; p1.alpha1 = s1.alpha1; p1.alpha2 = s1.alpha2;
+    conv_igemm_tile<NF0, 32, 1, false, 2, false, false, false, false, false, NF1, kDualStages>(g.p[pid], g.in_bytes[pid], g.w_bytes[pid], local * 128, 0, smem, &p1,
+                                                                                                s1.w_bytes);
+}
+
+}
+}
diff --git a/tensorrtx_amd/csrc/kernels/kernels.h b/tensorrtx_amd/csrc/kernels/kernels.h
--- a/tensorrtx_amd/csrc/kernels/kernels.h
+++ b/tensorrtx_amd/csrc/kernels/kernels.h
@@ -83,6 +83,10 @@
 constexpr int kMaxConvGroup = 4;
 bool conv_igemm_group_supported(const ConvArgs* a, int n);
 int32_t conv_igemm_group_f16(const ConvArgs* a, int n, hipStream_t s);
+constexpr int kMaxDualGroup = 3;
+bool conv_dual_group_possible(const ConvArgs* a0, const ConvArgs* a1, int n);
+int32_t conv_dual_group_f16(const ConvArgs* a0, const ConvArgs* a1, int n, hipStream_t s);
+int32_t conv_dual_group_or_two_f16(const ConvArgs* a0, const ConvArgs* a1, int n, hipStream_t s);
 bool conv_gemm256_possible(const ConvArgs& a);
 bool conv_gemm256_worthwhile(const ConvArgs& a);
 int32_t conv_gemm256_f16(const ConvArgs& a, hipStream_t s);
diff --git a/tensorrtx_amd/csrc/ops_capi.cpp b/tensorrtx_amd/csrc/ops_capi.cpp
--- a/tensorrtx_amd/csrc/ops_capi.cpp
+++ b/tensorrtx_amd/csrc/ops_capi.cpp
@@ -191,6 +191,42 @@
     return op_bneck_pair(in, N, H, W, ld_in, in_coff, w1_packed, bias1, act1, w2_packed, bias2, act2, shortcut, act_after, mid, out, ld_out, true, stream);
 }
 
+static int32_t op_dual_group(int n, const void* const* in, const int32_t* geom, int k, int stride, int pad, const void* const* w0, const float* const* bias0,
+                             void* const* out0, const int32_t* side0, const void* const* w1, const float* const* bias1, void* const* out1, const int32_t* side1,
+                             const void* const* res1, int ld_res1, int i8_1, bool or_two, trtx_stream_t stream) {
+    if (n < 1 || n > kMaxDualGroup || !in || !geom || !w0 || !out0 || !side0 || !w1 || !out1 || !side1 || k < 1 || stride < 1 || pad < 0) return TRTX_ERR_INVALID;
+    ConvArgs a0[kMaxDualGroup], a1[kMaxDualGroup];
+    for (int j = 0; j < n; ++j) {
+        const int32_t *g = geom + 5 * j, *s0 = side0 + 3 * j, *s1 = side1 + 3 * j;
+        if (!in[j] || !w0[j] || !out0[j] || !w1[j] || !out1[j] || g[0] < 1 || g[1] + 2 * pad < k || g[2] + 2 * pad < k || g[3] < 1) return TRTX_ERR_INVALID;
+        const void* r1 = res1 ? res1[j] : nullptr;
+        a0[j] = op_conv_args(g[0], g[1], g[2], g[3], g[4], s0[0], s0[1], k, k, stride, stride, pad, pad, s0[2], 0, 0, 0);
+        a1[j] = op_conv_args(g[0], g[1], g[2], g[3], g[4], s1[0], s1[1], k, k, stride, stride, pad, pad, s1[2], r1 != nullptr, ld_res1, 0);
+        a0[j].in = a1[j].in = in[j];
+        a0[j].wgt = w0[j]; a0[j].bias = bias0 ? bias0[j] : nullptr; a0[j].out = out0[j];
+        a1[j].wgt = w1[j]; a1[j].bias = bias1 ? bias1[j] : nullptr; a1[j].out = out1[j];
+        a1[j].residual = r1;
+        a1[j].in_i8 = i8_1 ? 1 : 0;
+        a0[j].t_wsk = a1[j].t_wsk = WSK_OFF;
+        a0[j].t_ws = a1[j].t_ws = WS_OFF;
+        a0[j].k_pinned = a1[j].k_pinned = 1;
+    }
+    return or_two ? conv_dual_group_or_two_f16(a0, a1, n, static_cast<hipStream_t>(stream)) : conv_dual_group_f16(a0, a1, n, static_cast<hipStream_t>(stream));
+}
+
+extern "C" int32_t trtx_op_conv_dual_group_f16(int n, const void* const* in, const int32_t* geom, int k, int stride, int pad, const void* const* w0,
+                                               const float* const* bias0, void* const* out0, const int32_t* side0, const void* const* w1, const float* const* bias1,
+                                               void* const* out1, const int32_t* side1, const void* const* res1, int ld_res1, int i8_1, trtx_stream_t stream) {
+    return op_dual_group(n, in, geom, k, stride, pad, w0, bias0, out0, side0, w1, bias1, out1, side1, res1, ld_res1, i8_1, false, stream);
+}
+
+extern "C" int32_t trtx_op_conv_dual_group_or_two_f16(int n, const void* const* in, const int32_t* geom, int k, int stride, int pad, const void* const* w0,
+                                                      const float* const* bias0, void* const* out0, const int32_t* side0, const void* const* w1,
+                                                      const float* const* bias1, void* const* out1, const int32_t* side1, const void* const* res1, int ld_res1, int i8_1,
+                                                      trtx_stream_t stream) {
+    return op_dual_group(n, in, geom, k, stride, pad, w0, bias0, out0, side0, w1, bias1, out1, side1, res1, ld_res1, i8_1, true, stream);
+}
+
 extern "C" int32_t trtx_conv_pack_weights_grouped_f16(const float* w_kcrs, int cout, int cin_g, int kh, int kw, const float* ch_scale, uint16_t* packed,
                                                       int32_t* kpad_out) {
     if (!w_kcrs || cout < 1 || cin_g < 1 || kh < 1 || kw < 1) return TRTX_ERR_INVALID;
diff --git a/tensorrtx_amd/csrc/options.cpp b/tensorrtx_amd/csrc/options.cpp
--- a/tensorrtx_amd/csrc/options.cpp
+++ b/tensorrtx_amd/csrc/options.cpp
@@ -30,6 +30,7 @@
     o.fold_upsample = !env_is("TRTX_FOLD_UPSAMPLE", 0);
     o.stem_pair = !env_is("TRTX_STEM_PAIR", 0);
     o.bneck_pair = !env_is("TRTX_BNECK_PAIR", 0);
+    o.sibling_pair = !env_is("TRTX_SIBLING_PAIR", 0);
     o.ws = !env_set("TRTX_CONV_NOWS");
     o.wsk = !env_set("TRTX_CONV_NOWSK");
     o.gemm256 = !env_is("TRTX_GEMM256", 0);
diff --git a/tensorrtx_amd/csrc/options.h b/tensorrtx_amd/csrc/options.h
--- a/tensorrtx_amd/csrc/options.h
+++ b/tensorrtx_amd/csrc/options.h
@@ -16,6 +16,7 @@
     bool fold_upsample = true;
     bool stem_pair = true;
     bool bneck_pair = true;
+    bool sibling_pair = true;
     bool ws = true;
     bool wsk = true;
     bool gemm256 = true;
diff --git a/tensorrtx_amd/csrc/runtime/engine.cpp b/tensorrtx_amd/csrc/runtime/engine.cpp
--- a/tensorrtx_amd/csrc/runtime/engine.cpp
+++ b/tensorrtx_amd/csrc/runtime/engine.cpp
@@ -134,6 +134,11 @@
         if (c->observer || c->tuning || k + 1 >= plan.ops.size()) return false;
         const POp &o = plan.ops[k], &nx = plan.ops[k + 1];
         return nx.bneck_pair && nx.kind == OP_CONV && o.kind == OP_CONV && o.igemm && nx.lane == o.lane && nx.in[0] == o.out[0];
+    };
+    auto group_defers_to_next = [&](size_t k) {
+        if (c->observer || c->tuning || c->frames || k + 1 >= plan.ops.size()) return false;
+        const POp &o = plan.ops[k], &nx = plan.ops[k + 1];
+        return nx.sibling_pair && nx.kind == OP_CONV_GROUP && o.kind == OP_CONV_GROUP && nx.lane == o.lane && nx.group.size() == o.group.size();
     };
     for (size_t k = 0; k < plan.ops.size(); ++k) {
         const POp& op = plan.ops[k];
@@ -225,9 +230,8 @@
                 ConvArgs ga[kMaxConvGroup];
                 const int gn = (int)op.group.size();
                 if (gn < 2 || gn > kMaxConvGroup) { st = TRTX_ERR_STATE; break; }
-                for (int m = 0; m < gn; ++m) {
-                    const POp& mo = op.group[m];
-                    ConvArgs& a = ga[m];
+                if (group_defers_to_next(k)) break;
+                auto member_args = [&](const POp& mo, ConvArgs& a) {
                     a = mo.conv;
                     a.in = R.ptr(mo.in[0]);
                     a.out = R.ptr(mo.out[0]);
@@ -238,6 +242,25 @@
                     a.cscale = a.in_i8 ? reinterpret_cast<const float*>(W + mo.s_off) : nullptr;
                     a.N = nb(plan.tensors[mo.in[0]]);
                     a.M = a.N * a.Ho * a.Wo;
+                };
+                for (int m = 0; m < gn; ++m) member_args(op.group[m], ga[m]);
+                if (op.sibling_pair && k > 0 && group_defers_to_next(k - 1)) {
+                    const POp& fo = plan.ops[k - 1];
+                    ConvArgs fa[kMaxConvGroup], sa[kMaxConvGroup];
+                    bool paired = true;
+                    for (int m = 0; m < gn; ++m) {
+                        member_args(fo.group[m], fa[m]);
+                        int q = 0;
+                        while (q < gn && op.group[q].in[0] != fo.group[m].in[0]) ++q;
+                        if (q == gn) { paired = false; break; }
+                        sa[m] = ga[q];
+                    }
+                    if (!paired) { st = TRTX_ERR_STATE; break; }
+                    const bool first64 = fa[0].bn == 64;
+                    if (prof && probes[k].start && probes[k].stop) conv_set_launch_probe(&probes[k]);
+                    st = conv_dual_group_or_two_f16(first64 ? fa : sa, first64 ? sa : fa, gn, stream);
+                    conv_set_launch_probe(nullptr);
+                    break;
                 }
                 if (prof && probes[k].start && probes[k].stop) conv_set_launch_probe(&probes[k]);
                 st = conv_igemm_group_f16(ga, gn, stream);
diff --git a/tensorrtx_amd/csrc/runtime/plan.cpp b/tensorrtx_amd/csrc/runtime/plan.cpp
--- a/tensorrtx_amd/csrc/runtime/plan.cpp
+++ b/tensorrtx_amd/csrc/runtime/plan.cpp
@@ -100,7 +100,7 @@
                 for (size_t q = 0; q < m.in.size(); ++q) o << (q ? "," : "") << m.in[q];
                 o << "],\"out\":[" << m.out[0] << "]}";
             }
-            o << "]";
+            o << "]" << (op.sibling_pair ? ",\"sibling_pair\":true" : "");
         }
         o << ",\"lane\":" << op.lane << ",\"waits\":[";
         for (size_t j = 0; j < op.wait_ops.size(); ++j) o << (j ? "," : "") << op.wait_ops[j];
diff --git a/tensorrtx_amd/csrc/runtime/plan.h b/tensorrtx_amd/csrc/runtime/plan.h
--- a/tensorrtx_amd/csrc/runtime/plan.h
+++ b/tensorrtx_amd/csrc/runtime/plan.h
@@ -103,6 +103,7 @@
     int reorg_cin = 0;
     int cout_real = 0;
     std::vector<POp> group;
+    bool sibling_pair = false;
     int src_layer = -1;
     int scale_layer = -1;
     size_t w_off = 0, b_off = 0, s_off = 0;
diff --git a/tensorrtx_amd/csrc/runtime/plan_passes.cpp b/tensorrtx_amd/csrc/runtime/plan_passes.cpp
--- a/tensorrtx_amd/csrc/runtime/plan_passes.cpp
+++ b/tensorrtx_amd/csrc/runtime/plan_passes.cpp
@@ -716,10 +716,72 @@
     }
 }
 
+int lane_limit(const PassInputs& e) {
+    int max_lanes = e.max_aux_streams >= 0 ? 1 + e.max_aux_streams : 4;
+    if (e.opt.lanes > 0) max_lanes = std::max(1, std::min(16, e.opt.lanes));
+    return max_lanes;
+}
+void mark_sibling_pair(Plan& plan, const PassInputs& e) {
+    if (!e.opt.sibling_pair || e.dt != DT_F16 || e.int8 || CalibrationLowering::active()) return;
+    if (lane_limit(e) > 1) return;
+    const int n = (int)plan.ops.size();
+    if (n < 2 || n > 4096) return;
+    auto member_args = [&](const POp& m) {
+        ConvArgs a = m.conv;
+        const PTensor& ti = plan.tensors[m.in[0]];
+        a.N = (ti.nfix ? ti.nfix : plan.max_batch) * ti.nmul;
+        a.M = a.N * a.Ho * a.Wo;
+        return a;
+    };
+    auto shares_elements = [&](int t, int u) {
+        const PTensor &x = plan.tensors[t], &y = plan.tensors[u];
+        if (x.storage != y.storage) return false;
+        if (x.layout != LAY_NHWC || y.layout != LAY_NHWC) return true;
+        return x.rcoff < y.rcoff + std::max(y.C, 1) && y.rcoff < x.rcoff + std::max(x.C, 1);
+    };
+    auto mark_one = [&]() {
+        const std::vector<std::vector<int>> deps = op_dependencies(plan);
+        const Ancestors anc = ancestors(plan, deps, false);
+        for (int i = 0; i + 1 < n; ++i) {
+            const POp& a = plan.ops[i];
+            if (a.kind != OP_CONV_GROUP || a.sibling_pair || plan.ops[i + 1].sibling_pair || a.group.empty() || (int)a.group.size() > kMaxDualGroup) continue;
+            for (int j = i + 1; j < n; ++j) {
+                const POp& b = plan.ops[j];
+                if (b.kind != OP_CONV_GROUP || b.sibling_pair || (j + 1 < n && plan.ops[j + 1].sibling_pair) || b.group.size() != a.group.size()) continue;
+                std::vector<ConvArgs> xa, xb;
+                bool ok = true;
+                for (const POp& ma : a.group) {
+                    const POp* mb = nullptr;
+                    for (const POp& c : b.group)
+                        if (c.in.size() == 1 && ma.in.size() == 1 && c.in[0] == ma.in[0]) mb = &c;
+                    if (!mb || !ma.extra_in.empty() || !mb->extra_in.empty()) { ok = false; break; }
+                    xa.push_back(member_args(ma));
+                    xb.push_back(member_args(*mb));
+                }
+                if (!ok) continue;
+                const int gn = (int)xa.size();
+                if (!conv_dual_group_possible(xa.data(), xb.data(), gn) && !conv_dual_group_possible(xb.data(), xa.data(), gn)) continue;
+                for (int t : a.out) {
+                    for (int u : a.in) ok = ok && !shares_elements(t, u);
+                    for (int u : b.out) ok = ok && !shares_elements(t, u);
+                }
+                for (int t : b.out)
+                    for (int u : a.in) ok = ok && !shares_elements(t, u);
+                for (int k = i; k < j; ++k) ok = ok && !anc.has(k, j);
+                if (!ok) continue;
+                if (j != i + 1) std::rotate(plan.ops.begin() + i + 1, plan.ops.begin() + j, plan.ops.begin() + j + 1);
+                plan.ops[i + 1].sibling_pair = true;
+                return true;
+            }
+        }
+        return false;
+    };
+    while (mark_one()) {}
+}
+
 void assign_lanes(Plan& plan, const PassInputs& e, const std::vector<std::vector<int>>& deps) {
     const int nops = (int)plan.ops.size();
-    int max_lanes = e.max_aux_streams >= 0 ? 1 + e.max_aux_streams : 4;
-    if (e.opt.lanes > 0) max_lanes = std::max(1, std::min(16, e.opt.lanes));
+    const int max_lanes = lane_limit(e);
     std::vector<int> tail(max_lanes, -1);
     plan.num_lanes = 1;
     for (int k = 0; k < nops; ++k) {
@@ -771,6 +833,8 @@
         for (int t : op.out) mark(t);
         if (op.bneck_pair && k > 0)
             for (int t : plan.ops[k - 1].in) mark(t);
+        if (op.sibling_pair && k > 0)
+            for (int t : plan.ops[k - 1].out) mark(t);
     }
     std::vector<std::pair<int, int>> ws_storage;
     for (int k = 0; k < nops; ++k) {
@@ -831,12 +895,15 @@
     chain_sppf_pools(plan, e);
     chain_spp_parallel_pools(plan, e);
     group_convs(plan, e);
+    mark_sibling_pair(plan, e);
     mark_stem_pair(plan, e);
     mark_bneck_pair(plan, e);
     const std::vector<std::vector<int>> deps = op_dependencies(plan);
     assign_lanes(plan, e, deps);
     for (size_t k = 1; k < plan.ops.size(); ++k)
         if (plan.ops[k].bneck_pair && (plan.ops[k].lane != plan.ops[k - 1].lane || plan.ops[k - 1].signal)) plan.ops[k].bneck_pair = false;
+    for (size_t k = 1; k < plan.ops.size(); ++k)
+        if (plan.ops[k].sibling_pair && (plan.ops[k].lane != plan.ops[k - 1].lane || plan.ops[k - 1].signal)) plan.ops[k].sibling_pair = false;
     plan_arena(plan, ancestors(plan, deps, true));
     return true;
 }
```

Measured after the change: 41050, median of 6. 1.04x the previous value.
